# JeanElsner/practical-multi-view

Hardware: AMD Instinct MI355X
Metric: VO frames/sec on 1241x376 KITTI mono @400 tracks, bundle=5 (higher is better)
Workload: dtype u8/int32 front-end, f64 back-end

## Files before the change

### include/pmv_hip.h

```cpp
#ifndef PMV_HIP_H
#define PMV_HIP_H
#include <stdint.h>
#ifdef __cplusplus
extern "C" {
#endif

typedef struct pmv_ctx pmv_ctx;

enum pmv_status {
    PMV_OK = 0,
    PMV_ERR_NO_DEVICE = -1,
    PMV_ERR_INVALID = -2,
    PMV_ERR_CAPACITY = -3,
    PMV_ERR_HIP = -4,
    PMV_ERR_DEGENERATE = -5,
    PMV_ERR_OVERFLOW = -6
};

int pmv_ctx_create(pmv_ctx** out, int device, int max_w, int max_h, int n_slots, int max_tracks,
                   int max_ba_cams, int max_ba_points, int max_ba_obs);
void pmv_ctx_destroy(pmv_ctx* ctx);
const char* pmv_last_error(pmv_ctx* ctx);
const char* pmv_thread_error(void);
int pmv_sync(pmv_ctx* ctx);

int pmv_frame_upload(pmv_ctx* ctx, int slot, const uint8_t* gray, int w, int h, int stride);
int pmv_frame_upload_bgr(pmv_ctx* ctx, int slot, const uint8_t* bgr, int w, int h, int stride);
enum pmv_frame_format { PMV_FRAMES_GRAY = 0, PMV_FRAMES_BGR = 1 };
int pmv_set_frame_format(pmv_ctx* ctx, int format);
int pmv_frames_stage(pmv_ctx* ctx, int first_slot, int n, const uint8_t* gray, int w, int h);
int pmv_frames_build(pmv_ctx* ctx, int first_slot, int n);
int pmv_frames_stream_begin(pmv_ctx* ctx, int first_slot, int n, const uint8_t* gray, int w, int h);
int pmv_frames_stream_end(pmv_ctx* ctx);
int pmv_frame_get_level(pmv_ctx* ctx, int slot, int level, uint8_t* out, int* w, int* h);
int pmv_frame_num_levels(pmv_ctx* ctx, int slot);
#define PMV_PYR_PAD 64
int pmv_frame_get_level_padded(pmv_ctx* ctx, int slot, int level, uint8_t* out, int* pw, int* ph);

typedef struct pmv_clahe_params {
    double clip_limit;
    int tiles_x, tiles_y;
} pmv_clahe_params;
int pmv_frames_clahe(pmv_ctx* ctx, int first_slot, int n, const pmv_clahe_params* p);
int pmv_debug_clahe_launches(pmv_ctx* ctx, long long* out3);

int pmv_remap_map_create(pmv_ctx* ctx, int w, int h, const float* map_x, const float* map_y, int* out_id);
int pmv_remap_map_destroy(pmv_ctx* ctx, int id);
int pmv_frames_remap(pmv_ctx* ctx, int first_slot, int n, int map_id, int border_value);
int pmv_debug_remap_launches(pmv_ctx* ctx, long long* out3);
#define PMV_PREPROC_MAX_MAPS 8
typedef struct pmv_frame_preproc {
    int n_maps;
    int map_ids[PMV_PREPROC_MAX_MAPS];
    int border_value;
    int clahe;
    pmv_clahe_params clahe_params;
} pmv_frame_preproc;
int pmv_set_frame_preproc(pmv_ctx* ctx, const pmv_frame_preproc* p_or_null);
int pmv_get_frame_preproc(pmv_ctx* ctx, pmv_frame_preproc* out);
int pmv_debug_preproc_launches(pmv_ctx* ctx, long long* out4);
int pmv_debug_mem_live(long long* out2);
int pmv_undistort_map_build(const double* K9, const double* dist8, const double* R9_or_null, const double* newK9_or_null, int w, int h, float* map_x,
                            float* map_y);

#define PMV_GFTT_UNLIMITED_CAP 4096
int pmv_detect_gftt(pmv_ctx* ctx, int slot, const int* cells, int n_cells, int max_per_cell, double quality,
                    double min_dist, int* out_xy, int* out_count);
typedef struct pmv_gftt_params {
    double quality;
    double min_dist;
    int    block_size;
    int    use_harris;
    double k;
} pmv_gftt_params;
int pmv_detect_gftt_ex(pmv_ctx* ctx, int slot, const int* cells, int n_cells, int max_per_cell, const pmv_gftt_params* p, const uint8_t* mask,
                       int mask_stride, int* out_xy, int* out_count);
int pmv_debug_gftt_response_ex(pmv_ctx* ctx, int slot, const int* cell, const pmv_gftt_params* p, float* out);
int pmv_debug_gftt_general(pmv_ctx* ctx, int on);
int pmv_detect_shitomasi(pmv_ctx* ctx, int slot, const int* cells, int n_cells, int max_per_cell, double quality,
                         int* out_xy, double* out_score, int* out_count);
int pmv_debug_gftt_response(pmv_ctx* ctx, int slot, const int* cell, float* out);
int pmv_debug_shitomasi_response(pmv_ctx* ctx, int slot, const int* cell, double* out);

typedef struct pmv_subpix_params {
    int win_w, win_h;
    int zero_w, zero_h;
    int max_iter;
    double eps;
} pmv_subpix_params;
int pmv_corner_subpix(pmv_ctx* ctx, int slot, float* xy, int n, const pmv_subpix_params* p, uint8_t* out_iters, uint8_t* out_flags);
int pmv_debug_subpix_launches(pmv_ctx* ctx, long long* out3);

int pmv_detect_fast(pmv_ctx* ctx, int slot, const int* cells, int n_cells, int max_per_cell, int threshold, int nonmax, int* out_xy,
                    float* out_response, int* out_count);

int pmv_knn_match(pmv_ctx* ctx, int src_slot, int cmp_slot, const int* src_xy, int n, const int* cmp_xy, int m, int n_neighbours, int window,
                  int* out_best, float* out_err);
int pmv_lk_track(pmv_ctx* ctx, int prev_slot, int next_slot, const float* prev_xy, int n, float* out_xy,
                 uint8_t* out_status, float* out_err);
typedef struct pmv_lk_params {
    int win;
    int max_level;
    int max_iter;
    double eps;
    float min_eig;
} pmv_lk_params;
int pmv_set_lk_params(pmv_ctx* ctx, const pmv_lk_params* p);
int pmv_get_lk_params(pmv_ctx* ctx, pmv_lk_params* out);
enum { PMV_LK_USE_INITIAL_FLOW = 4, PMV_LK_GET_MIN_EIGENVALS = 8 };
int pmv_lk_track_ex(pmv_ctx* ctx, int prev_slot, int next_slot, const float* prev_xy, int n, float* next_xy , int flags,
                    uint8_t* out_status, float* out_err);
int pmv_lk_track_fb(pmv_ctx* ctx, int prev_slot, int next_slot, const float* prev_xy, int n, float* next_xy , int flags,
                    uint8_t* out_status, float* out_err, float* back_xy, uint8_t* back_status, float* back_err);
int pmv_debug_lk_general(pmv_ctx* ctx, int on);

int pmv_pnp_ransac(pmv_ctx* ctx, const float* obj_xyz, const float* img_xy, int m, const double* K, double* rvec,
                   double* tvec, int iterations, float reproj_err, double confidence, int* out_inliers,
                   int* out_n_inliers);

int pmv_debug_pnp_hypotheses(pmv_ctx* ctx, int n, double* models, int* counts);
int pmv_debug_ba_stamps(pmv_ctx* ctx, unsigned long long* out32);
int pmv_debug_lk_stamps(pmv_ctx* ctx, unsigned long long* out16);

typedef struct pmv_ba_summary {
    double initial_cost, final_cost;
    int iterations;
    int successful_steps;
    int termination;
} pmv_ba_summary;

int pmv_ba_residuals(pmv_ctx* ctx, const double* cams, int nc, const double* pts, int np, const double* obs_xy,
                     const int* cam_idx, const int* pt_idx, int n_obs, const double* K, double* out_r,
                     double* out_J);
int pmv_set_ba_mode(pmv_ctx* ctx, int mode);
int pmv_ba_solve(pmv_ctx* ctx, double* cams, int nc, double* pts, int np, const double* obs_xy, const int* cam_idx,
                 const int* pt_idx, int n_obs, const double* K, double huber_delta, int max_iterations,
                 pmv_ba_summary* summary);

int pmv_fivepoint_hypotheses(pmv_ctx* ctx, const double* q1, const double* q2, int n, const int* samples, int n_hyp, float thr, double* models,
                             int* n_models, int* counts);

int pmv_triangulate_candidates(pmv_ctx* ctx, const double* q1, const double* q2, int n, const double* P1x4,
                               const uint8_t* mask_in, double* out_Q, uint8_t* out_mask, int* out_good);
int pmv_triangulate_candidates_ahead(pmv_ctx* ctx, const double* q1, const double* q2, int n, const double* P1x4, const uint8_t* mask_in,
                                     double* out_Q, uint8_t* out_mask, int* out_good);

int pmv_find_essential_mat(pmv_ctx* ctx, const double* p1_xy, const double* p2_xy, int n, const double* K, double prob, double threshold,
                           double* E9, uint8_t* mask, int* out_found, int* out_samples_drawn);
int pmv_recover_pose(pmv_ctx* ctx, const double* E9, const double* p1_xy, const double* p2_xy, int n, const double* K, double* R9, double* t3,
                     uint8_t* mask, double* tri4n, int* out_good);
int pmv_debug_essential_iters_table(int n, double prob, double* out_denoms, double* out_num);

int pmv_find_fundamental_mat(pmv_ctx* ctx, const float* p1_xy, const float* p2_xy, int n, double threshold, double confidence, double* F9,
                             uint8_t* mask, int* out_found, int* out_samples_drawn);
int pmv_debug_fundamental_iters_table(int n, double confidence, double* out_denoms, double* out_num);
int pmv_debug_set_fundamental_r(int r);
int pmv_debug_fundamental_r(void);
int pmv_debug_whole_rounds(pmv_ctx* ctx, long long* out3);

int pmv_record_enable(pmv_ctx* ctx, int on);
int pmv_record_count(pmv_ctx* ctx);
long long pmv_record_size(pmv_ctx* ctx, int i);
int pmv_record_get(pmv_ctx* ctx, int i, void* out, long long capacity);

int pmv_prof_enable(pmv_ctx* ctx, int on);
int pmv_prof_select(pmv_ctx* ctx, unsigned mask);
int pmv_prof_kernel_count(void);
int pmv_lk_counters(pmv_ctx* ctx, unsigned long long* out3, int reset);
const char* pmv_prof_kernel_name(int id);
int pmv_prof_read(pmv_ctx* ctx, int id, int* launches, double* total_ms, double* max_ms);

typedef struct pmv_pipeline_params {
    int n_frames, w, h;
    int min_tracked_features, tracked_features_tol, init_frames, bundle_size, ba_iterations;
    int extractor;
    int threaded;
    int n_threads;
    int build_pyramids;
    int matcher;
    int device_fivepoint;
} pmv_pipeline_params;
typedef struct pmv_pipeline_result pmv_pipeline_result;

int pmv_pipeline_run(pmv_ctx* ctx, const pmv_pipeline_params* params, const double* K9, const double* gt_poses12,
                     pmv_pipeline_result** out);
int pmv_pipeline_run_streamed(pmv_ctx* ctx, const pmv_pipeline_params* params, const double* K9, const double* gt_poses12,
                              const uint8_t* host_frames, pmv_pipeline_result** out);
int pmv_pipeline_run_batch(pmv_ctx* ctx, int B, const pmv_pipeline_params* params, const double* K9, const double* const* gt_poses12,
                           const int* first_slot, pmv_pipeline_result** out);
int pmv_debug_batch_launches(pmv_ctx* ctx, long long* out4);
int pmv_pipeline_run_batch_streamed(pmv_ctx* ctx, int B, const pmv_pipeline_params* params, const double* K9, const double* const* gt_poses12,
                                    const uint8_t* const* host_frames, const int* first_slot, int ring, pmv_pipeline_result** out);
#define PMV_BATCH_INGEST_STATS 6
int pmv_batch_ingest_stats(pmv_ctx* ctx, double* out);
int pmv_batch_stats(pmv_ctx* ctx, long long* counts10, double* times15);

int pmv_batch_open(pmv_ctx* ctx, int n_seq, const int* sizes_wh, int n_sizes);
int pmv_batch_close(pmv_ctx* ctx);
int pmv_batch_frame_upload(pmv_ctx* ctx, int slot, const uint8_t* pixels, int w, int h, int stride, int format);
int pmv_batch_frame_upload_clahe(pmv_ctx* ctx, int slot, const uint8_t* pixels, int w, int h, int stride, int format, const pmv_clahe_params* p);
int pmv_batch_frame_upload_remap(pmv_ctx* ctx, int slot, const uint8_t* pixels, int w, int h, int stride, int format, int map_id, int border_value,
                                 const pmv_clahe_params* clahe_or_null);
int pmv_batch_lk_track(pmv_ctx* ctx, int prev_slot, int next_slot, const float* prev_xy, int n, float* out_xy, uint8_t* out_status, float* out_err);
int pmv_batch_lk_track_ex(pmv_ctx* ctx, int prev_slot, int next_slot, const float* prev_xy, int n, float* next_xy , int flags,
                          uint8_t* out_status, float* out_err);
int pmv_batch_lk_track_fb(pmv_ctx* ctx, int prev_slot, int next_slot, const float* prev_xy, int n, float* next_xy , int flags,
                          uint8_t* out_status, float* out_err, float* back_xy, uint8_t* back_status, float* back_err);
int pmv_batch_knn_match(pmv_ctx* ctx, int src_slot, int cmp_slot, const int* src_xy, int n, const int* cmp_xy, int m, int n_neighbours, int window,
                        int* out_best, float* out_err);
int pmv_batch_detect_gftt(pmv_ctx* ctx, int slot, const int* cells, int n_cells, int max_per_cell, double quality, double min_dist, int* out_xy,
                          int* out_count);
int pmv_batch_detect_gftt_ex(pmv_ctx* ctx, int slot, const int* cells, int n_cells, int max_per_cell, const pmv_gftt_params* p, const uint8_t* mask,
                             int mask_stride, int* out_xy, int* out_count);
int pmv_batch_corner_subpix(pmv_ctx* ctx, int slot, float* xy, int n, const pmv_subpix_params* p, uint8_t* out_iters, uint8_t* out_flags);
int pmv_batch_detect_shitomasi(pmv_ctx* ctx, int slot, const int* cells, int n_cells, int max_per_cell, double quality, int* out_xy, double* out_score,
                               int* out_count);
int pmv_batch_detect_fast(pmv_ctx* ctx, int slot, const int* cells, int n_cells, int max_per_cell, int threshold, int nonmax, int* out_xy,
                          float* out_response, int* out_count);
int pmv_batch_pnp_ransac(pmv_ctx* ctx, int seq, const float* obj_xyz, const float* img_xy, int m, const double* K, double* rvec, double* tvec,
                         int iterations, float reproj_err, double confidence, int* out_inliers, int* out_n_inliers);
int pmv_batch_ba_solve(pmv_ctx* ctx, int seq, double* cams, int nc, double* pts, int np, const double* obs_xy, const int* cam_idx, const int* pt_idx,
                       int n_obs, const double* K, double huber_delta, int max_iterations, pmv_ba_summary* summary);
int pmv_batch_triangulate_candidates(pmv_ctx* ctx, int seq, const double* q1, const double* q2, int n, const double* P1x4, const uint8_t* mask_in,
                                     double* out_Q, uint8_t* out_mask, int* out_good);
int pmv_batch_fivepoint_hypotheses(pmv_ctx* ctx, int seq, const double* q1, const double* q2, int n, const int* samples, int n_hyp, float thr,
                                   double* models, int* n_models, int* counts);
int pmv_batch_find_essential_mat(pmv_ctx* ctx, int seq, const double* p1_xy, const double* p2_xy, int n, const double* K, double prob, double threshold,
                                 double* E9, uint8_t* mask, int* out_found, int* out_samples_drawn);
int pmv_batch_recover_pose(pmv_ctx* ctx, int seq, const double* E9, const double* p1_xy, const double* p2_xy, int n, const double* K, double* R9, double* t3,
                           uint8_t* mask, double* tri4n, int* out_good);
int pmv_batch_find_fundamental_mat(pmv_ctx* ctx, int seq, const float* p1_xy, const float* p2_xy, int n, double threshold, double confidence,
                                   double* F9, uint8_t* mask, int* out_found, int* out_samples_drawn);
int pmv_batch_upload_stats(pmv_ctx* ctx, long long* out4);
int pmv_batch_upload_rounds(pmv_ctx* ctx, int* out8, int capacity);

void pmv_pipeline_free(pmv_pipeline_result* r);
void pmv_pipeline_release(pmv_pipeline_result* r);
void pmv_pipeline_drain(void);
int pmv_pipeline_num_poses(const pmv_pipeline_result* r);
void pmv_pipeline_get_poses(const pmv_pipeline_result* r, double* out12);
int pmv_pipeline_num_frames(const pmv_pipeline_result* r);
int pmv_pipeline_frame_feature_count(const pmv_pipeline_result* r, int k);
void pmv_pipeline_get_frame_features(const pmv_pipeline_result* r, int k, int* out3);
int pmv_pipeline_stats_count(void);
void pmv_pipeline_get_stats(const pmv_pipeline_result* r, double* out25);

#ifdef __cplusplus
}
#endif
#endif
```

### practical-multi-view_amd/__init__.py

```python
import ctypes as C
import os

import numpy as np

from . import build as _build

HERE = os.path.dirname(os.path.abspath(__file__))
ROOT = os.path.dirname(HERE)

_u8p = C.POINTER(C.c_uint8)
_i32p = C.POINTER(C.c_int)
_f32p = C.POINTER(C.c_float)
_f64p = C.POINTER(C.c_double)


class PmvError(RuntimeError):
    def __init__(self, code, msg):
        super().__init__(f"pmv error {code}: {msg}")
        self.code = code


class BaSummary(C.Structure):
    _fields_ = [("initial_cost", C.c_double), ("final_cost", C.c_double), ("iterations", C.c_int),
                ("successful_steps", C.c_int), ("termination", C.c_int)]


class LKParams(C.Structure):
    _fields_ = [("win", C.c_int), ("max_level", C.c_int), ("max_iter", C.c_int), ("eps", C.c_double), ("min_eig", C.c_float)]


class GfttParams(C.Structure):
    _fields_ = [("quality", C.c_double), ("min_dist", C.c_double), ("block_size", C.c_int), ("use_harris", C.c_int), ("k", C.c_double)]


class SubpixParams(C.Structure):
    _fields_ = [("win_w", C.c_int), ("win_h", C.c_int), ("zero_w", C.c_int), ("zero_h", C.c_int), ("max_iter", C.c_int), ("eps", C.c_double)]


class ClaheParams(C.Structure):
    _fields_ = [("clip_limit", C.c_double), ("tiles_x", C.c_int), ("tiles_y", C.c_int)]


def _clahe_params(who, clip_limit, tiles):
    if isinstance(clip_limit, (bool, np.bool_)) or not isinstance(clip_limit, (int, float, np.integer, np.floating)):
        raise ValueError(f"{who}: clip_limit must be a number, got {clip_limit!r}")
    try:
        tx, ty = tiles
    except (TypeError, ValueError):
        raise ValueError(f"{who}: tiles is a (tiles_x, tiles_y) pair, got {tiles!r}") from None
    for t in (tx, ty):
        if isinstance(t, (bool, np.bool_)) or not isinstance(t, (int, np.integer)):
            raise ValueError(f"{who}: tiles is a pair of integers, got {tiles!r}")
    return ClaheParams(float(clip_limit), int(tx), int(ty))


PREPROC_MAX_MAPS = 8


class FramePreproc(C.Structure):
    _fields_ = [("n_maps", C.c_int), ("map_ids", C.c_int * PREPROC_MAX_MAPS), ("border_value", C.c_int), ("clahe", C.c_int), ("clahe_params", ClaheParams)]


def _preproc_arg(who, remap, border_value, clahe):
    def is_int(v):
        return isinstance(v, (int, np.integer)) and not isinstance(v, (bool, np.bool_))
    if remap is None:
        ids = []
    elif is_int(remap):
        ids = [int(remap)]
    else:
        try:
            ids = list(remap)
        except TypeError:
            raise ValueError(f"{who}: remap is a map id or a sequence of map ids, got {remap!r}") from None
        if isinstance(remap, (str, bytes)) or not all(is_int(i) for i in ids):
            raise ValueError(f"{who}: remap is a map id or a sequence of integer map ids, got {remap!r}")
        ids = [int(i) for i in ids]
    if len(ids) > PREPROC_MAX_MAPS:
        raise ValueError(f"{who}: at most {PREPROC_MAX_MAPS} maps, got {len(ids)}")
    if not is_int(border_value) or not 0 <= int(border_value) <= 255:
        raise ValueError(f"{who}: border_value is an integer in 0..255, got {border_value!r}")
    p = FramePreproc()
    p.n_maps = len(ids)
    for k, i in enumerate(ids):
        p.map_ids[k] = i
    p.border_value = int(border_value)
    if clahe is not None:
        try:
            clip, tiles = clahe
        except (TypeError, ValueError):
            raise ValueError(f"{who}: clahe is None or (clip_limit, (tiles_x, tiles_y)), got {clahe!r}") from None
        cp = _clahe_params(who, clip, tiles)
        if not (cp.clip_limit >= 0.0 and np.isfinite(cp.clip_limit)):
            raise ValueError(f"{who}: clip_limit is a finite number >= 0, got {clip!r}")
        if not (1 <= cp.tiles_x <= 16 and 1 <= cp.tiles_y <= 16):
            raise ValueError(f"{who}: tiles are in 1..16 each, got {tiles!r}")
        p.clahe = 1
        p.clahe_params = cp
    if not ids and clahe is None and int(border_value) == 0:
        return None
    return p


def _remap_arg(who, remap):
    def is_int(v):
        return isinstance(v, (int, np.integer)) and not isinstance(v, (bool, np.bool_))
    if is_int(remap):
        return int(remap), 0
    try:
        map_id, border = remap
    except (TypeError, ValueError):
        raise ValueError(f"{who}: remap is a map id or (map_id, border_value), got {remap!r}") from None
    if not is_int(map_id) or not is_int(border):
        raise ValueError(f"{who}: remap is a map id or (map_id, border_value) of integers, got {remap!r}")
    return int(map_id), int(border)


def undistort_map(K, dist, size, R=None, new_K=None):
    def mat(m, name):
        a = np.ascontiguousarray(m, np.float64)
        if a.shape != (3, 3):
            raise ValueError(f"undistort_map: {name} is 3 x 3, got shape {a.shape}")
        return a
    Km = mat(K, "K")
    d = np.asarray(dist, np.float64).reshape(-1)
    if d.size > 8:
        raise ValueError(f"undistort_map: at most 8 distortion coefficients (k1, k2, p1, p2, k3, k4, k5, k6), got {d.size}")
    d8 = np.zeros(8, np.float64)
    d8[:d.size] = d
    try:
        w, h = size
    except (TypeError, ValueError):
        raise ValueError(f"undistort_map: size is (w, h), got {size!r}") from None
    w, h = int(w), int(h)
    if w < 1 or h < 1:
        raise ValueError(f"undistort_map: size {size!r}")
    Rm = None if R is None else mat(R, "R")
    Nm = None if new_K is None else mat(new_K, "new_K")
    mx, my = np.empty((h, w), np.float32), np.empty((h, w), np.float32)
    lib = load_library()
    _f32p = C.POINTER(C.c_float)
    lib.pmv_undistort_map_build.argtypes = [_f64p, _f64p, _f64p, _f64p, C.c_int, C.c_int, _f32p, _f32p]
    rc = lib.pmv_undistort_map_build(_p(Km, _f64p), _p(d8, _f64p), None if Rm is None else _p(Rm, _f64p), None if Nm is None else _p(Nm, _f64p), w, h,
                                     _p(mx, _f32p), _p(my, _f32p))
    if rc != 0:
        raise PmvError(rc, lib.pmv_last_error(None).decode())
    return mx, my


def mem_live():
    lib = load_library()
    out = (C.c_longlong * 2)()
    lib.pmv_debug_mem_live.argtypes = [C.POINTER(C.c_longlong)]
    rc = lib.pmv_debug_mem_live(out)
    if rc != 0:
        raise PmvError(rc, lib.pmv_last_error(None).decode())
    return int(out[0]), int(out[1])


LK_USE_INITIAL_FLOW = 4
LK_GET_MIN_EIGENVALS = 8

ABI_SYMBOLS = [
    "pmv_ctx_create", "pmv_ctx_destroy", "pmv_last_error", "pmv_thread_error", "pmv_sync",
    "pmv_frame_upload", "pmv_frame_upload_bgr", "pmv_set_frame_format", "pmv_frames_stage", "pmv_frames_build", "pmv_frames_stream_begin", "pmv_frames_stream_end", "pmv_frame_get_level", "pmv_frame_get_level_padded", "pmv_frame_num_levels",
    "pmv_detect_gftt", "pmv_detect_shitomasi", "pmv_detect_fast", "pmv_knn_match", "pmv_debug_gftt_response", "pmv_debug_shitomasi_response",
    "pmv_detect_gftt_ex", "pmv_debug_gftt_response_ex", "pmv_debug_gftt_general", "pmv_batch_detect_gftt_ex",
    "pmv_corner_subpix", "pmv_batch_corner_subpix", "pmv_debug_subpix_launches",
    "pmv_frames_clahe", "pmv_batch_frame_upload_clahe", "pmv_debug_clahe_launches",
    "pmv_remap_map_create", "pmv_remap_map_destroy", "pmv_frames_remap", "pmv_debug_remap_launches", "pmv_batch_frame_upload_remap", "pmv_undistort_map_build",
    "pmv_set_frame_preproc", "pmv_get_frame_preproc", "pmv_debug_preproc_launches",
    "pmv_debug_mem_live",
    "pmv_lk_track", "pmv_lk_track_ex", "pmv_lk_track_fb", "pmv_set_lk_params", "pmv_get_lk_params", "pmv_debug_lk_general", "pmv_set_ba_mode", "pmv_pnp_ransac", "pmv_debug_pnp_hypotheses", "pmv_debug_ba_stamps", "pmv_debug_lk_stamps", "pmv_ba_residuals", "pmv_ba_solve", "pmv_triangulate_candidates", "pmv_triangulate_candidates_ahead", "pmv_fivepoint_hypotheses",
    "pmv_find_essential_mat", "pmv_recover_pose", "pmv_debug_essential_iters_table",
    "pmv_find_fundamental_mat", "pmv_debug_fundamental_iters_table", "pmv_debug_set_fundamental_r", "pmv_debug_fundamental_r", "pmv_debug_whole_rounds",
    "pmv_record_enable", "pmv_record_count", "pmv_record_size", "pmv_record_get",
    "pmv_prof_enable", "pmv_prof_select", "pmv_prof_kernel_count", "pmv_lk_counters", "pmv_prof_kernel_name", "pmv_prof_read",
    "pmv_pipeline_run", "pmv_pipeline_run_streamed", "pmv_pipeline_run_batch", "pmv_pipeline_run_batch_streamed", "pmv_batch_ingest_stats", "pmv_batch_stats", "pmv_debug_batch_launches", "pmv_pipeline_free", "pmv_pipeline_release", "pmv_pipeline_drain", "pmv_pipeline_num_poses", "pmv_pipeline_get_poses", "pmv_pipeline_num_frames",
    "pmv_pipeline_frame_feature_count", "pmv_pipeline_get_frame_features", "pmv_pipeline_stats_count", "pmv_pipeline_get_stats",
    "pmv_batch_open", "pmv_batch_close", "pmv_batch_frame_upload", "pmv_batch_upload_stats", "pmv_batch_upload_rounds",
    "pmv_batch_lk_track", "pmv_batch_lk_track_ex", "pmv_batch_lk_track_fb", "pmv_batch_knn_match", "pmv_batch_detect_gftt", "pmv_batch_detect_shitomasi", "pmv_batch_detect_fast",
    "pmv_batch_pnp_ransac", "pmv_batch_ba_solve", "pmv_batch_triangulate_candidates", "pmv_batch_fivepoint_hypotheses",
    "pmv_batch_find_essential_mat", "pmv_batch_recover_pose", "pmv_batch_find_fundamental_mat",
]


GFTT_UNLIMITED_CAP = 4096


class PipelineParams(C.Structure):
    _fields_ = [("n_frames", C.c_int), ("w", C.c_int), ("h", C.c_int), ("min_tracked_features", C.c_int),
                ("tracked_features_tol", C.c_int), ("init_frames", C.c_int), ("bundle_size", C.c_int),
                ("ba_iterations", C.c_int), ("extractor", C.c_int), ("threaded", C.c_int), ("n_threads", C.c_int),
                ("build_pyramids", C.c_int), ("matcher", C.c_int), ("device_fivepoint", C.c_int)]


STAT_KEYS = ["lk_calls", "lk_points", "detect_calls", "pnp_calls", "pnp_points", "tri_calls", "ba_calls", "ba_obs",
             "ba_points", "heuristic_motion", "seconds", "init_offset", "n_landmarks", "scale", "t_lk", "t_detect", "t_pnp", "t_tri",
             "t_ba", "t_pnp_kernel", "t_ba_kernel", "t_tri_essential", "t_tri_pose", "tri_hypotheses", "tri_ahead"]


BATCH_INGEST_KEYS = ["rounds", "frames", "bytes", "memcpy_s", "ingest_wait_s", "seq_wait_s"]


FRAME_FORMATS = {"gray": 0, "bgr": 1}


def _host_frames(frames, fmt, who, h=None, w=None, n=None):
    if fmt != "bgr":
        f = np.ascontiguousarray(frames, np.uint8)
        if f.ndim != 3 or (h is not None and f.shape[1:] != (h, w)) or (n is not None and f.shape[0] != n):
            want = f"({'n' if n is None else n}, {'h' if h is None else h}, {'w' if w is None else w})"
            raise ValueError(f"{who}: the context's frame format is gray: frames must be {want} uint8, got {f.shape} (set_frame_format(\"bgr\") for colour frames)")
        return f
    f = np.asarray(frames)
    ok = f.dtype == np.uint8 and f.ndim == 4 and f.shape[3] == 3 and f.shape[0] >= 1
    if ok and h is not None:
        ok = f.shape[1:3] == (h, w)
    if ok and n is not None:
        ok = f.shape[0] == n
    if not ok:
        want = f"({'n' if n is None else n}, {'h' if h is None else h}, {'w' if w is None else w}, 3)"
        raise ValueError(f"{who}: the context's frame format is BGR: frames must be {want} uint8, got {f.shape} {f.dtype}")
    return np.ascontiguousarray(f)


def _batch_streamed_args(seqs, w, h, ring, first_slot, fmt="gray"):
    if len(seqs) < 1:
        raise ValueError("pipeline_run_batch_streamed: no sequences")
    if int(ring) != ring or ring < 1:
        raise ValueError(f"pipeline_run_batch_streamed: ring must be a positive integer, got {ring!r}")
    if (w is None) != (h is None):
        raise ValueError("pipeline_run_batch_streamed: w and h are given together, or both None (each sequence's own array shape)")
    ws = hs = [None] * len(seqs)
    if w is not None:
        ws = _per_sequence("pipeline_run_batch_streamed", "w", w, len(seqs))
        hs = _per_sequence("pipeline_run_batch_streamed", "h", h, len(seqs))
    frames, gts = [], []
    for b, seq in enumerate(seqs):
        if len(seq) != 2:
            raise ValueError(f"pipeline_run_batch_streamed: sequence {b} must be (frames, gt_poses)")
        f, gt = seq
        f = np.asarray(f)
        if fmt == "bgr":
            f = _host_frames(f, fmt, f"pipeline_run_batch_streamed: sequence {b}", hs[b], ws[b])
        elif f.dtype != np.uint8 or f.ndim != 3 or (ws[b] is not None and f.shape[1:] != (hs[b], ws[b])):
            want = f"(n, {hs[b]}, {ws[b]})" if ws[b] is not None else "(n, h, w)"
            raise ValueError(f"pipeline_run_batch_streamed: sequence {b}: frames must be {want} uint8, got {f.shape} {f.dtype}")
        f = np.ascontiguousarray(f)
        g = np.ascontiguousarray(gt, np.float64)
        if g.size != 12 * f.shape[0]:
            raise ValueError(f"pipeline_run_batch_streamed: sequence {b}: {f.shape[0]} frames but {g.size / 12:g} pose rows")
        frames.append(f)
        gts.append(g.reshape(f.shape[0], 12))
    B = len(frames)
    first = [b * int(ring) for b in range(B)] if first_slot is None else [int(v) for v in first_slot]
    if len(first) != B:
        raise ValueError(f"pipeline_run_batch_streamed: {len(first)} first slots for {B} sequences")
    return frames, gts, first


BATCH_UPLOAD_KEYS = ["rounds", "frames", "level0_launches", "pyrdown_launches"]


def _session_sizes(sizes):
    try:
        pairs = [tuple(p) for p in sizes]
    except TypeError:
        raise ValueError(f"batch_open: sizes must be a sequence of (w, h) integer pairs, got {sizes!r}") from None
    if not pairs:
        raise ValueError("batch_open: no sizes")
    for p in pairs:
        if len(p) != 2 or any(isinstance(v, (bool, np.bool_)) or not isinstance(v, (int, np.integer)) for v in p):
            raise ValueError(f"batch_open: sizes must be (w, h) integer pairs, got {p!r}")
    return np.asarray(pairs, np.int32).reshape(-1)


def _upload_source(frame, fmt):
    if not isinstance(fmt, str) or fmt not in FRAME_FORMATS:
        raise ValueError(f"batch_frame_upload: fmt must be one of {sorted(FRAME_FORMATS)}, got {fmt!r}")
    nd = 3 if fmt == "bgr" else 2
    if isinstance(frame, np.ndarray):
        if frame.dtype != np.uint8:
            raise ValueError(f"batch_frame_upload: frames are uint8, got {frame.dtype}")
        shape, strides, addr = tuple(frame.shape), tuple(frame.strides), frame.ctypes.data
    elif all(hasattr(frame, a) for a in ("data_ptr", "shape", "stride")):
        dt = str(getattr(frame, "dtype", "uint8"))
        if not dt.endswith("uint8"):
            raise ValueError(f"batch_frame_upload: frames are uint8, got {dt}")
        shape, strides, addr = tuple(int(v) for v in frame.shape), tuple(int(v) for v in frame.stride()), int(frame.data_ptr())
    else:
        raise ValueError(f"batch_frame_upload: a uint8 numpy array or an object with data_ptr(), shape and stride() is needed, got {type(frame).__name__}")
    if len(shape) != nd or (nd == 3 and shape[2] != 3):
        want = "(h, w, 3)" if nd == 3 else "(h, w)"
        raise ValueError(f"batch_frame_upload: a {fmt} frame is {want} uint8, got shape {shape}")
    h, w = shape[0], shape[1]
    if h < 1 or w < 1:
        raise ValueError(f"batch_frame_upload: empty frame {shape}")
    if (nd == 2 and strides[1] != 1) or (nd == 3 and (strides[2] != 1 or strides[1] != 3)):
        raise ValueError(f"batch_frame_upload: the pixels of a row must be contiguous (strides {strides} for shape {shape}); only the row stride is free")
    stride = strides[0] if h > 1 else max(strides[0], w * (nd == 3 and 3 or 1))
    if stride < w * (3 if nd == 3 else 1) or stride >= 2 ** 31:
        raise ValueError(f"batch_frame_upload: row stride {strides[0]} bytes for rows of {w * (3 if nd == 3 else 1)} bytes (overlapping or reversed rows)")
    return addr, w, h, stride, FRAME_FORMATS[fmt], frame


def _per_sequence(who, name, value, B):
    if np.ndim(value) == 0:
        return [int(value)] * B
    v = [int(x) for x in value]
    if len(v) != B:
        raise ValueError(f"{who}: {name} has {len(v)} entries for {B} sequences")
    return v


class PipelineResult:

    def __init__(self, lib, handle, want_features=True):
        n = lib.pmv_pipeline_num_poses(handle)
        self.poses = np.zeros((n, 12), np.float64)
        if n:
            lib.pmv_pipeline_get_poses(handle, _p(self.poses, _f64p))
        self.features = []
        if want_features:
            for k in range(lib.pmv_pipeline_num_frames(handle)):
                c = lib.pmv_pipeline_frame_feature_count(handle, k)
# ... 298 lines not shown
        return out

    def debug_gftt_general(self, on):
        self._ck(self.lib.pmv_debug_gftt_general(self.h, 1 if on else 0))

    def _corner_subpix(self, fn, ck, slot, xy, win, zero_zone, max_iter, eps, return_info):
        if not isinstance(xy, np.ndarray) or xy.dtype != np.float32 or xy.ndim != 2 or xy.shape[1] != 2:
            raise ValueError("corner_subpix: xy must be an (n, 2) float32 array")
        if len(win) != 2 or len(zero_zone) != 2:
            raise ValueError("corner_subpix: win and zero_zone are (w, h) pairs of half sizes")
        out = np.ascontiguousarray(xy).copy()
        n = out.shape[0]
        iters = np.zeros(n, np.uint8)
        flags = np.zeros(n, np.uint8)
        p = SubpixParams(int(win[0]), int(win[1]), int(zero_zone[0]), int(zero_zone[1]), int(max_iter), float(eps))
        fn.argtypes = [C.c_void_p, C.c_int, _f32p, C.c_int, C.POINTER(SubpixParams), _u8p, _u8p]
        ck(fn(self.h, int(slot), _p(out, _f32p), n, C.byref(p), _p(iters, _u8p) if return_info else None, _p(flags, _u8p) if return_info else None))
        return (out, iters, flags) if return_info else out

    def corner_subpix(self, slot, xy, win=(5, 5), zero_zone=(-1, -1), max_iter=30, eps=0.01, return_info=False):
        return self._corner_subpix(self.lib.pmv_corner_subpix, self._ck, slot, xy, win, zero_zone, max_iter, eps, return_info)

    def debug_subpix_launches(self):
        out = (C.c_longlong * 3)()
        self.lib.pmv_debug_subpix_launches.argtypes = [C.c_void_p, C.POINTER(C.c_longlong)]
        self._ck(self.lib.pmv_debug_subpix_launches(self.h, out))
        return [int(v) for v in out]

    def detect_shitomasi(self, slot, cells, max_per_cell, quality=0.4):
        cells = np.ascontiguousarray(cells, np.int32).reshape(-1, 4)
        n = cells.shape[0]
        xy = np.zeros((n, max(max_per_cell, 1), 2), np.int32)
        sc = np.zeros((n, max(max_per_cell, 1)), np.float64)
        cnt = np.zeros(n, np.int32)
        self._ck(self.lib.pmv_detect_shitomasi(self.h, slot, _p(cells, _i32p), n, max_per_cell, C.c_double(quality),
                                               _p(xy, _i32p), _p(sc, _f64p), _p(cnt, _i32p)))
        return [(xy[i, : cnt[i]].copy(), sc[i, : cnt[i]].copy()) for i in range(n)]

    def detect_fast(self, slot, cells, max_per_cell, threshold=10, nonmax=True):
        cells = np.ascontiguousarray(cells, np.int32).reshape(-1, 4)
        n = cells.shape[0]
        cap = max(max_per_cell, 1)
        xy = np.zeros((n, cap, 2), np.int32)
        rs = np.zeros((n, cap), np.float32)
        cnt = np.zeros(n, np.int32)
        self._ck(self.lib.pmv_detect_fast(self.h, slot, _p(cells, _i32p), n, max_per_cell, threshold, 1 if nonmax else 0, _p(xy, _i32p), _p(rs, _f32p),
                                          _p(cnt, _i32p)))
        return [(xy[i, : cnt[i]].copy(), rs[i, : cnt[i]].copy()) for i in range(n)]

    def knn_match(self, src_slot, cmp_slot, src_xy, cmp_xy, neighbours=7, window=15):
        s = np.ascontiguousarray(src_xy, np.int32).reshape(-1, 2)
        c = np.ascontiguousarray(cmp_xy, np.int32).reshape(-1, 2)
        best = np.zeros(max(len(s), 1), np.int32)
        err = np.zeros(max(len(s), 1), np.float32)
        self._ck(self.lib.pmv_knn_match(self.h, src_slot, cmp_slot, _p(s, _i32p), len(s), _p(c, _i32p), len(c), neighbours, window, _p(best, _i32p), _p(err, _f32p)))
        return best[: len(s)].copy(), err[: len(s)].copy()

    def gftt_response(self, slot, cell):
        cell = np.ascontiguousarray(cell, np.int32)
        out = np.zeros((cell[3], cell[2]), np.float32)
        self._ck(self.lib.pmv_debug_gftt_response(self.h, slot, _p(cell, _i32p), _p(out, _f32p)))
        return out

    def shitomasi_response(self, slot, cell):
        cell = np.ascontiguousarray(cell, np.int32)
        out = np.zeros((cell[3], cell[2]), np.float64)
        self._ck(self.lib.pmv_debug_shitomasi_response(self.h, slot, _p(cell, _i32p), _p(out, _f64p)))
        return out

    def lk_track(self, prev_slot, next_slot, prev_xy):
        p = np.ascontiguousarray(prev_xy, np.float32).reshape(-1, 2)
        n = p.shape[0]
        out = np.zeros((n, 2), np.float32)
        st = np.zeros(n, np.uint8)
        err = np.zeros(n, np.float32)
        self._ck(self.lib.pmv_lk_track(self.h, prev_slot, next_slot, _p(p, _f32p), n, _p(out, _f32p), _p(st, _u8p),
                                       _p(err, _f32p)))
        return out, st, err

    def _lk_ex(self, fn, ck, fb, prev_slot, next_slot, prev_xy, init_xy, min_eigenvals):
        p = np.ascontiguousarray(prev_xy, np.float32).reshape(-1, 2)
        n = p.shape[0]
        flags = (LK_USE_INITIAL_FLOW if init_xy is not None else 0) | (LK_GET_MIN_EIGENVALS if min_eigenvals else 0)
        nxt = np.zeros((n, 2), np.float32) if init_xy is None else np.array(init_xy, np.float32).reshape(-1, 2)
        if nxt.shape[0] != n:
            raise ValueError(f"init_xy has {nxt.shape[0]} points, prev_xy {n}")
        st = np.zeros(n, np.uint8)
        err = np.zeros(n, np.float32)
        args = [self.h, int(prev_slot), int(next_slot), _p(p, _f32p), n, _p(nxt, _f32p), flags, _p(st, _u8p), _p(err, _f32p)]
        if not fb:
            ck(fn(*args))
            return nxt, st, err
        bxy = np.zeros((n, 2), np.float32)
        bst = np.zeros(n, np.uint8)
        berr = np.zeros(n, np.float32)
        ck(fn(*args, _p(bxy, _f32p), _p(bst, _u8p), _p(berr, _f32p)))
        return nxt, st, err, bxy, bst, berr

    def lk_track_ex(self, prev_slot, next_slot, prev_xy, init_xy=None, min_eigenvals=False):
        return self._lk_ex(self.lib.pmv_lk_track_ex, self._ck, False, prev_slot, next_slot, prev_xy, init_xy, min_eigenvals)

    def lk_track_fb(self, prev_slot, next_slot, prev_xy, init_xy=None, min_eigenvals=False):
        return self._lk_ex(self.lib.pmv_lk_track_fb, self._ck, True, prev_slot, next_slot, prev_xy, init_xy, min_eigenvals)

    def set_lk_params(self, win=32, max_level=4, max_iter=30, eps=0.01, min_eig=1e-4):
        p = LKParams(int(win), int(max_level), int(max_iter), float(eps), float(min_eig))
        self.lib.pmv_set_lk_params.argtypes = [C.c_void_p, C.POINTER(LKParams)]
        self._ck(self.lib.pmv_set_lk_params(self.h, C.byref(p)))

    def lk_params(self):
        p = LKParams()
        self.lib.pmv_get_lk_params.argtypes = [C.c_void_p, C.POINTER(LKParams)]
        self._ck(self.lib.pmv_get_lk_params(self.h, C.byref(p)))
        return dict(win=p.win, max_level=p.max_level, max_iter=p.max_iter, eps=p.eps, min_eig=p.min_eig)

    def debug_lk_general(self, on):
        self._ck(self.lib.pmv_debug_lk_general(self.h, 1 if on else 0))

    def pnp_ransac(self, obj_xyz, img_xy, K, rvec, tvec, iterations=100, reproj_err=8.0, confidence=0.99):
        o = np.ascontiguousarray(obj_xyz, np.float32).reshape(-1, 3)
        i2 = np.ascontiguousarray(img_xy, np.float32).reshape(-1, 2)
        m = o.shape[0]
        Kd = np.ascontiguousarray(K, np.float64).reshape(9)
        rv = np.array(rvec, np.float64).reshape(3).copy()
        tv = np.array(tvec, np.float64).reshape(3).copy()
        inl = np.zeros(max(m, 1), np.int32)
        nin = C.c_int()
        self._ck(self.lib.pmv_pnp_ransac(self.h, _p(o, _f32p), _p(i2, _f32p), m, _p(Kd, _f64p), _p(rv, _f64p),
                                         _p(tv, _f64p), iterations, C.c_float(reproj_err), C.c_double(confidence),
                                         _p(inl, _i32p), C.byref(nin)))
        return rv, tv, inl[: nin.value].copy()

    def pnp_hypotheses(self, n=100):
        models = np.zeros((n, 6), np.float64)
        counts = np.zeros(n, np.int32)
        self._ck(self.lib.pmv_debug_pnp_hypotheses(self.h, n, _p(models, _f64p), _p(counts, _i32p)))
        return models, counts

    def ba_residuals(self, cams, pts, obs_xy, cam_idx, pt_idx, K):
        cams = np.ascontiguousarray(cams, np.float64).reshape(-1, 6)
        pts = np.ascontiguousarray(pts, np.float64).reshape(-1, 3)
        obs = np.ascontiguousarray(obs_xy, np.float64).reshape(-1, 2)
        ci = np.ascontiguousarray(cam_idx, np.int32)
        pi = np.ascontiguousarray(pt_idx, np.int32)
        Kd = np.ascontiguousarray(K, np.float64).reshape(9)
        n = obs.shape[0]
        r = np.zeros((n, 2), np.float64)
        J = np.zeros((n, 2, 9), np.float64)
        self._ck(self.lib.pmv_ba_residuals(self.h, _p(cams, _f64p), cams.shape[0], _p(pts, _f64p), pts.shape[0],
                                           _p(obs, _f64p), _p(ci, _i32p), _p(pi, _i32p), n, _p(Kd, _f64p),
                                           _p(r, _f64p), _p(J, _f64p)))
        return r, J

    def set_ba_mode(self, mode):
        self._ck(self.lib.pmv_set_ba_mode(self.h, int(mode)))

    def ba_solve(self, cams, pts, obs_xy, cam_idx, pt_idx, K, huber=1.0, max_iterations=5):
        cams = np.array(cams, np.float64).reshape(-1, 6).copy()
        pts = np.array(pts, np.float64).reshape(-1, 3).copy()
        obs = np.ascontiguousarray(obs_xy, np.float64).reshape(-1, 2)
        ci = np.ascontiguousarray(cam_idx, np.int32)
        pi = np.ascontiguousarray(pt_idx, np.int32)
        Kd = np.ascontiguousarray(K, np.float64).reshape(9)
        s = BaSummary()
        self._ck(self.lib.pmv_ba_solve(self.h, _p(cams, _f64p), cams.shape[0], _p(pts, _f64p), pts.shape[0],
                                       _p(obs, _f64p), _p(ci, _i32p), _p(pi, _i32p), obs.shape[0], _p(Kd, _f64p),
                                       C.c_double(huber), max_iterations, C.byref(s)))
        return cams, pts, s

    def fivepoint_hypotheses(self, q1, q2, samples, thr):
        q1 = np.ascontiguousarray(q1, np.float64).reshape(-1, 2)
        q2 = np.ascontiguousarray(q2, np.float64).reshape(-1, 2)
        s = np.ascontiguousarray(samples, np.int32).reshape(-1, 5)
        nh = s.shape[0]
        models = np.zeros((nh, 10, 9), np.float64)
        nm = np.zeros(nh, np.int32)
        counts = np.zeros((nh, 10), np.int32)
        self._ck(self.lib.pmv_fivepoint_hypotheses(self.h, _p(q1, _f64p), _p(q2, _f64p), q1.shape[0], _p(s, _i32p), nh, C.c_float(thr), _p(models, _f64p),
                                                   _p(nm, _i32p), _p(counts, _i32p)))
        return models, nm, counts

    def triangulate_candidates(self, q1, q2, P1x4, mask_in):
        q1 = np.ascontiguousarray(q1, np.float64).reshape(-1, 2)
        q2 = np.ascontiguousarray(q2, np.float64).reshape(-1, 2)
        n = q1.shape[0]
        P = np.ascontiguousarray(P1x4, np.float64).reshape(48)
        mi = np.ascontiguousarray(mask_in, np.uint8).reshape(n)
        Q = np.zeros((4, 4, n), np.float64)
        mask = np.zeros((4, n), np.uint8)
        good = np.zeros(4, np.int32)
        self._ck(self.lib.pmv_triangulate_candidates(self.h, _p(q1, _f64p), _p(q2, _f64p), n, _p(P, _f64p), _p(mi, _u8p),
                                                     _p(Q, _f64p), _p(mask, _u8p), _p(good, _i32p)))
        return Q, mask, good

    @staticmethod
    def _two_view_args(p1, p2, K):
        p1 = np.ascontiguousarray(p1, np.float64).reshape(-1, 2)
        p2 = np.ascontiguousarray(p2, np.float64).reshape(-1, 2)
        if p1.shape != p2.shape:
            raise ValueError(f"p1 {p1.shape} and p2 {p2.shape}: one (x, y) pair per correspondence in each")
        return p1, p2, np.ascontiguousarray(K, np.float64).reshape(9)

    def _find_essential(self, call, ck, head, p1, p2, K, prob, threshold):
        p1, p2, Kd = self._two_view_args(p1, p2, K)
        n = p1.shape[0]
        E = np.zeros(9, np.float64)
        mask = np.zeros(n, np.uint8)
        found, drawn = C.c_int(), C.c_int()
        ck(call(self.h, *head, _p(p1, _f64p), _p(p2, _f64p), n, _p(Kd, _f64p), C.c_double(prob), C.c_double(threshold), _p(E, _f64p), _p(mask, _u8p),
                C.byref(found), C.byref(drawn)))
        return bool(found.value), E.reshape(3, 3), mask, drawn.value

    def _recover_pose(self, call, ck, head, E, p1, p2, K, mask):
        p1, p2, Kd = self._two_view_args(p1, p2, K)
        n = p1.shape[0]
        Ed = np.ascontiguousarray(E, np.float64).reshape(9)
        m = np.array(mask, np.uint8).reshape(n).copy()
        R, t, tri = np.zeros(9, np.float64), np.zeros(3, np.float64), np.zeros((4, n), np.float64)
        good = C.c_int()
        ck(call(self.h, *head, _p(Ed, _f64p), _p(p1, _f64p), _p(p2, _f64p), n, _p(Kd, _f64p), _p(R, _f64p), _p(t, _f64p), _p(m, _u8p), _p(tri, _f64p),
                C.byref(good)))
        return R.reshape(3, 3), t, m, tri, good.value

    def find_essential_mat(self, p1, p2, K, prob=0.99, threshold=1.0):
        return self._find_essential(self.lib.pmv_find_essential_mat, self._ck, (), p1, p2, K, prob, threshold)

    def recover_pose(self, E, p1, p2, K, mask):
        return self._recover_pose(self.lib.pmv_recover_pose, self._ck, (), E, p1, p2, K, mask)

    def _find_fundamental(self, call, ck, head, p1, p2, threshold, confidence):
        p1 = np.ascontiguousarray(p1, np.float32).reshape(-1, 2)
        p2 = np.ascontiguousarray(p2, np.float32).reshape(-1, 2)
        if p1.shape != p2.shape:
            raise ValueError(f"p1 {p1.shape} and p2 {p2.shape}: one (x, y) pair per correspondence in each")
        n = p1.shape[0]
        F = np.zeros(9, np.float64)
        mask = np.zeros(n, np.uint8)
        found, drawn = C.c_int(), C.c_int()
        ck(call(self.h, *head, _p(p1, _f32p), _p(p2, _f32p), n, C.c_double(threshold), C.c_double(confidence), _p(F, _f64p), _p(mask, _u8p),
                C.byref(found), C.byref(drawn)))
        return bool(found.value), F.reshape(3, 3), mask, drawn.value

    def find_fundamental_mat(self, p1, p2, threshold=1.0, confidence=0.99):
        return self._find_fundamental(self.lib.pmv_find_fundamental_mat, self._ck, (), p1, p2, threshold, confidence)

    def record_enable(self, on=True):
        self._ck(self.lib.pmv_record_enable(self.h, 1 if on else 0))

    def records(self):
        self.lib.pmv_record_size.restype = C.c_longlong
        self.lib.pmv_record_size.argtypes = [C.c_void_p, C.c_int]
        self.lib.pmv_record_get.argtypes = [C.c_void_p, C.c_int, C.c_void_p, C.c_longlong]
        out = []
        for i in range(self.lib.pmv_record_count(self.h)):
            nb = self.lib.pmv_record_size(self.h, i)
            buf = np.zeros(nb, np.uint8)
            self._ck(self.lib.pmv_record_get(self.h, i, buf.ctypes.data_as(C.c_void_p), nb))
            out.append(parse_record(buf))
        return out

    def prof_enable(self, on=True):
        self._ck(self.lib.pmv_prof_enable(self.h, 1 if on else 0))

    def lk_counters(self, reset=False):
        out = (C.c_ulonglong * 3)()
        self._ck(self.lib.pmv_lk_counters(self.h, out, 1 if reset else 0))
        return int(out[0]), int(out[1]), int(out[2])

    def prof_select(self, names):
        self.lib.pmv_prof_kernel_name.restype = C.c_char_p
        mask = 0
        for i in range(self.lib.pmv_prof_kernel_count()):
            if self.lib.pmv_prof_kernel_name(i).decode() in names:
                mask |= 1 << i
        self._ck(self.lib.pmv_prof_select(self.h, C.c_uint(mask)))

    def prof_read(self):
        self.lib.pmv_prof_kernel_name.restype = C.c_char_p
        out = {}
        for i in range(self.lib.pmv_prof_kernel_count()):
            n, tot, mx = C.c_int(), C.c_double(), C.c_double()
            self._ck(self.lib.pmv_prof_read(self.h, i, C.byref(n), C.byref(tot), C.byref(mx)))
            if n.value:
                out[self.lib.pmv_prof_kernel_name(i).decode()] = (n.value, tot.value, mx.value)
        return out

    def pipeline_run(self, n_frames, w, h, K, gt_poses, min_tracked=400, tol=150, init_frames=5, bundle_size=5,
                     ba_iterations=5, extractor=0, threaded=0, build_pyramids=1, want_features=True, n_threads=1, async_free=False,
                     defer_free=False, host_frames=None, matcher=0, device_fivepoint=0):
        P = PipelineParams(n_frames, w, h, min_tracked, tol, init_frames, bundle_size, ba_iterations, extractor, threaded,
                           n_threads, build_pyramids, matcher, device_fivepoint)
        Kd = np.ascontiguousarray(K, np.float64).reshape(9)
        gt = np.ascontiguousarray(gt_poses, np.float64).reshape(n_frames, 12)
        out = C.c_void_p()
        if host_frames is not None:
            hf = _host_frames(host_frames, self.frame_format, "pipeline_run: host_frames", h, w, n_frames)
            self._ck(self.lib.pmv_pipeline_run_streamed(self.h, C.byref(P), _p(Kd, _f64p), _p(gt, _f64p), _p(hf, _u8p), C.byref(out)))
        else:
            self._ck(self.lib.pmv_pipeline_run(self.h, C.byref(P), _p(Kd, _f64p), _p(gt, _f64p), C.byref(out)))
        ok = False
        try:
            r = PipelineResult(self.lib, out, want_features)
            ok = True
        finally:
            if not (ok and defer_free):
                if async_free:
# ... 282 lines not shown
```

### practical-multi-view_amd/csrc/backend.h

```cpp
#pragma once
#include <hip/hip_runtime.h>
#include <stdint.h>
#include <stddef.h>
#include "../../include/pmv_hip.h"
#include "pmv_mem.h"
#include "backend_layout.h"

namespace pmv {


struct BackendBuffers {
    unsigned done_seq = 0;
    Buf<double> d_cams, d_pts, d_obs, d_K;
    Buf<int> d_cam_idx, d_pt_idx, d_pobs_start, d_pobs_list, d_cobs_start, d_cobs_list;
    Buf<double> d_x, d_cand, d_scale, d_diag, d_D2, d_step, d_res, d_J, d_Einv, d_gp, d_Yd, d_Wd, d_S, d_rhs, d_Gpart, d_summary;
    size_t ydwd_elems = 0, gpart_elems = 0;
    Buf<unsigned long long> d_stamps;
    Buf<void> d_bastate;
    Buf<double> d_bapart;
    Buf<char> d_tri_in, d_tri_out;
    Buf<char> d_fp_work;
    Buf<char> d_ess_in;
    Buf<char> d_fund_in;
    Buf<char> h_stage;
    Buf<char> d_ba_io;
    Buf<char> d_pnp_in;
    Buf<char> d_pnp_out;
    Buf<float> d_obj, d_img;
    Buf<int> d_samples, d_counts, d_inliers, d_info;
    Buf<double> d_models, d_rt, d_Kp;
    Buf<uint8_t> d_masks;
};

struct BAArgs {
    double* cams; double* pts; const double* obs; const int* cam_idx; const int* pt_idx; const double* K;
    const int* pobs_start; const int* pobs_list; const int* cobs_start; const int* cobs_list;
    const int4* erec;
    int nc, np, nobs, max_iterations;
    double huber;
    double *x, *cand, *scale, *diag, *D2, *step, *res, *J, *Einv, *gp, *Yd, *Wd, *S, *rhs, *Gpart, *summary;
    int ldw, krows, tiles_r, tiles_c, kslices, kper, gp_rows;
    unsigned long long* stamps;
    double* out;
    unsigned done_seq;
};

hipError_t launch_ba_residuals(hipStream_t s, const double* cams, const double* pts, const double* obs, const int* cam_idx,
                               const int* pt_idx, int nobs, const double* K, double* out_r, double* out_J);
hipError_t launch_ba_lm(hipStream_t s, const BAArgs& A);
constexpr int BA_MAX_ITERATIONS = 512;
hipError_t launch_ba_multi(hipStream_t s, const BAArgs& A, void* d_state, double* d_part);
hipError_t launch_pnp(hipStream_t s, const float* d_obj, const float* d_img, int m, const double* d_K, const int* d_samples,
                      int n_hyp, float thr, double confidence, double* d_models, uint8_t* d_masks, int* d_counts,
                      double* d_rt_out, int* d_inliers, int* d_info, char* host_out ,
                      unsigned long long* d_stamps , unsigned done_seq = 0 );

struct BAProb {
    BAArgs A;
    void* st2[2];
    int* chol_flags;
    double *part_cost, *part_gmax, *part4, *Ublk, *rhsblk, *candrot, *tmp3;
    int nbo, nbp, clear_blocks, tiles;
};
struct BABatchDims { int n_probs, max_eval_blocks, max_nc, max_nbp, max_tiles, max_m, max_iterations; };
void ba_fill_prob(BAProb& P, const BAArgs& A, void* d_state, double* d_part);
hipError_t launch_ba_multi_batch(hipStream_t s, const BAProb* d_probs, const BABatchDims& D);
hipError_t launch_ba_lm_batch(hipStream_t s, const BAArgs* d_args, int n_probs, int max_m);
struct PnPProblem {
    const float* obj; const float* img; const int* samples; const double* K;
    double* models; uint8_t* masks; int* counts; double* rt_out; int* inliers; int* info; char* host_out;
    int m, n_hyp; float thr; double confidence;
};
hipError_t launch_pnp_batch(hipStream_t s, const PnPProblem* d_probs, int n_probs, int max_hyp);
struct FivePointProblem {
    const int* samples; const double* q1; const double* q2;
    double* models_d; int* n_models_d;
    double* models_h; int* n_models_h; int* counts_h;
    int n, n_hyp; float thr;
};
hipError_t launch_fivepoint_batch(hipStream_t s, const FivePointProblem* d_probs, int n_probs, int max_hyp);
struct EssentialProblem {
    const double* q1; const double* q2;
    const double* iters;
    char* out;
    int n, max_iters; float thr;
    unsigned done_seq;
};
static_assert(sizeof(EssentialProblem) <= ESS_HDR, "the record is the header of the input block");
constexpr int ESS_MAX_WAVES = 16;
constexpr int ESS_DEFAULT_WAVES = 8;
int essential_round_width();
hipError_t launch_essential_ransac(hipStream_t s, const EssentialProblem* d_probs, int n_probs);
struct FundamentalProblem {
    const float* p1; const float* p2;
    const double* iters;
    char* out;
    int n, max_iters; float thr;
    unsigned done_seq;
};
static_assert(sizeof(FundamentalProblem) <= ESS_HDR, "the record is the header of the input block");
constexpr int FUND_MAX_R = 64;
constexpr int FUND_DEFAULT_R = 64;
int fundamental_round_width();
void fundamental_set_round_width(int r);
hipError_t launch_fundamental_ransac(hipStream_t s, const FundamentalProblem* d_probs, int n_probs);
struct DltProblem { const double* P1x4; const double* q1; const double* q2; const uint8_t* mask_in; double* Q; uint8_t* mask; int n; };
hipError_t launch_tri_dlt_batch(hipStream_t s, const DltProblem* d_probs, int n_probs, int max_n);
hipError_t launch_tri_dlt(hipStream_t s, const double* d_P1x4, const double* d_q1, const double* d_q2, const uint8_t* d_mask_in, int n,
                          double* d_Q, uint8_t* d_mask);

struct PnPProblem; struct DltProblem;
}
struct pmv_ctx;
namespace pmv {
int backend_alloc(pmv_ctx* c, BackendBuffers** out);
void backend_free(BackendBuffers* b);
int pnp_check(pmv_ctx* ctx, const float* obj_xyz, const float* img_xy, int m, const double* K, double* rvec, double* tvec, int iterations,
              double confidence, int* out_inliers, int* out_n_inliers);
int pnp_prepare(pmv_ctx* ctx, BackendBuffers* b, const float* obj_xyz, const float* img_xy, int m, const double* K, int iterations, float reproj_err,
                double confidence, PnPProblem* P, PnPLayout* L);
void pnp_finish(pmv_ctx* ctx, BackendBuffers* b, const float* obj_xyz, const float* img_xy, int m, const double* K, double* rvec, double* tvec,
                int iterations, float reproj_err, double confidence, const PnPLayout& L, int* out_inliers, int* out_n_inliers);
int ba_check(pmv_ctx* ctx, const double* cams, int nc, const double* pts, int np, const double* obs_xy, const int* cam_idx, const int* pt_idx,
             int n_obs, const double* K, double huber_delta, int max_iterations);
int ba_prepare(pmv_ctx* ctx, BackendBuffers* b, const double* cams, int nc, const double* pts, int np, const double* obs_xy, const int* cam_idx,
               const int* pt_idx, int n_obs, const double* K, double huber_delta, int max_iterations, bool multi, BAArgs* A, BaIoLayout* L);
void ba_finish(pmv_ctx* ctx, BackendBuffers* b, double* cams, int nc, double* pts, int np, const double* obs_xy, const int* cam_idx,
               const int* pt_idx, int n_obs, const double* K, double huber_delta, int max_iterations, const BaIoLayout& L, pmv_ba_summary* summary);
int fivepoint_prepare(pmv_ctx* ctx, BackendBuffers* b, const double* q1, const double* q2, int n, const int* samples, int n_hyp, float thr,
                      FivePointProblem* P, FivePointLayout* L);
void fivepoint_finish(BackendBuffers* b, int n_hyp, const FivePointLayout& L, double* models, int* n_models, int* counts);
int essential_check(pmv_ctx* ctx, const char* who, const double* p1_xy, const double* p2_xy, int n, const double* K, double prob, double threshold,
                    double* E9, uint8_t* mask, int* out_found, int* out_samples_drawn);
int essential_prepare(pmv_ctx* ctx, BackendBuffers* b, const double* p1_xy, const double* p2_xy, int n, const double* K, double prob, double threshold,
                      EssentialProblem* P, WholeLayout* L);
volatile unsigned* whole_done_word(BackendBuffers* b, const WholeLayout& L);
void whole_finish(BackendBuffers* b, int n, const WholeLayout& L, double* M9, uint8_t* mask, int* out_found, int* out_samples_drawn);
int fundamental_check(pmv_ctx* ctx, const char* who, const float* p1_xy, const float* p2_xy, int n, double threshold, double confidence, double* F9,
                      uint8_t* mask, int* out_found, int* out_samples_drawn);
int fundamental_prepare(pmv_ctx* ctx, BackendBuffers* b, const float* p1_xy, const float* p2_xy, int n, double threshold, double confidence,
                        FundamentalProblem* P, WholeLayout* L);
int recover_pose_check(pmv_ctx* ctx, const char* who, const double* E9, const double* p1_xy, const double* p2_xy, int n, const double* K, double* R9,
                       double* t3, uint8_t* mask, double* tri4n, int* out_good);
int dlt_prepare(pmv_ctx* ctx, BackendBuffers* b, const double* q1, const double* q2, int n, const double* P1x4, const uint8_t* mask_in, DltProblem* P,
                DltLayout* L);
void dlt_finish(pmv_ctx* ctx, BackendBuffers* b, const double* q1, const double* q2, int n, const double* P1x4, const uint8_t* mask_in,
                const DltLayout& L, double* out_Q, uint8_t* out_mask, int* out_good);
}
```

### practical-multi-view_amd/csrc/backend.hip

```cpp
#include "pmv_ctx.h"
#include "backend.h"
#include "pmv_wait.h"
#include "vo_pipeline.h"
#include <cmath>
#include <cstring>
#include <cstdio>
#include <cstdlib>
#include <vector>
#include <algorithm>

namespace pmv {

__global__ __launch_bounds__(256) void k_stage_block(const uint4* __restrict__ src, uint4* __restrict__ dst, unsigned n16) { BACKEND_PRIO();
    for (unsigned i = blockIdx.x * 256 + threadIdx.x; i < n16; i += gridDim.x * 256) dst[i] = src[i];
}
hipError_t stage_block(hipStream_t s, const void* mapped_src, void* dst, size_t bytes, unsigned max_blocks) {
    const unsigned n16 = (unsigned)((bytes + 15) >> 4);
    hipLaunchKernelGGL(k_stage_block, dim3(std::min(max_blocks, (n16 + 255u) / 256u)), dim3(256), 0, s, (const uint4*)mapped_src, (uint4*)dst, n16);
    return hipGetLastError();
}
static bool stage_by_kernel() { static const bool on = !(getenv("PMV_BA_STAGE") && !strcmp(getenv("PMV_BA_STAGE"), "dma")); return on; }

static int round_up(int a, int b) { return (a + b - 1) / b * b; }

int backend_alloc(pmv_ctx* c, BackendBuffers** out) {
    BackendBuffers* b = new BackendBuffers();
    *out = b;
    const size_t nc = (size_t)std::max(c->max_ba_cams, 1), np = (size_t)std::max(c->max_ba_points, 1), no = (size_t)std::max(c->max_ba_obs, 1);
    const size_t n = 6 * nc + 3 * np, m = 6 * nc;
    const size_t ldw = (size_t)round_up((int)m + 1, 16), krows = (size_t)round_up((int)(3 * np), 16);
    b->ydwd_elems = krows * ldw;
    b->gpart_elems = (size_t)8 * ldw * ldw;
    const size_t mt = (size_t)c->max_tracks;
    const BackendCaps caps = backend_caps(c->max_tracks, c->max_ba_cams, c->max_ba_points, c->max_ba_obs);
    const MemRow rows[] = {
        {&b->d_cams, nc * 6 * 8, MEM_DEVICE}, {&b->d_pts, np * 3 * 8, MEM_DEVICE}, {&b->d_obs, no * 2 * 8, MEM_DEVICE}, {&b->d_K, 9 * 8, MEM_DEVICE},
        {&b->d_cam_idx, no * 4, MEM_DEVICE}, {&b->d_pt_idx, no * 4, MEM_DEVICE},
        {&b->d_pobs_start, (np + 1) * 4, MEM_DEVICE}, {&b->d_pobs_list, no * 4, MEM_DEVICE},
        {&b->d_cobs_start, (nc + 1) * 4, MEM_DEVICE}, {&b->d_cobs_list, no * 4, MEM_DEVICE},
        {&b->d_x, 2 * n * 8, MEM_DEVICE}, {&b->d_cand, n * 8, MEM_DEVICE}, {&b->d_scale, n * 8, MEM_DEVICE}, {&b->d_diag, n * 8, MEM_DEVICE},
        {&b->d_D2, n * 8, MEM_DEVICE}, {&b->d_step, n * 8, MEM_DEVICE},
        {&b->d_res, 2 * no * 2 * 8, MEM_DEVICE}, {&b->d_J, 2 * no * 18 * 8, MEM_DEVICE},
        {&b->d_Einv, np * 9 * 8, MEM_DEVICE}, {&b->d_gp, np * 3 * 8, MEM_DEVICE},
        {&b->d_Yd, 2 * b->ydwd_elems * 8, MEM_DEVICE},
        {&b->d_Wd, b->ydwd_elems * 8, MEM_DEVICE},
        {&b->d_S, m * m * 8, MEM_DEVICE}, {&b->d_rhs, m * 8, MEM_DEVICE},
        {&b->d_Gpart, b->gpart_elems * 8, MEM_DEVICE},
        {&b->d_summary, 8 * 8, MEM_DEVICE},
        {&b->d_stamps, 32 * 8, MEM_DEVICE},
        {&b->d_bastate, 512 + 4 * BA_MAX_ITERATIONS, MEM_DEVICE},
        {&b->d_bapart, ((size_t)(no + 255) / 256 + 5 * ((size_t)(np + 63) / 64) + 64 * (size_t)nc + 3 * (size_t)no + 64) * 8, MEM_DEVICE},
        {&b->d_obj, mt * 12, MEM_DEVICE}, {&b->d_img, mt * 8, MEM_DEVICE},
        {&b->d_samples, MAX_HYP * 5 * 4, MEM_DEVICE}, {&b->d_counts, MAX_HYP * 4, MEM_DEVICE},
        {&b->d_inliers, mt * 4, MEM_DEVICE}, {&b->d_info, 16, MEM_DEVICE},
        {&b->d_models, MAX_HYP * 6 * 8, MEM_DEVICE}, {&b->d_rt, 6 * 8, MEM_DEVICE}, {&b->d_Kp, 9 * 8, MEM_DEVICE},
        {&b->d_masks, (size_t)MAX_HYP * mt, MEM_DEVICE},
        {&b->d_ba_io, caps.ba_io, MEM_DEVICE},
        {&b->d_pnp_in, caps.pnp_in, MEM_DEVICE}, {&b->d_pnp_out, caps.pnp_out, MEM_DEVICE},
        {&b->d_tri_in, caps.tri_in, MEM_DEVICE}, {&b->d_tri_out, caps.tri_out, MEM_DEVICE},
        {&b->d_fp_work, (size_t)FP_MAX_HYP * (90 * 8 + 4) + 64, MEM_DEVICE},
        {&b->d_ess_in, caps.ess_in, MEM_DEVICE},
        {&b->h_stage, caps.h_stage, MEM_MAPPED},
    };
    hipError_t e = mem_alloc_table(rows, sizeof(rows) / sizeof(rows[0]));
    if (e == hipSuccess) e = hipMemset(b->d_stamps, 0, 32 * 8);
    if (e != hipSuccess) { set_err(c, "backend_alloc: %s", hipGetErrorString(e)); return PMV_ERR_HIP; }
    return PMV_OK;
}
int backend_create(pmv_ctx* c) { return backend_alloc(c, &c->be); }

void backend_free(BackendBuffers* b) { delete b; }
void backend_destroy(pmv_ctx* c) {
    if (c->s_ahead) { (void)hipStreamSynchronize(c->s_ahead); (void)hipStreamDestroy(c->s_ahead); c->s_ahead = nullptr; }
    backend_free(c->be); c->be = nullptr;
    backend_free(c->be_ahead); c->be_ahead = nullptr;
}

struct CvRNG {
    uint64_t state;
    explicit CvRNG(uint64_t s) : state(s ? s : 0xffffffffULL) {}
    unsigned next() { state = (uint64_t)(unsigned)state * 4164903690U + (unsigned)(state >> 32); return (unsigned)state; }
    int uniform(int a, int b) { return a == b ? a : (int)(next() % (unsigned)(b - a) + a); }
};

}

using namespace pmv;

#define CKC(x) do { hipError_t e_ = (x); if (e_ != hipSuccess) { set_err(ctx, "%s: %s", #x, hipGetErrorString(e_)); return PMV_ERR_HIP; } } while (0)
#define REQ(cond, code, ...) do { if (!(cond)) { set_err(ctx, __VA_ARGS__); return code; } } while (0)

int pmv::pnp_check(pmv_ctx* ctx, const float* obj_xyz, const float* img_xy, int m, const double* K, double* rvec, double* tvec, int iterations,
                   double confidence, int* out_inliers, int* out_n_inliers) {
    REQ(ctx && obj_xyz && img_xy && K && rvec && tvec && out_inliers && out_n_inliers, PMV_ERR_INVALID, "pmv_pnp_ransac: null argument");
    *out_n_inliers = 0;
    REQ(m <= ctx->max_tracks, PMV_ERR_CAPACITY, "pmv_pnp_ransac: m=%d exceeds max_tracks=%d", m, ctx->max_tracks);
    REQ(m >= 6, PMV_ERR_DEGENERATE, "pmv_pnp_ransac: %d correspondences (need >= 6)", m);
    REQ(iterations >= 1 && iterations <= MAX_HYP, PMV_ERR_CAPACITY, "pmv_pnp_ransac: iterations=%d (1..%d)", iterations, MAX_HYP);
    REQ(confidence > 0 && confidence < 1, PMV_ERR_INVALID, "pmv_pnp_ransac: confidence must be in (0,1)");
    return PMV_OK;
}
int pmv::pnp_prepare(pmv_ctx* ctx, BackendBuffers* b, const float* obj_xyz, const float* img_xy, int m, const double* K, int iterations, float reproj_err,
                     double confidence, PnPProblem* P, PnPLayout* Lout) {
    const PnPLayout L = pnp_layout((size_t)m, (size_t)iterations);
    REQ(L.total <= b->h_stage.cap && L.in_bytes <= b->d_pnp_in.cap && L.total - L.out <= b->d_pnp_out.cap, PMV_ERR_CAPACITY,
        "pmv_pnp_ransac: m=%d with %d iterations does not fit the staging blocks", m, iterations);
    char* hs = (char*)b->h_stage;
    double* h_K = (double*)(hs + L.K);
    int* h_samples = (int*)(hs + L.samples);
    memcpy(h_K, K, 72);
    for (int k = -16; k <= 16; k++) h_K[10 + 16 + k] = std::exp(k * std::log(10.));
    memcpy(hs + L.obj, obj_xyz, (size_t)m * 12);
    memcpy(hs + L.img, img_xy, (size_t)m * 8);
    CvRNG rng((uint64_t)-1);
    for (int it = 0; it < iterations; it++) {
        int* idx = h_samples + it * 5;
        for (int i = 0; i < 5;) {
            int idx_i;
            for (;;) {
                idx_i = idx[i] = rng.uniform(0, m);
                int j = 0;
                for (; j < i; j++) if (idx_i == idx[j]) break;
                if (j == i) break;
            }
            i++;
        }
    }
    P->K = (const double*)(b->d_pnp_in + L.K);
    P->obj = (const float*)(b->d_pnp_in + L.obj);
    P->img = (const float*)(b->d_pnp_in + L.img);
    P->samples = (const int*)(b->d_pnp_in + L.samples);
    P->models = b->d_models; P->masks = b->d_masks; P->counts = b->d_counts;
    P->rt_out = (double*)b->d_pnp_out;
    P->info = (int*)(b->d_pnp_out + PNP_OUT_INFO);
    P->inliers = (int*)(b->d_pnp_out + PNP_OUT_INLIERS);
    P->host_out = b->h_stage.dm() + L.out;
    P->m = m; P->n_hyp = iterations;
    P->thr = (float)((double)reproj_err * (double)reproj_err);
    P->confidence = confidence;
    *Lout = L;
    return PMV_OK;
}
void pmv::pnp_finish(pmv_ctx* ctx, BackendBuffers* b, const float* obj_xyz, const float* img_xy, int m, const double* K, double* rvec, double* tvec,
                     int iterations, float reproj_err, double confidence, const PnPLayout& L, int* out_inliers, int* out_n_inliers) {
    const PnPResultHdr* R = (const PnPResultHdr*)((const char*)b->h_stage + L.out);
    const double* h_rt = R->rt;
    const int* h_inl = (const int*)((const char*)b->h_stage + L.inliers);
    const int n = R->info[0];
    if (ctx->log.on) {
        std::lock_guard<std::mutex> lk(ctx->log.mu);
        ctx->log.blobs.emplace_back();
        std::vector<char>& bl = ctx->log.blobs.back();
        const int hdr[4] = {0, m, iterations, n};
        const double opt[2] = {(double)reproj_err, confidence};
        pmv_call_log::put(bl, hdr, 16); pmv_call_log::put(bl, obj_xyz, (size_t)m * 12); pmv_call_log::put(bl, img_xy, (size_t)m * 8);
        pmv_call_log::put(bl, K, 72); pmv_call_log::put(bl, rvec, 24); pmv_call_log::put(bl, tvec, 24); pmv_call_log::put(bl, opt, 16);
        pmv_call_log::put(bl, h_rt, 48); pmv_call_log::put(bl, h_inl, (size_t)(n > 0 ? n : 0) * 4);
    }
    for (int i = 0; i < 3; i++) { rvec[i] = h_rt[i]; tvec[i] = h_rt[3 + i]; }
    *out_n_inliers = n;
    if (n > 0) memcpy(out_inliers, h_inl, (size_t)n * 4);
}

static int wait_done_word(pmv_ctx* ctx, hipStream_t s, volatile unsigned* done_word, unsigned done_seq, bool by_word) {
    if (by_word) CKC(spin_for_word(s, done_word, done_seq));
    else CKC(hipStreamSynchronize(s));
    return PMV_OK;
}

extern "C" {

static bool stamps_on() { static const bool on = getenv("PMV_BA_STAMPS") != nullptr; return on; }

int pmv_pnp_ransac(pmv_ctx* ctx, const float* obj_xyz, const float* img_xy, int m, const double* K, double* rvec, double* tvec,
                   int iterations, float reproj_err, double confidence, int* out_inliers, int* out_n_inliers) {
    int rc = pnp_check(ctx, obj_xyz, img_xy, m, K, rvec, tvec, iterations, confidence, out_inliers, out_n_inliers);
    if (rc) return rc;
    tl_prof = &ctx->prof;
    CKC(hipSetDevice(ctx->device));
    static const char* const dump = getenv("PMV_DUMP_PNP");
    if (dump) {
        if (FILE* f = fopen(dump, "ab")) {
            fwrite(&m, 4, 1, f); fwrite(obj_xyz, 12, m, f); fwrite(img_xy, 8, m, f); fwrite(K, 8, 9, f); fwrite(rvec, 8, 3, f); fwrite(tvec, 8, 3, f);
            fclose(f);
        }
    }
    BackendBuffers* b = ctx->be;
    hipStream_t s = ctx->s_back;
    PnPProblem P;
    PnPLayout L;
    if ((rc = pnp_prepare(ctx, b, obj_xyz, img_xy, m, K, iterations, reproj_err, confidence, &P, &L))) return rc;
    if (stage_by_kernel()) CKC(stage_block(s, b->h_stage.dm(), b->d_pnp_in, L.in_bytes, 8));
    else CKC(hipMemcpyAsync(b->d_pnp_in, b->h_stage, L.in_bytes, hipMemcpyHostToDevice, s));
    const bool flag_wait = back_wait_by_word();
    volatile unsigned* done_word = (volatile unsigned*)((char*)b->h_stage + L.done);
    if (++b->done_seq == 0) b->done_seq = 1;
    *done_word = 0;
    CKC(launch_pnp(s, P.obj, P.img, m, P.K, P.samples, iterations, P.thr, confidence, P.models, P.masks, P.counts,
                   P.rt_out, P.inliers, P.info, P.host_out, stamps_on() ? b->d_stamps : nullptr, flag_wait ? b->done_seq : 0u));
    if ((rc = wait_done_word(ctx, s, done_word, b->done_seq, flag_wait))) return rc;
    pnp_finish(ctx, b, obj_xyz, img_xy, m, K, rvec, tvec, iterations, reproj_err, confidence, L, out_inliers, out_n_inliers);
    return PMV_OK;
}

int pmv_record_enable(pmv_ctx* ctx, int on) {
    REQ(ctx, PMV_ERR_INVALID, "null ctx");
    if (on) ctx->log.blobs.clear();
    ctx->log.on = on != 0;
    return PMV_OK;
}
int pmv_record_count(pmv_ctx* ctx) { return ctx ? (int)ctx->log.blobs.size() : PMV_ERR_INVALID; }
long long pmv_record_size(pmv_ctx* ctx, int i) {
    if (!ctx || i < 0 || i >= (int)ctx->log.blobs.size()) return PMV_ERR_INVALID;
    return (long long)ctx->log.blobs[i].size();
}
int pmv_record_get(pmv_ctx* ctx, int i, void* out, long long capacity) {
    REQ(ctx && out && i >= 0 && i < (int)ctx->log.blobs.size(), PMV_ERR_INVALID, "pmv_record_get: bad argument");
    REQ(capacity >= (long long)ctx->log.blobs[i].size(), PMV_ERR_CAPACITY, "pmv_record_get: buffer too small");
    memcpy(out, ctx->log.blobs[i].data(), ctx->log.blobs[i].size());
    return PMV_OK;
}

int pmv_debug_ba_stamps(pmv_ctx* ctx, unsigned long long* out32) {
    REQ(ctx && out32, PMV_ERR_INVALID, "null argument");
    CKC(hipSetDevice(ctx->device));
    CKC(hipStreamSynchronize(ctx->s_back));
    CKC(hipMemcpy(out32, ctx->be->d_stamps, 256, hipMemcpyDeviceToHost));
    return PMV_OK;
}

int pmv_debug_pnp_hypotheses(pmv_ctx* ctx, int n, double* models, int* counts) {
    REQ(ctx && models && counts && n >= 1 && n <= MAX_HYP, PMV_ERR_INVALID, "pmv_debug_pnp_hypotheses: bad argument");
    CKC(hipSetDevice(ctx->device));
    CKC(hipStreamSynchronize(ctx->s_back));
    CKC(hipMemcpy(models, ctx->be->d_models, (size_t)n * 48, hipMemcpyDeviceToHost));
    CKC(hipMemcpy(counts, ctx->be->d_counts, (size_t)n * 4, hipMemcpyDeviceToHost));
    return PMV_OK;
}

int pmv_ba_residuals(pmv_ctx* ctx, const double* cams, int nc, const double* pts, int np, const double* obs_xy, const int* cam_idx,
                     const int* pt_idx, int n_obs, const double* K, double* out_r, double* out_J) {
    REQ(ctx && cams && pts && obs_xy && cam_idx && pt_idx && K && out_r && out_J, PMV_ERR_INVALID, "pmv_ba_residuals: null argument");
    REQ(nc >= 1 && nc <= ctx->max_ba_cams && np >= 1 && np <= ctx->max_ba_points && n_obs >= 0 && n_obs <= ctx->max_ba_obs, PMV_ERR_CAPACITY,
        "pmv_ba_residuals: nc=%d np=%d n_obs=%d exceed capacity %d/%d/%d", nc, np, n_obs, ctx->max_ba_cams, ctx->max_ba_points, ctx->max_ba_obs);
    for (int i = 0; i < n_obs; i++) REQ(cam_idx[i] >= 0 && cam_idx[i] < nc && pt_idx[i] >= 0 && pt_idx[i] < np, PMV_ERR_INVALID, "pmv_ba_residuals: index out of range at observation %d", i);
    if (n_obs == 0) return PMV_OK;
    tl_prof = &ctx->prof;
    CKC(hipSetDevice(ctx->device));
    BackendBuffers* b = ctx->be;
    hipStream_t s = ctx->s_back;
    CKC(hipMemcpyAsync(b->d_cams, cams, (size_t)nc * 48, hipMemcpyHostToDevice, s));
    CKC(hipMemcpyAsync(b->d_pts, pts, (size_t)np * 24, hipMemcpyHostToDevice, s));
    CKC(hipMemcpyAsync(b->d_obs, obs_xy, (size_t)n_obs * 16, hipMemcpyHostToDevice, s));
    CKC(hipMemcpyAsync(b->d_cam_idx, cam_idx, (size_t)n_obs * 4, hipMemcpyHostToDevice, s));
    CKC(hipMemcpyAsync(b->d_pt_idx, pt_idx, (size_t)n_obs * 4, hipMemcpyHostToDevice, s));
    CKC(hipMemcpyAsync(b->d_K, K, 72, hipMemcpyHostToDevice, s));
    CKC(launch_ba_residuals(s, b->d_cams, b->d_pts, b->d_obs, b->d_cam_idx, b->d_pt_idx, n_obs, b->d_K, b->d_res, b->d_J));
    CKC(hipMemcpyAsync(out_r, b->d_res, (size_t)n_obs * 16, hipMemcpyDeviceToHost, s));
    CKC(hipMemcpyAsync(out_J, b->d_J, (size_t)n_obs * 144, hipMemcpyDeviceToHost, s));
    CKC(hipStreamSynchronize(s));
    return PMV_OK;
}

}

int pmv::ba_check(pmv_ctx* ctx, const double* cams, int nc, const double* pts, int np, const double* obs_xy, const int* cam_idx, const int* pt_idx,
                  int n_obs, const double* K, double huber_delta, int max_iterations) {
    REQ(ctx && cams && pts && obs_xy && cam_idx && pt_idx && K, PMV_ERR_INVALID, "pmv_ba_solve: null argument");
    REQ(nc >= 1 && nc <= ctx->max_ba_cams && np >= 1 && np <= ctx->max_ba_points && n_obs >= 1 && n_obs <= ctx->max_ba_obs, PMV_ERR_CAPACITY,
        "pmv_ba_solve: nc=%d np=%d n_obs=%d exceed capacity %d/%d/%d", nc, np, n_obs, ctx->max_ba_cams, ctx->max_ba_points, ctx->max_ba_obs);
    REQ(max_iterations >= 0 && max_iterations <= BA_MAX_ITERATIONS && huber_delta > 0, PMV_ERR_INVALID, "pmv_ba_solve: bad options");
    for (int i = 0; i < n_obs; i++)
        REQ(cam_idx[i] >= 0 && cam_idx[i] < nc && pt_idx[i] >= 0 && pt_idx[i] < np, PMV_ERR_INVALID, "pmv_ba_solve: index out of range at observation %d", i);
    const int m = 6 * nc;
    REQ(((size_t)(m + 1) * m + (size_t)m) * 8 <= 150 * 1024, PMV_ERR_CAPACITY, "pmv_ba_solve: %d cameras exceed the LDS-resident reduced system (max 22)", nc);
    return PMV_OK;
}
int pmv::ba_prepare(pmv_ctx* ctx, BackendBuffers* b, const double* cams, int nc, const double* pts, int np, const double* obs_xy, const int* cam_idx,
                    const int* pt_idx, int n_obs, const double* K, double huber_delta, int max_iterations, bool multi, BAArgs* Aout, BaIoLayout* Lout) {
    const BaIoLayout L = ba_io_layout((size_t)nc, (size_t)np, (size_t)n_obs);
    REQ(L.total <= b->d_ba_io.cap && L.total <= b->h_stage.cap, PMV_ERR_CAPACITY, "pmv_ba_solve: io block too small");
    char* hs = (char*)b->h_stage;
    double* h_cams = (double*)(hs + L.cams); double* h_pts = (double*)(hs + L.pts); double* h_obs = (double*)(hs + L.obs); double* h_K = (double*)(hs + L.K);
    int* h_ci = (int*)(hs + L.cam_idx); int* h_pi = (int*)(hs + L.pt_idx);
    int* pstart = (int*)(hs + L.pstart); int* plist = (int*)(hs + L.plist); int* cstart = (int*)(hs + L.cstart); int* clist = (int*)(hs + L.clist);
    int* odup = (int*)(hs + L.erec);
    memcpy(h_cams, cams, (size_t)nc * 48); memcpy(h_pts, pts, (size_t)np * 24); memcpy(h_obs, obs_xy, (size_t)n_obs * 16);
    memcpy(h_K, K, 72); memcpy(h_ci, cam_idx, (size_t)n_obs * 4); memcpy(h_pi, pt_idx, (size_t)n_obs * 4);
    std::fill(pstart, pstart + np + 1, 0);
    std::fill(cstart, cstart + nc + 1, 0);
    for (int i = 0; i < n_obs; i++) { pstart[pt_idx[i] + 1]++; cstart[cam_idx[i] + 1]++; }
    for (int p = 0; p < np; p++) pstart[p + 1] += pstart[p];
    for (int c = 0; c < nc; c++) cstart[c + 1] += cstart[c];
    {
        std::vector<int> pf(pstart, pstart + np), cf(cstart, cstart + nc);
        for (int i = 0; i < n_obs; i++) { plist[pf[pt_idx[i]]++] = i; clist[cf[cam_idx[i]]++] = i; }
    }
    for (int p = 0; p < np; p++) {
        for (int e = pstart[p]; e < pstart[p + 1]; e++) {
            const int c = cam_idx[plist[e]];
            bool earlier = false, later = false;
            for (int e2 = pstart[p]; e2 < e; e2++) earlier = earlier || cam_idx[plist[e2]] == c;
            for (int e2 = e + 1; e2 < pstart[p + 1]; e2++) later = later || cam_idx[plist[e2]] == c;
            odup[4 * e] = plist[e]; odup[4 * e + 1] = c; odup[4 * e + 2] = p; odup[4 * e + 3] = earlier ? 2 : (later ? 1 : 0);
        }
    }
    const int m = 6 * nc;
    const int tiles_r = (m + 15) / 16, tiles_c = (m + 1 + 15) / 16;
    char* dio = b->d_ba_io;
    BAArgs A;
    A.cams = (double*)(dio + L.cams); A.pts = (double*)(dio + L.pts); A.obs = (const double*)(dio + L.obs); A.K = (const double*)(dio + L.K);
    A.cam_idx = (const int*)(dio + L.cam_idx); A.pt_idx = (const int*)(dio + L.pt_idx);
    A.pobs_start = (const int*)(dio + L.pstart); A.pobs_list = (const int*)(dio + L.plist); A.cobs_start = (const int*)(dio + L.cstart); A.cobs_list = (const int*)(dio + L.clist);
    A.erec = (const int4*)(dio + L.erec);
    A.nc = nc; A.np = np; A.nobs = n_obs; A.max_iterations = max_iterations; A.huber = huber_delta;
    A.x = b->d_x; A.cand = b->d_cand; A.scale = b->d_scale; A.diag = b->d_diag; A.D2 = b->d_D2; A.step = b->d_step; A.res = b->d_res; A.J = b->d_J;
    A.Einv = b->d_Einv; A.gp = b->d_gp; A.Yd = b->d_Yd; A.Wd = b->d_Wd; A.S = b->d_S; A.rhs = b->d_rhs; A.Gpart = b->d_Gpart; A.summary = (double*)(dio + L.summary);
    A.stamps = stamps_on() ? b->d_stamps : nullptr;
    A.out = nullptr;
    A.done_seq = 0;
    A.tiles_r = tiles_r; A.tiles_c = tiles_c;
    A.ldw = A.tiles_c * 16;
    A.krows = round_up(3 * np, 16);
    A.gp_rows = A.tiles_r * 16;
    int ks = 8 / (A.tiles_r * A.tiles_c);
    if (ks < 1) ks = 1;
    if (ks > 8) ks = 8;
    if (multi) ks = 8;
    A.kper = round_up((A.krows + ks - 1) / ks, 16);
    A.kslices = (A.krows + A.kper - 1) / A.kper;
    REQ((size_t)A.krows * A.ldw <= b->ydwd_elems && (size_t)A.kslices * A.gp_rows * A.ldw <= b->gpart_elems, PMV_ERR_CAPACITY, "pmv_ba_solve: workspace too small");
    if (multi) {
        A.Wd = A.Yd + (size_t)A.krows * A.ldw;
        A.out = (double*)b->h_stage.dm();
    }
    *Aout = A;
    *Lout = L;
    return PMV_OK;
}
void pmv::ba_finish(pmv_ctx* ctx, BackendBuffers* b, double* cams, int nc, double* pts, int np, const double* obs_xy, const int* cam_idx,
                    const int* pt_idx, int n_obs, const double* K, double huber_delta, int max_iterations, const BaIoLayout& L, pmv_ba_summary* summary) {
    const char* hs = (const char*)b->h_stage;
    const double* h_out = (const double*)(hs + L.summary);
    const double* h_cams = (const double*)(hs + L.cams);
    static const bool ba_trace = getenv("PMV_BA_TRACE") != nullptr;
    if (ba_trace) {
        fprintf(stderr, "[ba-trace] nc=%d np=%d nobs=%d cost %.15g -> %.15g it %d ok %d\n", nc, np, n_obs, h_out[0], h_out[1], (int)h_out[2], (int)h_out[3]);
        for (int c : {0, nc - 1}) {
            fprintf(stderr, "[ba-trace]   cam %d in ", c);
            for (int k = 0; k < 6; k++) fprintf(stderr, " %.15g", cams[6 * c + k]);
            fprintf(stderr, "\n[ba-trace]   cam %d out", c);
            for (int k = 0; k < 6; k++) fprintf(stderr, " %.15g", h_cams[6 * c + k]);
            fprintf(stderr, "\n");
        }
    }
    if (ctx->log.on) {
        std::lock_guard<std::mutex> lk(ctx->log.mu);
        ctx->log.blobs.emplace_back();
        std::vector<char>& bl = ctx->log.blobs.back();
        const int hdr[5] = {1, nc, np, n_obs, max_iterations};
        pmv_call_log::put(bl, hdr, 20); pmv_call_log::put(bl, cams, (size_t)nc * 48); pmv_call_log::put(bl, pts, (size_t)np * 24);
        pmv_call_log::put(bl, obs_xy, (size_t)n_obs * 16); pmv_call_log::put(bl, K, 72); pmv_call_log::put(bl, &huber_delta, 8);
        pmv_call_log::put(bl, cam_idx, (size_t)n_obs * 4); pmv_call_log::put(bl, pt_idx, (size_t)n_obs * 4);
        pmv_call_log::put(bl, h_cams, L.out_bytes - L.cams); pmv_call_log::put(bl, h_out, 40);
    }
    memcpy(cams, h_cams, (size_t)nc * 48);
    memcpy(pts, hs + L.pts, (size_t)np * 24);
    if (summary) {
        summary->initial_cost = h_out[0]; summary->final_cost = h_out[1]; summary->iterations = (int)h_out[2];
        summary->successful_steps = (int)h_out[3]; summary->termination = (int)h_out[4];
    }
}

extern "C" {

int pmv_set_ba_mode(pmv_ctx* ctx, int mode) {
    if (!ctx || (mode != 0 && mode != 1)) { set_err(ctx, "pmv_set_ba_mode: mode must be 0 (launch chain) or 1 (one workgroup per solve)"); return PMV_ERR_INVALID; }
    ctx->ba_mode = mode;
    return PMV_OK;
}

int pmv_ba_solve(pmv_ctx* ctx, double* cams, int nc, double* pts, int np, const double* obs_xy, const int* cam_idx, const int* pt_idx,
                 int n_obs, const double* K, double huber_delta, int max_iterations, pmv_ba_summary* summary) {
    int rc = ba_check(ctx, cams, nc, pts, np, obs_xy, cam_idx, pt_idx, n_obs, K, huber_delta, max_iterations);
    if (rc) return rc;
    if (max_iterations == 0) {
        if (summary) { summary->initial_cost = summary->final_cost = 0.0; summary->iterations = 0; summary->successful_steps = 0; summary->termination = 0; }
        return PMV_OK;
    }
    tl_prof = &ctx->prof;
    CKC(hipSetDevice(ctx->device));
    BackendBuffers* b = ctx->be;
    hipStream_t s = ctx->s_back;
    static const int mode = [] { const char* e = getenv("PMV_BA_MODE"); if (getenv("PMV_BA_SINGLE")) return 0;
                                 return (e && !strcmp(e, "single")) ? 0 : 1; }();
    const bool single = mode == 0 || ctx->ba_mode == 1;
    BAArgs A;
    BaIoLayout L;
    rc = ba_prepare(ctx, b, cams, nc, pts, np, obs_xy, cam_idx, pt_idx, n_obs, K, huber_delta, max_iterations, !single, &A, &L);
    if (rc) return rc;
    const size_t io_bytes = L.io_bytes;
    char* hs = (char*)b->h_stage;
    static const bool check = getenv("PMV_BA_CHECK") != nullptr;
    const bool flag_wait = back_wait_by_word() && !single && !check;
    volatile unsigned* done_word = (volatile unsigned*)(hs + L.done);
    if (flag_wait) {
        if (++b->done_seq == 0) b->done_seq = 1;
        *(double*)(hs + L.done) = 0.0;
        A.done_seq = b->done_seq;
    }
    if (stage_by_kernel() && !check) CKC(stage_block(s, b->h_stage.dm(), b->d_ba_io, io_bytes, 64));
    else CKC(hipMemcpyAsync(b->d_ba_io, hs, io_bytes, hipMemcpyHostToDevice, s));
    std::vector<char> saved;
    if (check) saved.assign(hs, hs + io_bytes);
    if (single) CKC(launch_ba_lm(s, A));
    else CKC(launch_ba_multi(s, A, b->d_bastate, b->d_bapart));
    const size_t out_bytes = L.out_bytes;
    if (single) CKC(hipMemcpyAsync(hs, b->d_ba_io, out_bytes, hipMemcpyDeviceToHost, s));
    if ((rc = wait_done_word(ctx, s, done_word, b->done_seq, flag_wait))) return rc;
    const double* h_out = (const double*)hs;
    if (!single && check) {
        std::vector<double> got(h_out, h_out + out_bytes / 8);
        CKC(hipMemcpyAsync(b->d_ba_io, saved.data(), io_bytes, hipMemcpyHostToDevice, s));
        A.Wd = b->d_Wd;
        CKC(launch_ba_lm(s, A));
        CKC(hipMemcpyAsync(hs, b->d_ba_io, out_bytes, hipMemcpyDeviceToHost, s));
        CKC(hipStreamSynchronize(s));
        double dmax = 0;
        for (size_t i = BA_SUM_SLOTS; i < out_bytes / 8; i++) dmax = std::max(dmax, fabs(got[i] - h_out[i]));
        fprintf(stderr, "[ba-check] nc=%d np=%d nobs=%d multi: cost %.12g -> %.12g it %d ok %d term %d | single: %.12g -> %.12g it %d ok %d term %d | max|dx| %.3e\n",
                nc, np, n_obs, got[0], got[1], (int)got[2], (int)got[3], (int)got[4], h_out[0], h_out[1], (int)h_out[2], (int)h_out[3],
                (int)h_out[4], dmax);
        {
            std::vector<double> base(h_out, h_out + out_bytes / 8);
            std::vector<char> pert(saved);
            double* pc = (double*)(pert.data() + L.cams);
            for (int i = 0; i < 6 * nc; i++) pc[i] += 1e-9 * ((i * 2654435761u >> 7) % 3 - 1.0);
            CKC(hipMemcpyAsync(b->d_ba_io, pert.data(), io_bytes, hipMemcpyHostToDevice, s));
            CKC(launch_ba_lm(s, A));
            CKC(hipMemcpyAsync(hs, b->d_ba_io, out_bytes, hipMemcpyDeviceToHost, s));
            CKC(hipStreamSynchronize(s));
            double d2 = 0;
            for (size_t i = BA_SUM_SLOTS; i < out_bytes / 8; i++) d2 = std::max(d2, fabs(base[i] - h_out[i]));
            fprintf(stderr, "[ba-check]    input perturbed by 1e-9 -> single-kernel output moves by %.3e\n", d2);
        }
        memcpy(hs, got.data(), out_bytes);
    }
    ba_finish(ctx, b, cams, nc, pts, np, obs_xy, cam_idx, pt_idx, n_obs, K, huber_delta, max_iterations, L, summary);
    return PMV_OK;
}

}

int pmv::fivepoint_prepare(pmv_ctx* ctx, BackendBuffers* b, const double* q1, const double* q2, int n, const int* samples, int n_hyp, float thr,
                           FivePointProblem* P, FivePointLayout* Lout) {
    REQ(q1 && q2 && samples && n >= 5 && n <= ctx->max_tracks && n_hyp >= 1 && n_hyp <= FP_MAX_HYP, PMV_ERR_INVALID,
        "five-point round: n=%d (5..max_tracks=%d), n_hyp=%d (1..%d)", n, ctx->max_tracks, n_hyp, FP_MAX_HYP);
    const FivePointLayout L = fivepoint_layout((size_t)n, (size_t)n_hyp);
    REQ(L.in_bytes <= b->d_tri_in.cap && L.total <= b->h_stage.cap, PMV_ERR_CAPACITY, "five-point round: input block too small");
    char* hs = (char*)b->h_stage;
    memcpy(hs + L.q1, q1, (size_t)n * 16); memcpy(hs + L.q2, q2, (size_t)n * 16); memcpy(hs + L.samples, samples, (size_t)5 * n_hyp * 4);
    P->q1 = (const double*)(b->d_tri_in + L.q1);
    P->q2 = (const double*)(b->d_tri_in + L.q2);
    P->samples = (const int*)(b->d_tri_in + L.samples);
    P->models_d = (double*)b->d_fp_work;
    P->n_models_d = (int*)(b->d_fp_work + (size_t)FP_MAX_HYP * 90 * 8);
    char* dh = b->h_stage.dm();
    P->models_h = (double*)(dh + L.models);
    P->n_models_h = (int*)(dh + L.n_models);
    P->counts_h = (int*)(dh + L.counts);
    P->n = n; P->n_hyp = n_hyp; P->thr = thr;
    memset(hs + L.n_models, 0, L.total - L.n_models);
    *Lout = L;
    return PMV_OK;
}
void pmv::fivepoint_finish(BackendBuffers* b, int n_hyp, const FivePointLayout& L, double* models, int* n_models, int* counts) {
    const char* hs = (const char*)b->h_stage;
    memcpy(models, hs + L.models, (size_t)n_hyp * 90 * 8);
    memcpy(n_models, hs + L.n_models, (size_t)n_hyp * 4);
    memcpy(counts, hs + L.counts, (size_t)n_hyp * 40);
}

int pmv::dlt_prepare(pmv_ctx* ctx, BackendBuffers* b, const double* q1, const double* q2, int n, const double* P1x4, const uint8_t* mask_in, DltProblem* P,
                     DltLayout* Lout) {
    const DltLayout L = dlt_layout((size_t)n);
    REQ(L.in_bytes <= b->d_tri_in.cap && L.total <= b->h_stage.cap, PMV_ERR_CAPACITY, "pmv_triangulate_candidates: n=%d does not fit the staging blocks", n);
    char* hs = (char*)b->h_stage;
    memcpy(hs + L.P, P1x4, 48 * 8); memcpy(hs + L.q1, q1, (size_t)n * 16); memcpy(hs + L.q2, q2, (size_t)n * 16); memcpy(hs + L.mask_in, mask_in, (size_t)n);
    P->P1x4 = (const double*)(b->d_tri_in + L.P);
    P->q1 = (const double*)(b->d_tri_in + L.q1);
    P->q2 = (const double*)(b->d_tri_in + L.q2);
    P->mask_in = (const uint8_t*)(b->d_tri_in + L.mask_in);
    P->Q = (double*)(b->h_stage.dm() + L.Q);
    P->mask = (uint8_t*)(b->h_stage.dm() + L.mask);
    P->n = n;
    *Lout = L;
    return PMV_OK;
}
void pmv::dlt_finish(pmv_ctx* ctx, BackendBuffers* b, const double* q1, const double* q2, int n, const double* P1x4, const uint8_t* mask_in,
                     const DltLayout& L, double* out_Q, uint8_t* out_mask, int* out_good) {
    const char* hs = (const char*)b->h_stage;
    memcpy(out_Q, hs + L.Q, (size_t)16 * n * 8);
    memcpy(out_mask, hs + L.mask, (size_t)4 * n);
    for (int c = 0; c < 4; c++) {
        int g = 0;
        for (int i = 0; i < n; i++) g += out_mask[(size_t)c * n + i];
        out_good[c] = g;
    }
    if (ctx->log.on) {
        std::lock_guard<std::mutex> lk(ctx->log.mu);
        ctx->log.blobs.emplace_back();
        std::vector<char>& bl = ctx->log.blobs.back();
        const int hdr[2] = {2, n};
        pmv_call_log::put(bl, hdr, 8); pmv_call_log::put(bl, q1, (size_t)n * 16); pmv_call_log::put(bl, q2, (size_t)n * 16); pmv_call_log::put(bl, P1x4, 384);
        pmv_call_log::put(bl, mask_in, (size_t)n); pmv_call_log::put(bl, out_Q, (size_t)n * 128); pmv_call_log::put(bl, out_mask, (size_t)n * 4);
        pmv_call_log::put(bl, out_good, 16);
    }
}

extern "C" {

int pmv_fivepoint_hypotheses(pmv_ctx* ctx, const double* q1, const double* q2, int n, const int* samples, int n_hyp, float thr, double* models,
                             int* n_models, int* counts) {
    REQ(ctx && models && n_models && counts, PMV_ERR_INVALID, "pmv_fivepoint_hypotheses: null argument");
    tl_prof = &ctx->prof;
    CKC(hipSetDevice(ctx->device));
    BackendBuffers* b = ctx->be;
    hipStream_t s = ctx->s_back;
// ... 226 lines not shown
```

### practical-multi-view_amd/csrc/backend_ba.hip

```cpp
#include "pmv_ctx.h"
#include <algorithm>
#include "backend.h"
#include "pmv_prof.h"
#include <float.h>

namespace pmv {

typedef double v4d __attribute__((ext_vector_type(4)));

constexpr int BA_T = 512;
constexpr int BA_NW = BA_T / 64;


__device__ inline void angle_axis_rotate(const double a[3], const double q[3], double p[3], double dpdw[9], double Rm[9], bool jac) {
    const double theta2 = a[0] * a[0] + a[1] * a[1] + a[2] * a[2];
    if (theta2 > DBL_EPSILON) {
        const double theta = sqrt(theta2);
        const double ct = cos(theta), st = sin(theta), ti = 1.0 / theta;
        const double w[3] = {a[0] * ti, a[1] * ti, a[2] * ti};
        const double wxq[3] = {w[1] * q[2] - w[2] * q[1], w[2] * q[0] - w[0] * q[2], w[0] * q[1] - w[1] * q[0]};
        const double wq = w[0] * q[0] + w[1] * q[1] + w[2] * q[2];
        const double tmp = wq * (1.0 - ct);
#pragma unroll
        for (int i = 0; i < 3; i++) p[i] = q[i] * ct + wxq[i] * st + w[i] * tmp;
// ... 1420 lines not shown
        __syncthreads();
        if (threadIdx.x == 0) __hip_atomic_store((unsigned*)(A.out + BA_SUM_DONE), A.done_seq, __ATOMIC_RELEASE, __HIP_MEMORY_SCOPE_SYSTEM);
    }
}

__global__ __launch_bounds__(BM_T) void k_bam_finish(BAArgs A, const BAGState* st_in, const double* part4, int nbp) { BACKEND_PRIO();
    bam_finish_role(A, st_in, part4, nbp);
}

hipError_t launch_ba_multi(hipStream_t s, const BAArgs& A, void* d_state, double* d_part) {
    BAGState* st2[2] = {(BAGState*)d_state, (BAGState*)((char*)d_state + 256)};
    int* chol_flags = (int*)((char*)d_state + 512);
    static_assert(sizeof(BAGState) <= 256, "BAGState");
    const int nbo = (A.nobs + BM_T - 1) / BM_T, nbp = (A.np + BM_PB - 1) / BM_PB, m = 6 * A.nc;
    double* part_cost = d_part;
    double* part_gmax = part_cost + nbo;
    double* part4 = part_gmax + nbp;
    double* Ublk = part4 + 4 * nbp;
    double* rhsblk = Ublk + 36 * A.nc;
    double* candrot = rhsblk + 6 * A.nc;
    double* tmp3 = candrot + 16 * A.nc;
    const size_t shm = ((size_t)(m + 1) * m + (size_t)m) * sizeof(double);
    if (A.max_iterations > BA_MAX_ITERATIONS) return hipErrorInvalidValue;
    ProfScope ps(K_BA_LM, s);
    const int tiles = A.tiles_r * A.tiles_c;
    const int clear_blocks = (int)std::min<size_t>(64, ((size_t)A.krows * A.ldw + 4 * BM_T - 1) / (4 * BM_T));
    { ProfScope p_(K_BAM_EVAL0, s);
    hipLaunchKernelGGL(k_bam_eval0, dim3(nbo + clear_blocks), dim3(BM_T), 0, s, A, st2[1], chol_flags, part_cost, nbo); }
    for (int it = 0; it < A.max_iterations; it++) {
        BAGState* sin = st2[it & 1];
        BAGState* sc = st2[(it + 1) & 1];
        int* cf = chol_flags + it;
        if (it == 0) {
            ProfScope p_(K_BAM_CAMPOINT, s);
            hipLaunchKernelGGL(k_bam_campoint, dim3(A.nc), dim3(BM_T), 0, s, A, sc, sc, 0, part4, nbp, cf, A.nc, Ublk, rhsblk, part_gmax);
            hipLaunchKernelGGL(k_bam_campoint, dim3(nbp), dim3(BM_T), 0, s, A, sc, sc, 0, part4, nbp, cf, 0, Ublk, rhsblk, part_gmax);
        } else {
            ProfScope p_(K_BAM_CAMPOINT, s);
            hipLaunchKernelGGL(k_bam_campoint, dim3(A.nc + nbp), dim3(BM_T), 0, s, A, sin, sc, 1, part4, nbp, cf, A.nc, Ublk, rhsblk, part_gmax);
        }
        { ProfScope p_(K_BAM_GEMM, s);
        hipLaunchKernelGGL(k_bam_gemm, dim3(tiles * BG_H), dim3(64 * BG_W), 0, s, A, sc); }
        { ProfScope p_(K_BAM_SOLVE, s);
        hipLaunchKernelGGL(k_bam_solve, dim3(1), dim3(BM_T), shm, s, A, sc, cf, part_cost, nbo, part_gmax, nbp, Ublk, rhsblk, candrot); }
        { ProfScope p_(K_BAM_BACKSUB, s);
        hipLaunchKernelGGL(k_bam_backsub, dim3(nbp), dim3(BM_T), 0, s, A, sc, candrot, tmp3, part4); }
    }
    { ProfScope p_(K_BAM_FINISH, s);
    hipLaunchKernelGGL(k_bam_finish, dim3(1), dim3(BM_T), 0, s, A, st2[A.max_iterations & 1], part4, nbp); }
    return hipGetLastError();
}

void ba_fill_prob(BAProb& P, const BAArgs& A, void* d_state, double* d_part) {
    P.A = A;
    P.st2[0] = d_state; P.st2[1] = (char*)d_state + 256;
    P.chol_flags = (int*)((char*)d_state + 512);
    P.nbo = (A.nobs + BM_T - 1) / BM_T; P.nbp = (A.np + BM_PB - 1) / BM_PB;
    P.part_cost = d_part; P.part_gmax = P.part_cost + P.nbo; P.part4 = P.part_gmax + P.nbp; P.Ublk = P.part4 + 4 * P.nbp;
    P.rhsblk = P.Ublk + 36 * A.nc; P.candrot = P.rhsblk + 6 * A.nc; P.tmp3 = P.candrot + 16 * A.nc;
    P.clear_blocks = (int)std::min<size_t>(64, ((size_t)A.krows * A.ldw + 4 * BM_T - 1) / (4 * BM_T));
    P.tiles = A.tiles_r * A.tiles_c;
}
__global__ __launch_bounds__(BM_T) void k_bamB_eval0(const BAProb* __restrict__ probs) { BACKEND_PRIO();
    const BAProb& P = probs[blockIdx.y];
    const BAArgs A = P.A;
    const int bx = blockIdx.x;
    if (bx < P.nbo) { bam_eval0_role(A, (BAGState*)P.st2[1], P.chol_flags, P.part_cost, bx, P.nbo); return; }
    const int zb = bx - P.nbo, nzb = P.clear_blocks;
    if (zb >= nzb) return;
    const size_t n2 = (size_t)A.krows * A.ldw;
    double2* z = (double2*)A.Yd;
    for (size_t i = (size_t)zb * BM_T + threadIdx.x; i < n2; i += (size_t)nzb * BM_T) z[i] = double2{0.0, 0.0};
}
__global__ __launch_bounds__(BM_T) void k_bamB_campoint(const BAProb* __restrict__ probs, int it, int part) { BACKEND_PRIO();
    __shared__ double swork[BM_WORK];
    const BAProb& P = probs[blockIdx.y];
    const BAArgs A = P.A;
    BAGState* sin = (BAGState*)P.st2[it & 1];
    BAGState* sc = (BAGState*)P.st2[(it + 1) & 1];
    int* cf = P.chol_flags + it;
    const int bx = blockIdx.x;
    if (part == 0) { if (bx >= A.nc) return; bam_campoint_role(A, sc, sc, false, P.part4, P.nbp, cf, A.nc, P.Ublk, P.rhsblk, P.part_gmax, bx, swork); }
    else if (part == 1) { if (bx >= P.nbp) return; bam_campoint_role(A, sc, sc, false, P.part4, P.nbp, cf, 0, P.Ublk, P.rhsblk, P.part_gmax, bx, swork); }
    else { if (bx >= A.nc + P.nbp) return; bam_campoint_role(A, sin, sc, true, P.part4, P.nbp, cf, A.nc, P.Ublk, P.rhsblk, P.part_gmax, bx, swork); }
}
__global__ __launch_bounds__(64 * BG_W) void k_bamB_gemm(const BAProb* __restrict__ probs, int it) { BACKEND_PRIO();
    __shared__ double swork[BG_W * 4 * 64];
    const BAProb& P = probs[blockIdx.y];
    if ((int)blockIdx.x >= P.tiles * BG_H) return;
    const BAArgs A = P.A;
    bam_gemm_role(A, (const BAGState*)P.st2[(it + 1) & 1], blockIdx.x, swork);
}
__global__ __launch_bounds__(BM_T) void k_bamB_solve(const BAProb* __restrict__ probs, int it) { BACKEND_PRIO();
    const BAProb& P = probs[blockIdx.x];
    const BAArgs A = P.A;
    bam_solve_role(A, (BAGState*)P.st2[(it + 1) & 1], P.chol_flags + it, P.part_cost, P.nbo, P.part_gmax, P.nbp, P.Ublk, P.rhsblk, P.candrot);
}
__global__ __launch_bounds__(BM_T) void k_bamB_backsub(const BAProb* __restrict__ probs, int it) { BACKEND_PRIO();
    const BAProb& P = probs[blockIdx.y];
    if ((int)blockIdx.x >= P.nbp) return;
    const BAArgs A = P.A;
    bam_backsub_role(A, (const BAGState*)P.st2[(it + 1) & 1], P.candrot, P.tmp3, P.part4, blockIdx.x);
}
__global__ __launch_bounds__(BM_T) void k_bamB_finish(const BAProb* __restrict__ probs, int max_it) { BACKEND_PRIO();
    const BAProb& P = probs[blockIdx.x];
    const BAArgs A = P.A;
    bam_finish_role(A, (const BAGState*)P.st2[max_it & 1], P.part4, P.nbp);
}
hipError_t launch_ba_multi_batch(hipStream_t s, const BAProb* d_probs, const BABatchDims& D) {
    if (D.n_probs <= 0) return hipSuccess;
    if (!d_probs || D.max_iterations < 1 || D.max_iterations > BA_MAX_ITERATIONS) return hipErrorInvalidValue;
    const size_t shm = ((size_t)(D.max_m + 1) * D.max_m + (size_t)D.max_m) * sizeof(double);
    if (shm > 150 * 1024) return hipErrorInvalidValue;
    const unsigned np = (unsigned)D.n_probs;
    ProfScope ps(K_BA_LM, s);
    hipLaunchKernelGGL(k_bamB_eval0, dim3(D.max_eval_blocks, np), dim3(BM_T), 0, s, d_probs);
    for (int it = 0; it < D.max_iterations; it++) {
        if (it == 0) {
            hipLaunchKernelGGL(k_bamB_campoint, dim3(D.max_nc, np), dim3(BM_T), 0, s, d_probs, it, 0);
            hipLaunchKernelGGL(k_bamB_campoint, dim3(D.max_nbp, np), dim3(BM_T), 0, s, d_probs, it, 1);
        } else
            hipLaunchKernelGGL(k_bamB_campoint, dim3(D.max_nc + D.max_nbp, np), dim3(BM_T), 0, s, d_probs, it, 2);
        hipLaunchKernelGGL(k_bamB_gemm, dim3(D.max_tiles * BG_H, np), dim3(64 * BG_W), 0, s, d_probs, it);
        hipLaunchKernelGGL(k_bamB_solve, dim3(np), dim3(BM_T), shm, s, d_probs, it);
        hipLaunchKernelGGL(k_bamB_backsub, dim3(D.max_nbp, np), dim3(BM_T), 0, s, d_probs, it);
    }
    hipLaunchKernelGGL(k_bamB_finish, dim3(np), dim3(BM_T), 0, s, d_probs, D.max_iterations);
    return hipGetLastError();
}

hipError_t launch_ba_residuals(hipStream_t s, const double* cams, const double* pts, const double* obs, const int* cam_idx,
                               const int* pt_idx, int nobs, const double* K, double* out_r, double* out_J) {
    if (nobs <= 0) return hipSuccess;
    ProfScope ps(K_BA_RESID, s);
    hipLaunchKernelGGL(k_ba_residuals, dim3((nobs + 255) / 256), dim3(256), 0, s, cams, pts, obs, cam_idx, pt_idx, nobs, K, out_r, out_J);
    return hipGetLastError();
}
hipError_t launch_ba_lm_batch(hipStream_t s, const BAArgs* d_args, int n_probs, int max_m) {
    if (!d_args || n_probs < 1 || max_m < 6) return hipErrorInvalidValue;
    const size_t shm = ((size_t)(max_m + 1) * max_m + (size_t)max_m) * sizeof(double);
    ProfScope ps(K_BA_LM, s);
    hipLaunchKernelGGL(k_ba_lm_batch, dim3(n_probs), dim3(BA_T), shm, s, d_args);
    return hipGetLastError();
}
hipError_t launch_ba_lm(hipStream_t s, const BAArgs& A) {
    const int m = 6 * A.nc;
    const size_t shm = ((size_t)(m + 1) * m + (size_t)m) * sizeof(double);
    ProfScope ps(K_BA_LM, s);
    hipLaunchKernelGGL(k_ba_lm, dim3(1), dim3(BA_T), shm, s, A);
    return hipGetLastError();
}

hipError_t backend_prepare_device() {
    hipError_t e = hipFuncSetAttribute((const void*)k_bam_solve, hipFuncAttributeMaxDynamicSharedMemorySize, 150 * 1024);
    if (e != hipSuccess) return e;
    e = hipFuncSetAttribute((const void*)k_bamB_solve, hipFuncAttributeMaxDynamicSharedMemorySize, 150 * 1024);
    if (e != hipSuccess) return e;
    e = hipFuncSetAttribute((const void*)k_ba_lm_batch, hipFuncAttributeMaxDynamicSharedMemorySize, 150 * 1024);
    if (e != hipSuccess) return e;
    return hipFuncSetAttribute((const void*)k_ba_lm, hipFuncAttributeMaxDynamicSharedMemorySize, 150 * 1024);
}

}
```

### practical-multi-view_amd/csrc/backend_pnp.hip

```cpp
#include "pmv_ctx.h"
#include "backend.h"
#include "pmv_prof.h"
#include "pmv_dense.h"
#include <float.h>

namespace pmv {

#define WAVE_SYNC_PNP() asm volatile("s_waitcnt lgkmcnt(0)" ::: "memory")

struct EpnpShared {
    double A[144], V[144];
    double M[10 * 12];
    double pws[15], us[10], alphas[20], cws[12];
    double v4[48];
    double L[60], rho[6];
    double case_err[3], case_R[27], case_t[9];
};

__device__ inline void epnp_qr_solve(double* A, double* b, double* X) {
    constexpr int nr = 6, nc = 4;
    double A1[4], A2[4];
#pragma unroll
    for (int k = 0; k < nc; k++) {
        double eta = fabs(A[k * nc + k]);
#pragma unroll
        for (int i = k + 1; i < nr; i++) {
            const double elt = fabs(A[(i - 1) * nc + k]);
            if (eta < elt) eta = elt;
        }
        if (eta == 0) { X[0] = X[1] = X[2] = X[3] = 0.0; return; }
        double sum2 = 0.0;
        const double inv_eta = 1. / eta;
#pragma unroll
        for (int i = k; i < nr; i++) { A[i * nc + k] *= inv_eta; sum2 += A[i * nc + k] * A[i * nc + k]; }
        double sigma = sqrt(sum2);
        if (A[k * nc + k] < 0) sigma = -sigma;
        A[k * nc + k] += sigma;
        A1[k] = sigma * A[k * nc + k];
        A2[k] = -eta * sigma;
#pragma unroll
        for (int j = k + 1; j < nc; j++) {
            double sum = 0;
#pragma unroll
            for (int i = k; i < nr; i++) sum += A[i * nc + k] * A[i * nc + j];
            const double tau = sum / A1[k];
#pragma unroll
            for (int i = k; i < nr; i++) A[i * nc + j] -= tau * A[i * nc + k];
        }
    }
#pragma unroll
    for (int j = 0; j < nc; j++) {
        double tau = 0;
#pragma unroll
        for (int i = j; i < nr; i++) tau += A[i * nc + j] * b[i];
        tau /= A1[j];
#pragma unroll
        for (int i = j; i < nr; i++) b[i] -= tau * A[i * nc + j];
    }
    X[nc - 1] = b[nc - 1] / A2[nc - 1];
#pragma unroll
    for (int i = nc - 2; i >= 0; i--) {
        double sum = 0;
#pragma unroll
        for (int j = i + 1; j < nc; j++) sum += A[i * nc + j] * X[j];
        X[i] = (b[i] - sum) / A2[i];
    }
}

__device__ inline void epnp_gauss_newton(const double* L, const double* rho, double* betas) {
    for (int k = 0; k < 5; k++) {
        double A[24], b[6], x[4];
#pragma unroll
        for (int i = 0; i < 6; i++) {
            const double* rowL = L + i * 10;
            double* rowA = A + i * 4;
            rowA[0] = 2 * rowL[0] * betas[0] + rowL[1] * betas[1] + rowL[3] * betas[2] + rowL[6] * betas[3];
            rowA[1] = rowL[1] * betas[0] + 2 * rowL[2] * betas[1] + rowL[4] * betas[2] + rowL[7] * betas[3];
            rowA[2] = rowL[3] * betas[0] + rowL[4] * betas[1] + 2 * rowL[5] * betas[2] + rowL[8] * betas[3];
            rowA[3] = rowL[6] * betas[0] + rowL[7] * betas[1] + rowL[8] * betas[2] + 2 * rowL[9] * betas[3];
            b[i] = rho[i] - (rowL[0] * betas[0] * betas[0] + rowL[1] * betas[0] * betas[1] + rowL[2] * betas[1] * betas[1] +
                             rowL[3] * betas[0] * betas[2] + rowL[4] * betas[1] * betas[2] + rowL[5] * betas[2] * betas[2] +
                             rowL[6] * betas[0] * betas[3] + rowL[7] * betas[1] * betas[3] + rowL[8] * betas[2] * betas[3] +
                             rowL[9] * betas[3] * betas[3]);
        }
        epnp_qr_solve(A, b, x);
        for (int i = 0; i < 4; i++) betas[i] += x[i];
    }
}

__device__ double epnp_R_and_t(const EpnpShared& sh, const double* betas, double fu, double fv, double uc, double vc,
                               double R[9], double t[3]) {
    const int n = 5;
    double ccs[12], pcs[15];
    for (int i = 0; i < 12; i++) ccs[i] = 0.0;
    for (int i = 0; i < 4; i++) {
        const double* v = sh.v4 + 12 * i;
        for (int j = 0; j < 4; j++)
            for (int k = 0; k < 3; k++) ccs[j * 3 + k] += betas[i] * v[3 * j + k];
    }
    for (int i = 0; i < n; i++) {
        const double* a = &sh.alphas[4 * i];
        for (int j = 0; j < 3; j++) pcs[3 * i + j] = a[0] * ccs[j] + a[1] * ccs[3 + j] + a[2] * ccs[6 + j] + a[3] * ccs[9 + j];
    }
    if (pcs[2] < 0.0) {
        for (int i = 0; i < 12; i++) ccs[i] = -ccs[i];
        for (int i = 0; i < 15; i++) pcs[i] = -pcs[i];
    }
    double pc0[3] = {0, 0, 0}, pw0[3] = {0, 0, 0};
    for (int i = 0; i < n; i++)
        for (int j = 0; j < 3; j++) { pc0[j] += pcs[3 * i + j]; pw0[j] += sh.pws[3 * i + j]; }
    for (int j = 0; j < 3; j++) { pc0[j] /= n; pw0[j] /= n; }
    double abt[9] = {0, 0, 0, 0, 0, 0, 0, 0, 0};
    for (int i = 0; i < n; i++) {
        const double* pc = &pcs[3 * i];
        const double* pw = &sh.pws[3 * i];
        for (int j = 0; j < 3; j++) {
            abt[3 * j] += (pc[j] - pc0[j]) * (pw[0] - pw0[0]);
            abt[3 * j + 1] += (pc[j] - pc0[j]) * (pw[1] - pw0[1]);
            abt[3 * j + 2] += (pc[j] - pc0[j]) * (pw[2] - pw0[2]);
        }
    }
    double U[9], s[3], V[9];
    d_svd3(abt, U, s, V);
    for (int i = 0; i < 3; i++)
        for (int j = 0; j < 3; j++) R[i * 3 + j] = U[i * 3] * V[j * 3] + U[i * 3 + 1] * V[j * 3 + 1] + U[i * 3 + 2] * V[j * 3 + 2];
    const double det = R[0] * R[4] * R[8] + R[1] * R[5] * R[6] + R[2] * R[3] * R[7] - R[2] * R[4] * R[6] - R[1] * R[3] * R[8] - R[0] * R[5] * R[7];
    if (det < 0) { R[6] = -R[6]; R[7] = -R[7]; R[8] = -R[8]; }
    t[0] = pc0[0] - d_dot3(R, pw0);
    t[1] = pc0[1] - d_dot3(R + 3, pw0);
    t[2] = pc0[2] - d_dot3(R + 6, pw0);
    double sum2 = 0.0;
    for (int i = 0; i < n; i++) {
        const double* pw = &sh.pws[3 * i];
        const double Xc = d_dot3(R, pw) + t[0], Yc = d_dot3(R + 3, pw) + t[1], inv_Zc = 1.0 / (d_dot3(R + 6, pw) + t[2]);
        const double ue = uc + fu * Xc * inv_Zc, ve = vc + fv * Yc * inv_Zc;
        const double u = sh.us[2 * i], v = sh.us[2 * i + 1];
        sum2 += sqrt((u - ue) * (u - ue) + (v - ve) * (v - ve));
    }
    return sum2 / n;
}

__device__ __forceinline__ bool d_jacobi_rotation(double apq, double app, double aqq, double tol_abs, double& c_out, double& s_out) {
    const double theta = (aqq - app) / (2.0 * apq);
    const double t = (theta >= 0 ? 1.0 : -1.0) / (fabs(theta) + sqrt(theta * theta + 1.0));
    const double c = 1.0 / sqrt(t * t + 1.0);
    const double s = t * c;
    const bool rot = !(fabs(apq) <= tol_abs);
    c_out = rot ? c : 1.0;
    s_out = rot ? s : 0.0;
    return rot;
}

template <bool LDS_L>
__device__ __forceinline__ void pnp_hyp_body(const float* __restrict__ obj, const float* __restrict__ img,
                                             const int* __restrict__ samples, const double* __restrict__ K,
                                             double* __restrict__ models, int m, float thr, uint8_t* __restrict__ masks,
                                             int* __restrict__ counts, unsigned long long* stamps, const int h) {
    __shared__ EpnpShared sh;
    __shared__ double sR[9], sT[3];
    const int lane = threadIdx.x;
    unsigned long long t_prev = __builtin_readcyclecounter();
#define HSTAMP(k) do { if (stamps && h == 0 && lane == 0) { const unsigned long long t_ = __builtin_readcyclecounter(); stamps[k] += t_ - t_prev; t_prev = t_; } } while (0)
    const double fu = K[0], fv = K[4], uc = K[2], vc = K[5];
    const int n = 5;
    if (lane < n) {
        const double ifx = 1. / fu, ify = 1. / fv;
        const int i = lane;
        const int s = samples[h * 5 + i];
        sh.pws[3 * i] = obj[3 * s]; sh.pws[3 * i + 1] = obj[3 * s + 1]; sh.pws[3 * i + 2] = obj[3 * s + 2];
        const float xn = (float)(((double)img[2 * s] - uc) * ifx);
        const float yn = (float)(((double)img[2 * s + 1] - vc) * ify);
        sh.us[2 * i] = xn * fu + uc;
        sh.us[2 * i + 1] = yn * fv + vc;
    }
    WAVE_SYNC_PNP();
    if (lane == 0) {
        double* cws = sh.cws;
        cws[0] = cws[1] = cws[2] = 0;
        for (int i = 0; i < n; i++)
            for (int j = 0; j < 3; j++) cws[j] += sh.pws[3 * i + j];
        for (int j = 0; j < 3; j++) cws[j] /= n;
        double C[9], w[3], V[9];
        for (int a = 0; a < 3; a++)
            for (int b = 0; b < 3; b++) {
                double acc = 0;
                for (int i = 0; i < n; i++) acc += (sh.pws[3 * i + a] - cws[a]) * (sh.pws[3 * i + b] - cws[b]);
                C[a * 3 + b] = acc;
            }
        d_jacobi_eig<3>(C, w, V);
        for (int i = 1; i < 4; i++) {
            const int src = 3 - i;
            const double k = sqrt((w[src] > 0 ? w[src] : 0.0) / n);
            for (int j = 0; j < 3; j++) cws[3 * i + j] = cws[j] + k * V[j * 3 + src];
        }
        double cc[9], U[9], s3[3], V3[9], ci[9];
        for (int i = 0; i < 3; i++)
            for (int j = 1; j < 4; j++) cc[3 * i + j - 1] = cws[3 * j + i] - cws[i];
        d_svd3(cc, U, s3, V3);
        const double thr = 2 * DBL_EPSILON * (s3[0] + s3[1] + s3[2]);
        for (int i = 0; i < 3; i++)
            for (int j = 0; j < 3; j++) {
                double acc = 0;
                for (int k = 0; k < 3; k++)
                    if (s3[k] > thr) acc += V3[i * 3 + k] * U[j * 3 + k] / s3[k];
                ci[i * 3 + j] = acc;
            }
        for (int i = 0; i < n; i++) {
            const double* pi = &sh.pws[3 * i];
            double* a = &sh.alphas[4 * i];
            for (int j = 0; j < 3; j++)
                a[1 + j] = ci[3 * j] * (pi[0] - cws[0]) + ci[3 * j + 1] * (pi[1] - cws[1]) + ci[3 * j + 2] * (pi[2] - cws[2]);
            a[0] = 1.0f - a[1] - a[2] - a[3];
        }
        for (int i = 0; i < n; i++) {
            const double* as = &sh.alphas[4 * i];
            double* M1 = &sh.M[(2 * i) * 12];
            double* M2 = M1 + 12;
            const double u = sh.us[2 * i], v = sh.us[2 * i + 1];
            for (int k = 0; k < 4; k++) {
                M1[3 * k] = as[k] * fu; M1[3 * k + 1] = 0.0; M1[3 * k + 2] = as[k] * (uc - u);
                M2[3 * k] = 0.0; M2[3 * k + 1] = as[k] * fv; M2[3 * k + 2] = as[k] * (vc - v);
            }
        }
    }
    __syncthreads();
    HSTAMP(22);
    for (int idx = lane; idx < 144; idx += 64) {
        const int a = idx / 12, b = idx - a * 12;
        const int lo = a < b ? a : b, hi = a < b ? b : a;
        double acc = 0;
        for (int r = 0; r < 2 * n; r++) acc += sh.M[r * 12 + lo] * sh.M[r * 12 + hi];
        sh.A[idx] = acc;
        sh.V[idx] = (a == b) ? 1.0 : 0.0;
    }
    __syncthreads();
    double tol_abs = 0;
    for (int i = 0; i < 12; i++) tol_abs += fabs(sh.A[i * 13]);
    tol_abs *= 1e-17;
    const int jg = lane / 6, jg2 = lane - jg * 6;
    unsigned sched[6] = {0u, 0u, 0u, 0u, 0u, 0u};
#pragma unroll
    for (int r = 0; r < 11; r++) {
        int a = 11, b = r, a2 = 11, b2 = r;
        if (jg != 0) { a = (r + jg) % 11; b = (r - jg + 11) % 11; }
        if (jg2 != 0) { a2 = (r + jg2) % 11; b2 = (r - jg2 + 11) % 11; }
        const int p = a < b ? a : b, q = a < b ? b : a, p2 = a2 < b2 ? a2 : b2, q2 = a2 < b2 ? b2 : a2;
        sched[r >> 1] |= (unsigned)((p & 15) | ((q & 15) << 4) | (p2 << 8) | (q2 << 12)) << ((r & 1) * 16);
    }
    const unsigned long long t_jac0 = __builtin_readcyclecounter();
    int n_rounds = 0;
    for (int sweep = 0; sweep < 30; sweep++) {
        int rotated = 0;
#pragma unroll
        for (int r = 0; r < 11; r++) {
            const unsigned w = sched[r >> 1] >> ((r & 1) * 16);
            const int p = w & 15, q = (w >> 4) & 15, p2 = (w >> 8) & 15, q2 = (w >> 12) & 15;
            bool rot2 = false;
            double c2 = 1.0, sn2 = 0.0;
            double app = 0, apq = 0, aqp = 0, aqq = 0, v0p = 0, v0q = 0, v1p = 0, v1q = 0;
            if (lane < 36) {
                const double hpq = sh.A[p2 * 12 + q2], hpp = sh.A[p2 * 12 + p2], hqq = sh.A[q2 * 12 + q2];
                app = sh.A[p * 12 + p2]; apq = sh.A[p * 12 + q2]; aqp = sh.A[q * 12 + p2]; aqq = sh.A[q * 12 + q2];
                v0p = sh.V[jg * 12 + p2]; v0q = sh.V[jg * 12 + q2]; v1p = sh.V[(jg + 6) * 12 + p2]; v1q = sh.V[(jg + 6) * 12 + q2];
                rot2 = d_jacobi_rotation(hpq, hpp, hqq, tol_abs, c2, sn2);
            }
            const int nrot = __popcll(__ballot(rot2 && lane < 6));
            rotated += nrot;
            n_rounds++;
            if (nrot == 0) continue;
            const double c = __shfl(c2, jg), sn = __shfl(sn2, jg);
            if (lane < 36) {
                const double bpp = c2 * app - sn2 * apq, bpq = sn2 * app + c2 * apq;
                const double bqp = c2 * aqp - sn2 * aqq, bqq = sn2 * aqp + c2 * aqq;
                sh.A[p * 12 + p2] = c * bpp - sn * bqp;
                sh.A[q * 12 + p2] = sn * bpp + c * bqp;
                sh.A[p * 12 + q2] = c * bpq - sn * bqq;
                sh.A[q * 12 + q2] = sn * bpq + c * bqq;
                sh.V[jg * 12 + p2] = c2 * v0p - sn2 * v0q;
                sh.V[jg * 12 + q2] = sn2 * v0p + c2 * v0q;
                sh.V[(jg + 6) * 12 + p2] = c2 * v1p - sn2 * v1q;
                sh.V[(jg + 6) * 12 + q2] = sn2 * v1p + c2 * v1q;
            }
            WAVE_SYNC_PNP();
        }
        if (!rotated) break;
    }
    if (stamps && h == 0 && lane == 0) { stamps[19] += __builtin_readcyclecounter() - t_jac0; stamps[20] += n_rounds; }
    HSTAMP(23);
    if (lane == 0) {
        double w[12];
        int ord[12];
        for (int i = 0; i < 12; i++) { w[i] = sh.A[i * 12 + i]; ord[i] = i; }
        for (int i = 0; i < 11; i++) {
            int m = i;
            for (int j = i + 1; j < 12; j++) if (w[j] < w[m]) m = j;
            if (m != i) { double t = w[i]; w[i] = w[m]; w[m] = t; int o = ord[i]; ord[i] = ord[m]; ord[m] = o; }
        }
        for (int i = 0; i < 4; i++)
            for (int k = 0; k < 12; k++) sh.v4[i * 12 + k] = sh.V[k * 12 + ord[i]];
        const double* cws = sh.cws;
        double* rho = sh.rho;
        rho[0] = d_dist2(cws, cws + 3); rho[1] = d_dist2(cws, cws + 6); rho[2] = d_dist2(cws, cws + 9);
        rho[3] = d_dist2(cws + 3, cws + 6); rho[4] = d_dist2(cws + 3, cws + 9); rho[5] = d_dist2(cws + 6, cws + 9);
    }
    WAVE_SYNC_PNP();
    if (lane < 60) {
        const int i = lane / 10, k = lane - i * 10;
        const int pa = (i < 3) ? 0 : ((i < 5) ? 1 : 2), pb = (i < 3) ? i + 1 : ((i < 5) ? i - 1 : 3);
        const int u = (k == 0 || k == 1 || k == 3 || k == 6) ? 0 : ((k == 2 || k == 4 || k == 7) ? 1 : ((k == 5 || k == 8) ? 2 : 3));
        const int w = (k == 0) ? 0 : ((k == 1 || k == 2) ? 1 : ((k == 3 || k == 4 || k == 5) ? 2 : 3));
        const double* vu = sh.v4 + 12 * u;
        const double* vw = sh.v4 + 12 * w;
        const double du[3] = {vu[3 * pa] - vu[3 * pb], vu[3 * pa + 1] - vu[3 * pb + 1], vu[3 * pa + 2] - vu[3 * pb + 2]};
        const double dw[3] = {vw[3 * pa] - vw[3 * pb], vw[3 * pa + 1] - vw[3 * pb + 1], vw[3 * pa + 2] - vw[3 * pb + 2]};
        const double d = d_dot3(du, dw);
        sh.L[i * 10 + k] = (u == w) ? d : 2.0f * d;
    }
    __syncthreads();
    HSTAMP(24);
    if (lane < 3) {
        const int N = lane + 1;
        double Lr[LDS_L ? 1 : 60], rhor[LDS_L ? 1 : 6], betas[4];
        if (!LDS_L) {
            for (int i = 0; i < 60; i++) Lr[i] = sh.L[i];
            for (int i = 0; i < 6; i++) rhor[i] = sh.rho[i];
        }
        const double* L = LDS_L ? sh.L : Lr;
        const double* rho = LDS_L ? sh.rho : rhor;
        double l5[30], b5[5];
        {
            const int c0 = 0, c1 = 1, c2 = (N == 1) ? 3 : 2, c3 = (N == 1) ? 6 : ((N == 3) ? 3 : -1), c4 = (N == 3) ? 4 : -1;
#pragma unroll
            for (int i = 0; i < 6; i++) {
                l5[i * 5 + 0] = sh.L[i * 10 + c0];
                l5[i * 5 + 1] = sh.L[i * 10 + c1];
                l5[i * 5 + 2] = sh.L[i * 10 + c2];
                l5[i * 5 + 3] = (c3 >= 0) ? sh.L[i * 10 + (c3 >= 0 ? c3 : 0)] : 0.0;
                l5[i * 5 + 4] = (c4 >= 0) ? sh.L[i * 10 + (c4 >= 0 ? c4 : 0)] : 0.0;
            }
        }
        d_pinv_solve<6, 5>(l5, rho, b5);
        if (N == 1) {
            if (b5[0] < 0) { betas[0] = sqrt(-b5[0]); betas[1] = -b5[1] / betas[0]; betas[2] = -b5[2] / betas[0]; betas[3] = -b5[3] / betas[0]; }
            else { betas[0] = sqrt(b5[0]); betas[1] = b5[1] / betas[0]; betas[2] = b5[2] / betas[0]; betas[3] = b5[3] / betas[0]; }
        } else if (N == 2) {
            if (b5[0] < 0) { betas[0] = sqrt(-b5[0]); betas[1] = (b5[2] < 0) ? sqrt(-b5[2]) : 0.0; }
            else { betas[0] = sqrt(b5[0]); betas[1] = (b5[2] > 0) ? sqrt(b5[2]) : 0.0; }
            if (b5[1] < 0) betas[0] = -betas[0];
            betas[2] = 0.0; betas[3] = 0.0;
        } else {
            if (b5[0] < 0) { betas[0] = sqrt(-b5[0]); betas[1] = (b5[2] < 0) ? sqrt(-b5[2]) : 0.0; }
            else { betas[0] = sqrt(b5[0]); betas[1] = (b5[2] > 0) ? sqrt(b5[2]) : 0.0; }
            if (b5[1] < 0) betas[0] = -betas[0];
            betas[2] = b5[3] / betas[0];
            betas[3] = 0.0;
        }
        HSTAMP(25);
        epnp_gauss_newton(L, rho, betas);
        HSTAMP(26);
        double R[9], t[3];
        sh.case_err[lane] = epnp_R_and_t(sh, betas, fu, fv, uc, vc, R, t);
        for (int i = 0; i < 9; i++) sh.case_R[lane * 9 + i] = R[i];
        for (int i = 0; i < 3; i++) sh.case_t[lane * 3 + i] = t[i];
    }
    __syncthreads();
    HSTAMP(27);
    if (lane == 0) {
        int N = 0;
        if (sh.case_err[1] < sh.case_err[0]) N = 1;
        if (sh.case_err[2] < sh.case_err[N]) N = 2;
        double rv[3];
        d_rodrigues_m2v(sh.case_R + 9 * N, rv);
        for (int i = 0; i < 3; i++) { models[h * 6 + i] = rv[i]; models[h * 6 + 3 + i] = sh.case_t[N * 3 + i]; sT[i] = sh.case_t[N * 3 + i]; }
        d_rodrigues_v2m(rv, sR);
    }
    __syncthreads();
    HSTAMP(28);
    {
        const double t0 = sT[0], t1 = sT[1], t2 = sT[2];
        int good = 0;
        for (int i = lane; i < m; i += 64) {
            const double X = obj[3 * i], Y = obj[3 * i + 1], Z = obj[3 * i + 2];
            double x = sR[0] * X + sR[1] * Y + sR[2] * Z + t0;
            double y = sR[3] * X + sR[4] * Y + sR[5] * Z + t1;
            double z = sR[6] * X + sR[7] * Y + sR[8] * Z + t2;
            z = z ? 1. / z : 1;
            x *= z; y *= z;
            const float px = (float)(x * fu + uc), py = (float)(y * fv + vc);
            const float dx = img[2 * i] - px, dy = img[2 * i + 1] - py;
            const float e = dx * dx + dy * dy;
            const int f = e <= thr;
            masks[(size_t)h * m + i] = (uint8_t)f;
            good += f;
        }
#pragma unroll
        for (int o = 32; o > 0; o >>= 1) good += __shfl_xor(good, o, 64);
        if (lane == 0) counts[h] = good;
    }
    HSTAMP(29);
#undef HSTAMP
}

__device__ inline int d_ransac_update_num_iters(double p, double ep, int modelPoints, int maxIters) {
    p = fmax(p, 0.); p = fmin(p, 1.);
    ep = fmax(ep, 0.); ep = fmin(ep, 1.);
    double num = fmax(1. - p, DBL_MIN);
    double denom = 1. - pow(1. - ep, (double)modelPoints);
    if (denom < DBL_MIN) return 0;
    num = log(num);
    denom = log(denom);
    return denom >= 0 || -num >= maxIters * (-denom) ? maxIters : (int)rint(num / denom);
}

__device__ inline void d_angle_axis_rotate_jac(const double a[3], const double q[3], double p[3], double dpdw[9]) {
    const double theta2 = a[0] * a[0] + a[1] * a[1] + a[2] * a[2];
    if (theta2 > DBL_EPSILON) {
        const double theta = sqrt(theta2);
        const double ct = cos(theta), st = sin(theta), ti = 1.0 / theta;
        const double w[3] = {a[0] * ti, a[1] * ti, a[2] * ti};
        const double wxq[3] = {w[1] * q[2] - w[2] * q[1], w[2] * q[0] - w[0] * q[2], w[0] * q[1] - w[1] * q[0]};
        const double wq = w[0] * q[0] + w[1] * q[1] + w[2] * q[2];
        const double tmp = wq * (1.0 - ct);
        for (int i = 0; i < 3; i++) p[i] = q[i] * ct + wxq[i] * st + w[i] * tmp;
        if (!dpdw) return;
        for (int k = 0; k < 3; k++) {
            double dwk[3];
            for (int i = 0; i < 3; i++) dwk[i] = ((i == k ? 1.0 : 0.0) - w[i] * w[k]) * ti;
            const double dwxq[3] = {dwk[1] * q[2] - dwk[2] * q[1], dwk[2] * q[0] - dwk[0] * q[2], dwk[0] * q[1] - dwk[1] * q[0]};
            const double dwq = dwk[0] * q[0] + dwk[1] * q[1] + dwk[2] * q[2];
            const double dct = -st * w[k], dst = ct * w[k];
            const double dtmp = dwq * (1.0 - ct) + wq * (st * w[k]);
            for (int i = 0; i < 3; i++) dpdw[i * 3 + k] = q[i] * dct + dwxq[i] * st + wxq[i] * dst + dwk[i] * tmp + w[i] * dtmp;
        }
    } else {
        const double wxq[3] = {a[1] * q[2] - a[2] * q[1], a[2] * q[0] - a[0] * q[2], a[0] * q[1] - a[1] * q[0]};
        for (int i = 0; i < 3; i++) p[i] = q[i] + wxq[i];
        if (!dpdw) return;
        dpdw[0] = 0;     dpdw[1] = q[2];  dpdw[2] = -q[1];
        dpdw[3] = -q[2]; dpdw[4] = 0;     dpdw[5] = q[0];
        dpdw[6] = q[1];  dpdw[7] = -q[0]; dpdw[8] = 0;
    }
}

constexpr int RF_T = 256;
struct RefitShared {
    double tile[28 * (256 + 8)];
    double part[28 * 8];
    double red[4 * 28];
    double JtJ[36], JtErr[6], param[6], prev[6];
    double err2, prevErr2;
    int best, last, n_in, state, lambdaLg10, iters, done;
    int wsum[4];
};

constexpr int RF_ROW = RF_T + 8;
__device__ inline void block_sum28(const double* acc, RefitShared& sh) {
    const int tid = threadIdx.x;
#pragma unroll
    for (int k = 0; k < 28; k++) sh.tile[k * RF_ROW + tid] = acc[k];
    __syncthreads();
    if (tid < 28 * 8) {
        const int k = tid >> 3, part = tid & 7;
        const double* src = &sh.tile[k * RF_ROW + part];
        double s0 = 0, s1 = 0, s2 = 0, s3 = 0;
#pragma unroll
        for (int j = 0; j < 32; j += 4) { s0 += src[8 * j]; s1 += src[8 * (j + 1)]; s2 += src[8 * (j + 2)]; s3 += src[8 * (j + 3)]; }
        sh.part[k * 8 + part] = (s0 + s1) + (s2 + s3);
    }
    __syncthreads();
    if (tid < 28) {
        double sacc = sh.part[tid * 8];
#pragma unroll
        for (int q = 1; q < 8; q++) sacc += sh.part[tid * 8 + q];
        sh.red[tid] = sacc;
    }
    __syncthreads();
}

__device__ __forceinline__ void pnp_select_refit_body(const float* __restrict__ obj, const float* __restrict__ img, int m,
                                                      const double* __restrict__ K, const double* __restrict__ models,
                                                      const uint8_t* __restrict__ masks, const int* __restrict__ counts,
                                                      int n_hyp, double confidence, double* __restrict__ rt_out,
                                                      int* __restrict__ inliers, int* __restrict__ info, char* __restrict__ host_out,
                                                      unsigned long long* stamps, const unsigned done_seq) {
    __shared__ RefitShared sh;
    const unsigned long long t_start = __builtin_readcyclecounter();
    unsigned long long t_lm0 = 0;
    int n_pass = 0;
    const int tid = threadIdx.x, lane = tid & 63, wid = tid >> 6;
    if (tid == 0) {
        int maxGood = 0, niters = n_hyp > 1 ? n_hyp : 1, best = -1, last = -1;
        for (int iter = 0; iter < niters && iter < n_hyp; iter++) {
            last = iter;
            const int good = counts[iter];
            if (good > (maxGood > 4 ? maxGood : 4)) {
                best = iter;
                maxGood = good;
                niters = d_ransac_update_num_iters(confidence, (double)(m - good) / m, 5, niters);
            }
        }
        sh.best = best; sh.last = last; sh.n_in = 0;
        info[1] = last + 1;
    }
    __syncthreads();
    if (sh.best < 0) {
        if (tid == 0) {
            info[0] = 0;
            const int l = sh.last < 0 ? 0 : sh.last;
            for (int i = 0; i < 6; i++) rt_out[i] = models[l * 6 + i];
            if (host_out) {
                for (int i = 0; i < 6; i++) ((double*)host_out)[i] = models[l * 6 + i];
                ((int*)(host_out + PNP_OUT_INFO))[0] = 0; ((int*)(host_out + PNP_OUT_INFO))[1] = sh.last + 1;
                if (done_seq) { __threadfence_system(); __hip_atomic_store((unsigned*)(host_out + PNP_OUT_DONE), done_seq, __ATOMIC_RELEASE, __HIP_MEMORY_SCOPE_SYSTEM); }
            }
        }
        return;
    }
    const uint8_t* mk = masks + (size_t)sh.best * m;
    int base = 0;
    for (int c0 = 0; c0 < m; c0 += RF_T) {
        const int i = c0 + tid;
        const int f = (i < m) ? mk[i] : 0;
        const unsigned long long bal = __ballot(f);
        const int before = __popcll(bal & ((1ull << lane) - 1ull));
        if (lane == 0) sh.wsum[wid] = __popcll(bal);
        __syncthreads();
        int off = base;
        for (int w = 0; w < wid; w++) off += sh.wsum[w];
        if (f) inliers[off + before] = i;
        const int tot = sh.wsum[0] + sh.wsum[1] + sh.wsum[2] + sh.wsum[3];
        __syncthreads();
        base += tot;
    }
    const int n = base;
    if (tid == 0) { sh.n_in = n; info[0] = n; }
    if (tid < 6) { sh.param[tid] = models[sh.last * 6 + tid]; }
    if (tid == 0) { sh.lambdaLg10 = -3; sh.iters = 0; sh.done = 0; sh.state = 0; }
    __syncthreads();
    const double fx = K[0], fy = K[4], cx = K[2], cy = K[5];
    constexpr int RF_KEEP = 2;
    double keepX[RF_KEEP][3], keepU[RF_KEEP][2];
#pragma unroll
    for (int q = 0; q < RF_KEEP; q++) {
        const int e = tid + q * RF_T;
        const int i = e < n ? inliers[e] : 0;
        keepX[q][0] = (double)obj[3 * i]; keepX[q][1] = (double)obj[3 * i + 1]; keepX[q][2] = (double)obj[3 * i + 2];
        keepU[q][0] = (double)img[2 * i]; keepU[q][1] = (double)img[2 * i + 1];
    }
    t_lm0 = __builtin_readcyclecounter();
    for (;;) {
        n_pass++;
        unsigned long long t_p = __builtin_readcyclecounter();
#define RSTAMP(k) do { if (stamps && tid == 0) { const unsigned long long t_ = __builtin_readcyclecounter(); stamps[k] += t_ - t_p; t_p = t_; } } while (0)
        double acc[28];
#pragma unroll
        for (int k = 0; k < 28; k++) acc[k] = 0;
        const double p0 = sh.param[0], p1 = sh.param[1], p2 = sh.param[2], p3 = sh.param[3], p4 = sh.param[4], p5 = sh.param[5];
        const double pa[3] = {p0, p1, p2};
        for (int e = tid, q = 0; e < n; e += RF_T, q++) {
            double X[3], U[2];
            if (q == 0) { X[0] = keepX[0][0]; X[1] = keepX[0][1]; X[2] = keepX[0][2]; U[0] = keepU[0][0]; U[1] = keepU[0][1]; }
            else if (q == 1) { X[0] = keepX[1][0]; X[1] = keepX[1][1]; X[2] = keepX[1][2]; U[0] = keepU[1][0]; U[1] = keepU[1][1]; }
            else {
                const int i = inliers[e];
                X[0] = (double)obj[3 * i]; X[1] = (double)obj[3 * i + 1]; X[2] = (double)obj[3 * i + 2];
                U[0] = (double)img[2 * i]; U[1] = (double)img[2 * i + 1];
            }
            double Xc[3], dpdw[9];
            d_angle_axis_rotate_jac(pa, X, Xc, dpdw);
            Xc[0] += p3; Xc[1] += p4; Xc[2] += p5;
            const double z = Xc[2] ? 1. / Xc[2] : 1;
            const double x = Xc[0] * z, y = Xc[1] * z;
            const double ex = x * fx + cx - U[0], ey = y * fy + cy - U[1];
            acc[27] += ex * ex + ey * ey;
            {
                double Ju[6], Jv[6];
                const double du[3] = {fx * z, 0, -fx * x * z}, dv[3] = {0, fy * z, -fy * y * z};
#pragma unroll
                for (int k = 0; k < 3; k++) {
                    Ju[k] = du[0] * dpdw[k] + du[1] * dpdw[3 + k] + du[2] * dpdw[6 + k];
                    Jv[k] = dv[0] * dpdw[k] + dv[1] * dpdw[3 + k] + dv[2] * dpdw[6 + k];
                    Ju[3 + k] = du[k];
                    Jv[3 + k] = dv[k];
                }
                int k = 0;
#pragma unroll
                for (int a = 0; a < 6; a++) {
#pragma unroll
                    for (int b = a; b < 6; b++) acc[k++] += Ju[a] * Ju[b] + Jv[a] * Jv[b];
                }
#pragma unroll
                for (int a = 0; a < 6; a++) acc[21 + a] += Ju[a] * ex + Jv[a] * ey;
            }
        }
        RSTAMP(10);
        block_sum28(acc, sh);
        RSTAMP(11);
        if (tid == 0) {
            const double err2 = sh.red[27];
            bool do_step = false, take_j = false;
            if (sh.state == 0) {
                if (sh.iters == 0) sh.prevErr2 = err2;
                take_j = do_step = true;
                sh.state = 1;
            } else {
                bool retry = false;
                if (err2 > sh.prevErr2) {
                    if (++sh.lambdaLg10 <= 16) { do_step = true; retry = true; }
                }
                if (!retry) {
                    sh.lambdaLg10 = sh.lambdaLg10 - 1 > -16 ? sh.lambdaLg10 - 1 : -16;
                    double dn = 0, pn = 0;
                    for (int i = 0; i < 6; i++) { dn += (sh.param[i] - sh.prev[i]) * (sh.param[i] - sh.prev[i]); pn += sh.prev[i] * sh.prev[i]; }
                    if (++sh.iters >= 20 || sqrt(dn) / sqrt(pn) < (double)FLT_EPSILON) sh.done = 1;
                    else { sh.prevErr2 = err2; take_j = do_step = true; }
                }
            }
            if (take_j) {
                int k = 0;
                for (int a = 0; a < 6; a++)
                    for (int b = a; b < 6; b++) { sh.JtJ[a * 6 + b] = sh.JtJ[b * 6 + a] = sh.red[k]; k++; }
                for (int a = 0; a < 6; a++) { sh.JtErr[a] = sh.red[21 + a]; sh.prev[a] = sh.param[a]; }
            }
            if (do_step) {
                const double lambda = K[10 + 16 + sh.lambdaLg10];
                double a[6][7];
#pragma unroll
                for (int i = 0; i < 6; i++) {
#pragma unroll
                    for (int k = 0; k < 6; k++) a[i][k] = sh.JtJ[i * 6 + k];
                    a[i][i] *= 1. + lambda;
                    a[i][6] = sh.JtErr[i];
                }
                bool ok = true;
#pragma unroll
                for (int c = 0; c < 6; c++) {
                    if (!ok) continue;
                    int piv = c;
                    double best = fabs(a[c][c]);
#pragma unroll
                    for (int q = c + 1; q < 6; q++) { const double v = fabs(a[q][c]); if (v > best) { best = v; piv = q; } }
                    if (best == 0.0) { ok = false; continue; }
#pragma unroll
                    for (int q = c + 1; q < 6; q++) {
                        if (piv == q) {
#pragma unroll
                            for (int k = 0; k < 7; k++) { const double t = a[c][k]; a[c][k] = a[q][k]; a[q][k] = t; }
                        }
                    }
#pragma unroll
                    for (int r = c + 1; r < 6; r++) {
                        const double f = a[r][c] / a[c][c];
                        if (f != 0.0) {
#pragma unroll
                            for (int k = c; k < 7; k++) a[r][k] -= f * a[c][k];
                        }
                    }
                }
                double bb[6] = {0, 0, 0, 0, 0, 0};
                if (ok) {
#pragma unroll
                    for (int q = 5; q >= 0; q--) {
                        double v = a[q][6];
#pragma unroll
                        for (int k = q + 1; k < 6; k++) v -= a[q][k] * bb[k];
                        bb[q] = v / a[q][q];
                    }
                }
#pragma unroll
                for (int i = 0; i < 6; i++) sh.param[i] = sh.prev[i] - bb[i];
            }
        }
        __syncthreads();
        RSTAMP(12);
        if (sh.done) break;
    }
#undef RSTAMP
    if (stamps && tid == 0) {
        const unsigned long long t_end = __builtin_readcyclecounter();
        stamps[30] += t_lm0 - t_start; stamps[31] += t_end - t_lm0; stamps[21] += n_pass;
    }
    if (tid < 6) rt_out[tid] = sh.param[tid];
    if (host_out) {
        if (tid < 6) ((double*)host_out)[tid] = sh.param[tid];
        if (tid == 0) { ((int*)(host_out + PNP_OUT_INFO))[0] = n; ((int*)(host_out + PNP_OUT_INFO))[1] = sh.last + 1; }
        int* hin = (int*)(host_out + PNP_OUT_INLIERS);
        for (int e = tid; e < n; e += RF_T) hin[e] = inliers[e];
        if (done_seq) {
            __threadfence_system();
            __syncthreads();
            if (tid == 0) __hip_atomic_store((unsigned*)(host_out + PNP_OUT_DONE), done_seq, __ATOMIC_RELEASE, __HIP_MEMORY_SCOPE_SYSTEM);
        }
    }
}

__global__ __launch_bounds__(64) void k_pnp_hyp(const float* __restrict__ obj, const float* __restrict__ img,
                                                const int* __restrict__ samples, const double* __restrict__ K,
                                                double* __restrict__ models, int m, float thr, uint8_t* __restrict__ masks,
                                                int* __restrict__ counts, unsigned long long* stamps) { BACKEND_PRIO();
    pnp_hyp_body<false>(obj, img, samples, K, models, m, thr, masks, counts, stamps, blockIdx.x);
}
__global__ __launch_bounds__(RF_T) void k_pnp_select_refit(const float* __restrict__ obj, const float* __restrict__ img, int m,
                                                           const double* __restrict__ K, const double* __restrict__ models,
                                                           const uint8_t* __restrict__ masks, const int* __restrict__ counts,
                                                           int n_hyp, double confidence, double* __restrict__ rt_out,
                                                           int* __restrict__ inliers, int* __restrict__ info, char* __restrict__ host_out,
                                                           unsigned long long* stamps, unsigned done_seq) { BACKEND_PRIO();
    pnp_select_refit_body(obj, img, m, K, models, masks, counts, n_hyp, confidence, rt_out, inliers, info, host_out, stamps, done_seq);
}
__global__ __launch_bounds__(64) __attribute__((amdgpu_waves_per_eu(2, 2))) void k_pnp_hyp_batch(const PnPProblem* __restrict__ probs, int h0, int replay) { BACKEND_PRIO();
    const PnPProblem p = probs[blockIdx.y];
    const int h = h0 + (int)blockIdx.x;
    if (h >= p.n_hyp) return;
    if (replay) {
        int maxGood = 0, niters = p.n_hyp > 1 ? p.n_hyp : 1;
        for (int iter = 0; iter < niters && iter < h0; iter++) {
            const int good = p.counts[iter];
            if (good > (maxGood > 4 ? maxGood : 4)) {
                maxGood = good;
                niters = d_ransac_update_num_iters(p.confidence, (double)(p.m - good) / p.m, 5, niters);
            }
        }
        if (niters <= h0) return;
    }
    pnp_hyp_body<true>(p.obj, p.img, p.samples, p.K, p.models, p.m, p.thr, p.masks, p.counts, nullptr, h);
}
__global__ __launch_bounds__(RF_T) void k_pnp_select_refit_batch(const PnPProblem* __restrict__ probs) { BACKEND_PRIO();
    const PnPProblem p = probs[blockIdx.x];
    pnp_select_refit_body(p.obj, p.img, p.m, p.K, p.models, p.masks, p.counts, p.n_hyp, p.confidence, p.rt_out, p.inliers, p.info, p.host_out, nullptr, 0u);
}

hipError_t launch_pnp_batch(hipStream_t s, const PnPProblem* d_probs, int n_probs, int max_hyp) {
    if (n_probs <= 0) return hipSuccess;
    if (!d_probs || max_hyp < 1) return hipErrorInvalidValue;
    static const int stage1 = getenv("PMV_PNP_STAGE1") ? atoi(getenv("PMV_PNP_STAGE1")) : 16;
    const int h0 = stage1 > 0 && stage1 < max_hyp ? stage1 : max_hyp;
    { ProfScope ps(K_PNP_HYP, s);
    hipLaunchKernelGGL(k_pnp_hyp_batch, dim3(h0, n_probs), dim3(64), 0, s, d_probs, 0, 0); }
    if (h0 < max_hyp) {
        ProfScope ps(K_PNP_HYP, s);
        hipLaunchKernelGGL(k_pnp_hyp_batch, dim3(max_hyp - h0, n_probs), dim3(64), 0, s, d_probs, h0, 1);
    }
    ProfScope ps3(K_PNP_REFIT, s);
    hipLaunchKernelGGL(k_pnp_select_refit_batch, dim3(n_probs), dim3(RF_T), 0, s, d_probs);
    return hipGetLastError();
}

hipError_t launch_pnp(hipStream_t s, const float* d_obj, const float* d_img, int m, const double* d_K, const int* d_samples,
                      int n_hyp, float thr, double confidence, double* d_models, uint8_t* d_masks, int* d_counts,
                      double* d_rt_out, int* d_inliers, int* d_info, char* host_out, unsigned long long* d_stamps, unsigned done_seq) {
    { ProfScope ps(K_PNP_HYP, s);
    hipLaunchKernelGGL(k_pnp_hyp, dim3(n_hyp), dim3(64), 0, s, d_obj, d_img, d_samples, d_K, d_models, m, thr, d_masks, d_counts, d_stamps); }
    ProfScope ps3(K_PNP_REFIT, s);
    hipLaunchKernelGGL(k_pnp_select_refit, dim3(1), dim3(RF_T), 0, s, d_obj, d_img, m, d_K, d_models, d_masks, d_counts, n_hyp,
                       confidence, d_rt_out, d_inliers, d_info, host_out, d_stamps, done_seq);
    return hipGetLastError();
}

}
```

### practical-multi-view_amd/csrc/pmv_ctx.h

```cpp
#pragma once
#include <atomic>
#include "pmv_device.h"
#include "pmv_mem.h"
#include "pmv_block.h"
#include "pmv_prof.h"
#include "../../include/pmv_hip.h"
#include <algorithm>
#include <utility>
#include <vector>
#include <mutex>

namespace pmv {
struct BatchEngine;
struct BatchSession;
struct BatchIngest;
enum SlotState : uint8_t { SLOT_EMPTY = 0, SLOT_STAGED, SLOT_BUILT };
constexpr int MAX_CELLS = 64;
constexpr int MAX_PER_CELL = 4096;
struct BackendBuffers;
}

struct pmv_call_log {
    bool on = false;
    std::mutex mu;
    std::vector<std::vector<char>> blobs;
    static void put(std::vector<char>& b, const void* p, size_t n) { const char* c = (const char*)p; b.insert(b.end(), c, c + n); }
};

struct pmv_ctx {
    int device = 0;
    int max_w = 0, max_h = 0, n_slots = 0, max_tracks = 0, max_ba_cams = 0, max_ba_points = 0, max_ba_obs = 0;
    hipStream_t s_front = nullptr, s_back = nullptr;
    pmv::PyrLayout cap;
    std::vector<pmv::PyrLayout> slot_layout;
    std::vector<uint8_t> slot_state;
    pmv::Buf<uint8_t> d_slots;
    static constexpr int MAX_GEOM = 256;
    std::vector<pmv::PyrLayout> geom;
    pmv::Buf<pmv::PyrLayout> d_geom;
    int geom_index(int w, int h) const { for (size_t i = 0; i < geom.size(); i++) if (geom[i].w[0] == w && geom[i].h[0] == h) return (int)i; return -1; }
    std::atomic<long long> batch_launches[4];
    std::atomic<long long> whole_rounds[3];
    static constexpr int TIGHT_FRAMES = 64;
    pmv::Buf<uint8_t> d_tight;
    pmv::Buf<float> d_prev_xy, d_out_xy, d_err;
    pmv::Buf<uint8_t> d_status;
    pmv::Buf<float> h_prev_xy, h_out_xy, h_err;
    pmv::Buf<uint8_t> h_status;
    pmv::Buf<int> h_knn, d_knn;
    pmv::Buf<unsigned long long> d_lk_stamps;
    pmv::Buf<uint16_t> h_work;
    pmv::Buf<uint8_t> h_lkx{pmv::MEM_MAPPED};
    std::atomic<unsigned long long> lk_work[3];
    void add_lk_work(const uint16_t* w, size_t n) { unsigned long long it = 0, lv = 0; for (size_t i = 0; i < n; i++) { it += w[i] & 0xffu; lv += w[i] >> 8; } lk_work[0] += it; lk_work[1] += lv; lk_work[2] += n; }
    pmv::Buf<int> d_cells;
    pmv::Buf<int> h_cells;
    pmv::Buf<double> d_eig;
    pmv::Buf<void> d_cellmax;
    pmv::Buf<unsigned> d_spill;
    pmv::Buf<int> d_det_xy, d_det_count, d_flags;
    pmv::Buf<double> d_det_score;
    pmv::Buf<int> h_det_xy, h_det_count;
    pmv::Buf<double> h_det_score;
    pmv::Buf<uint8_t> h_gmask{pmv::MEM_PINNED}, d_gmask;
    int gftt_general = 0;
    pmv::Buf<uint8_t> h_subpix{pmv::MEM_MAPPED};
    pmv::Buf<float> d_subpix_tab, h_subpix_tab{pmv::MEM_PINNED};
    int subpix_tab_key[4] = {0, 0, 0, 0};
    std::atomic<long long> subpix_launches[3];
    static constexpr int CLAHE_CHUNK = 64;
    pmv::Buf<uint8_t> h_clahe{pmv::MEM_PINNED}, d_clahe, d_clahe_lut;
    std::atomic<long long> clahe_launches[3];
    static constexpr int MAX_REMAP_MAPS = 16;
    struct RemapMap { int w = 0, h = 0; const uint8_t* d = nullptr; };
    RemapMap remap_maps[MAX_REMAP_MAPS];
    pmv::Buf<uint8_t> remap_mem[MAX_REMAP_MAPS];
    std::mutex remap_mu;
    static constexpr int REMAP_CHUNK = 64;
    pmv::Buf<uint8_t> h_remap{pmv::MEM_PINNED}, d_remap, d_remap_scratch;
    std::atomic<long long> remap_launches[3];
    pmv::BackendBuffers* be = nullptr;
    pmv::BackendBuffers* be_ahead = nullptr;
    hipStream_t s_ahead = nullptr;
    std::mutex ahead_mu;
    int ba_mode = 0;
    int frame_format = PMV_FRAMES_GRAY;
    pmv_frame_preproc preproc = {};
    std::atomic<long long> preproc_launches[4];
    pmv_lk_params lk = {pmv::LK_WIN, 4, 30, 0.01, 1e-4f};
    int lk_general = 0;
    std::atomic<int> batch_open{0};
    pmv::BatchEngine* engine = nullptr;
    std::mutex owner_mu;
    pmv::BatchSession* session = nullptr;
    std::atomic<int> session_state{0}, session_calls{0};
    pmv::BatchIngest* ingest = nullptr;
    pmv::BatchIngest* bingest = nullptr;
    double bingest_stats[PMV_BATCH_INGEST_STATS] = {};
    pmv::Profiler prof;
    pmv_call_log log;
    std::mutex err_mu;
    char err[512] = "";
};

namespace pmv {
void set_err(pmv_ctx* c, const char* fmt, ...);
const char* thread_error();
PyrLayout make_layout(int w, int h, int win, int max_level);
LKParams lk_launch_params(const pmv_ctx* ctx);
int backend_create(pmv_ctx* c);
void backend_destroy(pmv_ctx* c);
PyrLayout layout_for(pmv_ctx* ctx, int w, int h);
int geom_table_set(pmv_ctx* ctx, const int* w, const int* h, int B);
int slot_ready(pmv_ctx* ctx, int slot, BatchIngest* feed = nullptr, int seq = 0, hipStream_t s = nullptr, int* round = nullptr);
void batch_ingest_destroy(BatchIngest*& g);
void batch_engine_destroy(pmv_ctx* ctx);
void batch_session_destroy(pmv_ctx* ctx);
int lkx_check(pmv_ctx* ctx, const char* who, int flags, const float* next_xy, int n, bool fb, const float* back_xy, const uint8_t* back_status, const float* back_err);
int lk_check(pmv_ctx* ctx, bool bracket, int prev_slot, int next_slot, const float* prev_xy, int n, const float* out_xy, const uint8_t* out_status, const float* out_err);
int knn_check(pmv_ctx* ctx, bool bracket, int src_slot, int cmp_slot, const int* src_xy, int n, const int* cmp_xy, int m, int n_neighbours, int window, const int* out_best,
              const float* out_err);
int detect_check(pmv_ctx* ctx, bool bracket, int slot, const int* cells, int n_cells, int max_per_cell);
int gftt_ex_check(pmv_ctx* ctx, const char* who, const pmv_gftt_params* p, const int* out_xy, const int* out_count);
int gftt_mask_check(pmv_ctx* ctx, const char* who, int slot, const uint8_t* mask, int mask_stride);
size_t gftt_pack_mask(uint8_t* dst, size_t pos, int* cell_recs, const int* cells, int n_cells, const uint8_t* mask, int mask_stride);
int subpix_check(pmv_ctx* ctx, const char* who, bool bracket, int slot, const float* xy, int n, const pmv_subpix_params* p);
inline void subpix_zero_zone(const pmv_subpix_params* p, int* zw, int* zh) {
    const bool on = p->zero_w >= 0 && p->zero_h >= 0 && 2 * p->zero_w + 1 < 2 * p->win_w + 1 && 2 * p->zero_h + 1 < 2 * p->win_h + 1;
    *zw = on ? p->zero_w : -1; *zh = on ? p->zero_h : -1;
}
int clahe_check(pmv_ctx* ctx, const char* who, const pmv_clahe_params* p);
int remap_check(pmv_ctx* ctx, const char* who, int map_id, int border_value, pmv_ctx::RemapMap* map);
int fast_check(pmv_ctx* ctx, bool bracket, int slot, const int* cells, int n_cells, int max_per_cell, const int* out_xy, const float* out_response);
inline void lk_xcd_order(const float* prev_xy, int n, int* order) {
    static thread_local std::vector<std::pair<float, int>> byx;
    const int nb = (n + 7) / 8 * 8;
    byx.resize(n);
    for (int i = 0; i < n; i++) byx[i] = {prev_xy[2 * i], i};
    std::sort(byx.begin(), byx.end());
    for (int b = 0; b < nb; b++) order[b] = -1;
    for (int i = 0; i < n; i++) {
        const int s8 = (int)((long)i * 8 / n), first = (int)(((long)s8 * n + 7) / 8);
        order[(i - first) * 8 + s8] = byx[i].second;
    }
}
inline Carve carve_of(const Growable& g) { return Carve(g.p, g.dev, g.cap); }
struct SubpixBlock { Carved<SubpixRec> rec; Carved<float> xy; Carved<uint8_t> iters, flags; };
inline SubpixBlock subpix_block(Carve& c, size_t cap) { return {c.take<SubpixRec>(cap), c.take<float>(2 * cap), c.take<uint8_t>(cap), c.take<uint8_t>(cap)}; }
struct LkBackBlock { Carved<float> xy, err; Carved<uint8_t> status; };
inline LkBackBlock lk_back_block(Carve& c, size_t cap) { return {c.take<float>(2 * cap), c.take<float>(cap), c.take<uint8_t>(cap)}; }
hipError_t frontend_prepare_device();
hipError_t backend_prepare_device();
}
```

Before: 3618.

## Fuse PnP RANSAC hypothesis and refit kernels into one launch with flag handoff

Adds a fused PnP kernel where the first n_hyp workgroups compute EPnP hypotheses from inputs staged into LDS and publish inlier counts through per-hypothesis tagged flags. The final workgroup spins on those flags, runs the adaptive RANSAC selection as counts arrive, then does the LM refit from the LDS copy. This removes a second kernel launch and the inter-kernel gap, and lets the refit overlap with hypothesis evaluation. It relies on the refit block co-residing with the hypothesis blocks, adds a spin-wait with a timeout error path, and is the default via a new pnp_mode setting.

```diff
diff --git a/include/pmv_hip.h b/include/pmv_hip.h
--- a/include/pmv_hip.h
+++ b/include/pmv_hip.h
@@ -133,6 +133,7 @@
                      const int* cam_idx, const int* pt_idx, int n_obs, const double* K, double* out_r,
                      double* out_J);
 int pmv_set_ba_mode(pmv_ctx* ctx, int mode);
+int pmv_set_pnp_mode(pmv_ctx* ctx, int mode);
 int pmv_ba_solve(pmv_ctx* ctx, double* cams, int nc, double* pts, int np, const double* obs_xy, const int* cam_idx,
                  const int* pt_idx, int n_obs, const double* K, double huber_delta, int max_iterations,
                  pmv_ba_summary* summary);
diff --git a/practical-multi-view_amd/__init__.py b/practical-multi-view_amd/__init__.py
--- a/practical-multi-view_amd/__init__.py
+++ b/practical-multi-view_amd/__init__.py
@@ -171,7 +171,7 @@
     "pmv_remap_map_create", "pmv_remap_map_destroy", "pmv_frames_remap", "pmv_debug_remap_launches", "pmv_batch_frame_upload_remap", "pmv_undistort_map_build",
     "pmv_set_frame_preproc", "pmv_get_frame_preproc", "pmv_debug_preproc_launches",
     "pmv_debug_mem_live",
-    "pmv_lk_track", "pmv_lk_track_ex", "pmv_lk_track_fb", "pmv_set_lk_params", "pmv_get_lk_params", "pmv_debug_lk_general", "pmv_set_ba_mode", "pmv_pnp_ransac", "pmv_debug_pnp_hypotheses", "pmv_debug_ba_stamps", "pmv_debug_lk_stamps", "pmv_ba_residuals", "pmv_ba_solve", "pmv_triangulate_candidates", "pmv_triangulate_candidates_ahead", "pmv_fivepoint_hypotheses",
+    "pmv_lk_track", "pmv_lk_track_ex", "pmv_lk_track_fb", "pmv_set_lk_params", "pmv_get_lk_params", "pmv_debug_lk_general", "pmv_set_ba_mode", "pmv_set_pnp_mode", "pmv_pnp_ransac", "pmv_debug_pnp_hypotheses", "pmv_debug_ba_stamps", "pmv_debug_lk_stamps", "pmv_ba_residuals", "pmv_ba_solve", "pmv_triangulate_candidates", "pmv_triangulate_candidates_ahead", "pmv_fivepoint_hypotheses",
     "pmv_find_essential_mat", "pmv_recover_pose", "pmv_debug_essential_iters_table",
     "pmv_find_fundamental_mat", "pmv_debug_fundamental_iters_table", "pmv_debug_set_fundamental_r", "pmv_debug_fundamental_r", "pmv_debug_whole_rounds",
     "pmv_record_enable", "pmv_record_count", "pmv_record_size", "pmv_record_get",
@@ -776,6 +776,9 @@
                                            _p(r, _f64p), _p(J, _f64p)))
         return r, J
 
+    def set_pnp_mode(self, mode):
+        self._ck(self.lib.pmv_set_pnp_mode(self.h, int(mode)))
+
     def set_ba_mode(self, mode):
         self._ck(self.lib.pmv_set_ba_mode(self.h, int(mode)))
 
diff --git a/practical-multi-view_amd/csrc/backend.h b/practical-multi-view_amd/csrc/backend.h
--- a/practical-multi-view_amd/csrc/backend.h
+++ b/practical-multi-view_amd/csrc/backend.h
@@ -30,6 +30,7 @@
     Buf<int> d_samples, d_counts, d_inliers, d_info;
     Buf<double> d_models, d_rt, d_Kp;
     Buf<uint8_t> d_masks;
+    Buf<unsigned long long> d_pnp_flags;
 };
 
 struct BAArgs {
@@ -54,6 +55,13 @@
                       int n_hyp, float thr, double confidence, double* d_models, uint8_t* d_masks, int* d_counts,
                       double* d_rt_out, int* d_inliers, int* d_info, char* host_out ,
                       unsigned long long* d_stamps , unsigned done_seq = 0 );
+
+bool pnp_fused_fits(const float* d_obj, const float* d_img, int m, const double* d_K);
+hipError_t launch_pnp_fused(hipStream_t s, const float* d_obj, const float* d_img, int m, const double* d_K, const int* d_samples,
+                            int n_hyp, float thr, double confidence, double* d_models, uint8_t* d_masks, int* d_counts,
+                            double* d_rt_out, int* d_inliers, int* d_info, char* host_out, unsigned long long* d_stamps, unsigned done_seq,
+                            unsigned long long* d_flags, unsigned tag);
+hipError_t pnp_prepare_device();
 
 struct BAProb {
     BAArgs A;
diff --git a/practical-multi-view_amd/csrc/backend.hip b/practical-multi-view_amd/csrc/backend.hip
--- a/practical-multi-view_amd/csrc/backend.hip
+++ b/practical-multi-view_amd/csrc/backend.hip
@@ -54,7 +54,7 @@
         {&b->d_samples, MAX_HYP * 5 * 4, MEM_DEVICE}, {&b->d_counts, MAX_HYP * 4, MEM_DEVICE},
         {&b->d_inliers, mt * 4, MEM_DEVICE}, {&b->d_info, 16, MEM_DEVICE},
         {&b->d_models, MAX_HYP * 6 * 8, MEM_DEVICE}, {&b->d_rt, 6 * 8, MEM_DEVICE}, {&b->d_Kp, 9 * 8, MEM_DEVICE},
-        {&b->d_masks, (size_t)MAX_HYP * mt, MEM_DEVICE},
+        {&b->d_masks, (size_t)MAX_HYP * mt, MEM_DEVICE}, {&b->d_pnp_flags, MAX_HYP * 8, MEM_DEVICE},
         {&b->d_ba_io, caps.ba_io, MEM_DEVICE},
         {&b->d_pnp_in, caps.pnp_in, MEM_DEVICE}, {&b->d_pnp_out, caps.pnp_out, MEM_DEVICE},
         {&b->d_tri_in, caps.tri_in, MEM_DEVICE}, {&b->d_tri_out, caps.tri_out, MEM_DEVICE},
@@ -64,6 +64,7 @@
     };
     hipError_t e = mem_alloc_table(rows, sizeof(rows) / sizeof(rows[0]));
     if (e == hipSuccess) e = hipMemset(b->d_stamps, 0, 32 * 8);
+    if (e == hipSuccess) e = hipMemset(b->d_pnp_flags, 0, MAX_HYP * 8);
     if (e != hipSuccess) { set_err(c, "backend_alloc: %s", hipGetErrorString(e)); return PMV_ERR_HIP; }
     return PMV_OK;
 }
@@ -196,9 +197,14 @@
     volatile unsigned* done_word = (volatile unsigned*)((char*)b->h_stage + L.done);
     if (++b->done_seq == 0) b->done_seq = 1;
     *done_word = 0;
-    CKC(launch_pnp(s, P.obj, P.img, m, P.K, P.samples, iterations, P.thr, confidence, P.models, P.masks, P.counts,
-                   P.rt_out, P.inliers, P.info, P.host_out, stamps_on() ? b->d_stamps : nullptr, flag_wait ? b->done_seq : 0u));
+    if (ctx->pnp_mode == 0 && pnp_fused_fits(P.obj, P.img, m, P.K))
+        CKC(launch_pnp_fused(s, P.obj, P.img, m, P.K, P.samples, iterations, P.thr, confidence, P.models, P.masks, P.counts, P.rt_out, P.inliers,
+                             P.info, P.host_out, stamps_on() ? b->d_stamps : nullptr, flag_wait ? b->done_seq : 0u, b->d_pnp_flags, b->done_seq));
+    else
+        CKC(launch_pnp(s, P.obj, P.img, m, P.K, P.samples, iterations, P.thr, confidence, P.models, P.masks, P.counts,
+                       P.rt_out, P.inliers, P.info, P.host_out, stamps_on() ? b->d_stamps : nullptr, flag_wait ? b->done_seq : 0u));
     if ((rc = wait_done_word(ctx, s, done_word, b->done_seq, flag_wait))) return rc;
+    REQ(((const PnPResultHdr*)((const char*)b->h_stage + L.out))->info[0] >= 0, PMV_ERR_HIP, "pmv_pnp_ransac: a hypothesis of the launch never reported");
     pnp_finish(ctx, b, obj_xyz, img_xy, m, K, rvec, tvec, iterations, reproj_err, confidence, L, out_inliers, out_n_inliers);
     return PMV_OK;
 }
@@ -374,6 +380,11 @@
 
 extern "C" {
 
+int pmv_set_pnp_mode(pmv_ctx* ctx, int mode) {
+    if (!ctx || (mode != 0 && mode != 1)) { set_err(ctx, "pmv_set_pnp_mode: mode must be 0 (one launch) or 1 (hypotheses and refit as two launches)"); return PMV_ERR_INVALID; }
+    ctx->pnp_mode = mode;
+    return PMV_OK;
+}
 int pmv_set_ba_mode(pmv_ctx* ctx, int mode) {
     if (!ctx || (mode != 0 && mode != 1)) { set_err(ctx, "pmv_set_ba_mode: mode must be 0 (launch chain) or 1 (one workgroup per solve)"); return PMV_ERR_INVALID; }
     ctx->ba_mode = mode;
diff --git a/practical-multi-view_amd/csrc/backend_ba.hip b/practical-multi-view_amd/csrc/backend_ba.hip
--- a/practical-multi-view_amd/csrc/backend_ba.hip
+++ b/practical-multi-view_amd/csrc/backend_ba.hip
@@ -1596,7 +1596,9 @@
 }
 
 hipError_t backend_prepare_device() {
-    hipError_t e = hipFuncSetAttribute((const void*)k_bam_solve, hipFuncAttributeMaxDynamicSharedMemorySize, 150 * 1024);
+    hipError_t e = pnp_prepare_device();
+    if (e != hipSuccess) return e;
+    e = hipFuncSetAttribute((const void*)k_bam_solve, hipFuncAttributeMaxDynamicSharedMemorySize, 150 * 1024);
     if (e != hipSuccess) return e;
     e = hipFuncSetAttribute((const void*)k_bamB_solve, hipFuncAttributeMaxDynamicSharedMemorySize, 150 * 1024);
     if (e != hipSuccess) return e;
diff --git a/practical-multi-view_amd/csrc/backend_pnp.hip b/practical-multi-view_amd/csrc/backend_pnp.hip
--- a/practical-multi-view_amd/csrc/backend_pnp.hip
+++ b/practical-multi-view_amd/csrc/backend_pnp.hip
@@ -7,6 +7,28 @@
 namespace pmv {
 
 #define WAVE_SYNC_PNP() asm volatile("s_waitcnt lgkmcnt(0)" ::: "memory")
+
+constexpr int PNP_FUSED_MAX_M = 2048;
+__host__ __device__ inline int pnp_in_granules(int m) { return (int)((PNP_HDR + (size_t)m * 20 + 15) / 16); }
+inline size_t pnp_fused_lds(int m) { return (size_t)pnp_in_granules(m) * 16 + (size_t)m * 4; }
+template <int T>
+__device__ __forceinline__ void pnp_stage_in(float4* dst, const float4* __restrict__ src, int n_gran, int tid) {
+    for (int gb = tid; gb < n_gran; gb += 8 * T) {
+#define PNP_LD(u) const int g##u = gb + u * T; float4 v##u = make_float4(0.f, 0.f, 0.f, 0.f); if (g##u < n_gran) v##u = src[g##u];
+#define PNP_ST(u) if (g##u < n_gran) dst[g##u] = v##u;
+        PNP_LD(0) PNP_LD(1) PNP_LD(2) PNP_LD(3) PNP_LD(4) PNP_LD(5) PNP_LD(6) PNP_LD(7)
+        PNP_ST(0) PNP_ST(1) PNP_ST(2) PNP_ST(3) PNP_ST(4) PNP_ST(5) PNP_ST(6) PNP_ST(7)
+#undef PNP_LD
+#undef PNP_ST
+    }
+}
+__device__ __forceinline__ void pnp_publish(unsigned long long* flag, unsigned tag, int count, int lane) {
+    asm volatile("s_waitcnt vmcnt(0)" ::: "memory");
+    __builtin_amdgcn_fence(__ATOMIC_RELEASE, "agent");
+    asm volatile("s_waitcnt vmcnt(0)" ::: "memory");
+    if (lane == 0) __hip_atomic_store(flag, ((unsigned long long)tag << 32) | (unsigned)count, __ATOMIC_RELAXED, __HIP_MEMORY_SCOPE_AGENT);
+}
+constexpr unsigned long long PNP_WAIT_TICKS = 5000000ull;
 
 struct EpnpShared {
     double A[144], V[144];
@@ -151,25 +173,37 @@
     return rot;
 }
 
-template <bool LDS_L>
+template <bool LDS_L, bool FUSED = false>
 __device__ __forceinline__ void pnp_hyp_body(const float* __restrict__ obj, const float* __restrict__ img,
                                              const int* __restrict__ samples, const double* __restrict__ K,
                                              double* __restrict__ models, int m, float thr, uint8_t* __restrict__ masks,
-                                             int* __restrict__ counts, unsigned long long* stamps, const int h) {
+                                             int* __restrict__ counts, unsigned long long* stamps, const int h,
+                                             float4* lds_blk = nullptr, unsigned long long* flags = nullptr, unsigned tag = 0) {
     __shared__ EpnpShared sh;
     __shared__ double sR[9], sT[3];
     const int lane = threadIdx.x;
+#define HYP_BLOCK_SYNC() do { if constexpr (FUSED) WAVE_SYNC_PNP(); else __syncthreads(); } while (0)
     unsigned long long t_prev = __builtin_readcyclecounter();
 #define HSTAMP(k) do { if (stamps && h == 0 && lane == 0) { const unsigned long long t_ = __builtin_readcyclecounter(); stamps[k] += t_ - t_prev; t_prev = t_; } } while (0)
     const double fu = K[0], fv = K[4], uc = K[2], vc = K[5];
     const int n = 5;
+    const float* pobj = obj;
+    const float* pimg = img;
+    int s_fused = 0;
+    if constexpr (FUSED) {
+        if (lane < n) s_fused = samples[h * 5 + lane];
+        pnp_stage_in<64>(lds_blk, (const float4*)K, pnp_in_granules(m), lane);
+        pobj = (const float*)((const char*)lds_blk + PNP_HDR);
+        pimg = pobj + 3 * m;
+        WAVE_SYNC_PNP();
+    }
     if (lane < n) {
         const double ifx = 1. / fu, ify = 1. / fv;
         const int i = lane;
-        const int s = samples[h * 5 + i];
-        sh.pws[3 * i] = obj[3 * s]; sh.pws[3 * i + 1] = obj[3 * s + 1]; sh.pws[3 * i + 2] = obj[3 * s + 2];
-        const float xn = (float)(((double)img[2 * s] - uc) * ifx);
-        const float yn = (float)(((double)img[2 * s + 1] - vc) * ify);
+        const int s = FUSED ? s_fused : samples[h * 5 + i];
+        sh.pws[3 * i] = pobj[3 * s]; sh.pws[3 * i + 1] = pobj[3 * s + 1]; sh.pws[3 * i + 2] = pobj[3 * s + 2];
+        const float xn = (float)(((double)pimg[2 * s] - uc) * ifx);
+        const float yn = (float)(((double)pimg[2 * s + 1] - vc) * ify);
         sh.us[2 * i] = xn * fu + uc;
         sh.us[2 * i + 1] = yn * fv + vc;
     }
@@ -223,7 +257,7 @@
             }
         }
     }
-    __syncthreads();
+    HYP_BLOCK_SYNC();
     HSTAMP(22);
     for (int idx = lane; idx < 144; idx += 64) {
         const int a = idx / 12, b = idx - a * 12;
@@ -233,7 +267,7 @@
         sh.A[idx] = acc;
         sh.V[idx] = (a == b) ? 1.0 : 0.0;
     }
-    __syncthreads();
+    HYP_BLOCK_SYNC();
     double tol_abs = 0;
     for (int i = 0; i < 12; i++) tol_abs += fabs(sh.A[i * 13]);
     tol_abs *= 1e-17;
@@ -316,7 +350,7 @@
         const double d = d_dot3(du, dw);
         sh.L[i * 10 + k] = (u == w) ? d : 2.0f * d;
     }
-    __syncthreads();
+    HYP_BLOCK_SYNC();
     HSTAMP(24);
     if (lane < 3) {
         const int N = lane + 1;
@@ -363,7 +397,7 @@
         for (int i = 0; i < 9; i++) sh.case_R[lane * 9 + i] = R[i];
         for (int i = 0; i < 3; i++) sh.case_t[lane * 3 + i] = t[i];
     }
-    __syncthreads();
+    HYP_BLOCK_SYNC();
     HSTAMP(27);
     if (lane == 0) {
         int N = 0;
@@ -374,20 +408,20 @@
         for (int i = 0; i < 3; i++) { models[h * 6 + i] = rv[i]; models[h * 6 + 3 + i] = sh.case_t[N * 3 + i]; sT[i] = sh.case_t[N * 3 + i]; }
         d_rodrigues_v2m(rv, sR);
     }
-    __syncthreads();
+    HYP_BLOCK_SYNC();
     HSTAMP(28);
     {
         const double t0 = sT[0], t1 = sT[1], t2 = sT[2];
         int good = 0;
         for (int i = lane; i < m; i += 64) {
-            const double X = obj[3 * i], Y = obj[3 * i + 1], Z = obj[3 * i + 2];
+            const double X = pobj[3 * i], Y = pobj[3 * i + 1], Z = pobj[3 * i + 2];
             double x = sR[0] * X + sR[1] * Y + sR[2] * Z + t0;
             double y = sR[3] * X + sR[4] * Y + sR[5] * Z + t1;
             double z = sR[6] * X + sR[7] * Y + sR[8] * Z + t2;
             z = z ? 1. / z : 1;
             x *= z; y *= z;
             const float px = (float)(x * fu + uc), py = (float)(y * fv + vc);
-            const float dx = img[2 * i] - px, dy = img[2 * i + 1] - py;
+            const float dx = pimg[2 * i] - px, dy = pimg[2 * i + 1] - py;
             const float e = dx * dx + dy * dy;
             const int f = e <= thr;
             masks[(size_t)h * m + i] = (uint8_t)f;
@@ -396,9 +430,11 @@
 #pragma unroll
         for (int o = 32; o > 0; o >>= 1) good += __shfl_xor(good, o, 64);
         if (lane == 0) counts[h] = good;
+        if constexpr (FUSED) pnp_publish(flags + h, tag, good, lane);
     }
     HSTAMP(29);
 #undef HSTAMP
+#undef HYP_BLOCK_SYNC
 }
 
 __device__ inline int d_ransac_update_num_iters(double p, double ep, int modelPoints, int maxIters) {
@@ -477,18 +513,59 @@
     __syncthreads();
 }
 
+template <bool FUSED = false>
 __device__ __forceinline__ void pnp_select_refit_body(const float* __restrict__ obj, const float* __restrict__ img, int m,
                                                       const double* __restrict__ K, const double* __restrict__ models,
                                                       const uint8_t* __restrict__ masks, const int* __restrict__ counts,
                                                       int n_hyp, double confidence, double* __restrict__ rt_out,
                                                       int* __restrict__ inliers, int* __restrict__ info, char* __restrict__ host_out,
-                                                      unsigned long long* stamps, const unsigned done_seq) {
+                                                      unsigned long long* stamps, const unsigned done_seq,
+                                                      float4* lds_blk = nullptr, const unsigned long long* flags = nullptr, unsigned tag = 0) {
     __shared__ RefitShared sh;
     const unsigned long long t_start = __builtin_readcyclecounter();
     unsigned long long t_lm0 = 0;
     int n_pass = 0;
     const int tid = threadIdx.x, lane = tid & 63, wid = tid >> 6;
-    if (tid == 0) {
+    const double* Kt = K;
+    const float* pobj = obj;
+    const float* pimg = img;
+    const int* inl = inliers;
+    int* inl_lds = nullptr;
+    if constexpr (FUSED) {
+        pnp_stage_in<RF_T>(lds_blk, (const float4*)K, pnp_in_granules(m), tid);
+        Kt = (const double*)lds_blk;
+        pobj = (const float*)((const char*)lds_blk + PNP_HDR);
+        pimg = pobj + 3 * m;
+        inl = inl_lds = (int*)(lds_blk + pnp_in_granules(m));
+        if (wid == 0) {
+            int maxGood = 0, niters = n_hyp > 1 ? n_hyp : 1, best = -1, last = -1, iter = 0;
+            const unsigned long long t_wait0 = wall_clock64();
+            while (iter < niters && iter < n_hyp) {
+                const int gi = iter + lane;
+                unsigned long long g = 0;
+                if (gi < n_hyp) g = __hip_atomic_load(flags + gi, __ATOMIC_RELAXED, __HIP_MEMORY_SCOPE_AGENT);
+                const unsigned long long bal = __ballot(gi < n_hyp && (unsigned)(g >> 32) == tag);
+                const int ready = bal == ~0ull ? 64 : __ffsll((unsigned long long)~bal) - 1;
+                if (ready == 0) {
+                    if (wall_clock64() - t_wait0 > PNP_WAIT_TICKS) { best = -2; break; }
+                    __builtin_amdgcn_s_sleep(2);
+                    continue;
+                }
+                for (int k = 0; k < ready && iter < niters; k++, iter++) {
+                    last = iter;
+                    const int good = __shfl((int)(unsigned)g, k);
+                    if (good > (maxGood > 4 ? maxGood : 4)) {
+                        best = iter;
+                        maxGood = good;
+                        niters = d_ransac_update_num_iters(confidence, (double)(m - good) / m, 5, niters);
+                    }
+                }
+            }
+            if (lane == 0) { sh.best = best; sh.last = last; sh.n_in = 0; info[1] = last + 1; }
+            __builtin_amdgcn_fence(__ATOMIC_ACQUIRE, "agent");
+            asm volatile("s_waitcnt vmcnt(0)" ::: "memory");
+        }
+    } else if (tid == 0) {
         int maxGood = 0, niters = n_hyp > 1 ? n_hyp : 1, best = -1, last = -1;
         for (int iter = 0; iter < niters && iter < n_hyp; iter++) {
             last = iter;
@@ -503,6 +580,22 @@
         info[1] = last + 1;
     }
     __syncthreads();
+    if (FUSED && sh.best < 0) {
+        const int n0 = sh.best == -2 ? -1 : 0, l = sh.last < 0 ? 0 : sh.last;
+        double v = 0;
+        if (tid < 6 && n0 == 0) v = models[l * 6 + tid];
+        if (tid < 6) { rt_out[tid] = v; if (host_out) ((double*)host_out)[tid] = v; }
+        if (tid == 0) {
+            info[0] = n0;
+            if (host_out) { ((int*)(host_out + PNP_OUT_INFO))[0] = n0; ((int*)(host_out + PNP_OUT_INFO))[1] = sh.last + 1; }
+        }
+        if (host_out && done_seq) {
+            __threadfence_system();
+            __syncthreads();
+            if (tid == 0) __hip_atomic_store((unsigned*)(host_out + PNP_OUT_DONE), done_seq, __ATOMIC_RELEASE, __HIP_MEMORY_SCOPE_SYSTEM);
+        }
+        return;
+    }
     if (sh.best < 0) {
         if (tid == 0) {
             info[0] = 0;
@@ -527,7 +620,7 @@
         __syncthreads();
         int off = base;
         for (int w = 0; w < wid; w++) off += sh.wsum[w];
-        if (f) inliers[off + before] = i;
+        if (f) { inliers[off + before] = i; if constexpr (FUSED) inl_lds[off + before] = i; }
         const int tot = sh.wsum[0] + sh.wsum[1] + sh.wsum[2] + sh.wsum[3];
         __syncthreads();
         base += tot;
@@ -537,15 +630,15 @@
     if (tid < 6) { sh.param[tid] = models[sh.last * 6 + tid]; }
     if (tid == 0) { sh.lambdaLg10 = -3; sh.iters = 0; sh.done = 0; sh.state = 0; }
     __syncthreads();
-    const double fx = K[0], fy = K[4], cx = K[2], cy = K[5];
+    const double fx = Kt[0], fy = Kt[4], cx = Kt[2], cy = Kt[5];
     constexpr int RF_KEEP = 2;
     double keepX[RF_KEEP][3], keepU[RF_KEEP][2];
 #pragma unroll
     for (int q = 0; q < RF_KEEP; q++) {
         const int e = tid + q * RF_T;
-        const int i = e < n ? inliers[e] : 0;
-        keepX[q][0] = (double)obj[3 * i]; keepX[q][1] = (double)obj[3 * i + 1]; keepX[q][2] = (double)obj[3 * i + 2];
-        keepU[q][0] = (double)img[2 * i]; keepU[q][1] = (double)img[2 * i + 1];
+        const int i = e < n ? inl[e] : 0;
+        keepX[q][0] = (double)pobj[3 * i]; keepX[q][1] = (double)pobj[3 * i + 1]; keepX[q][2] = (double)pobj[3 * i + 2];
+        keepU[q][0] = (double)pimg[2 * i]; keepU[q][1] = (double)pimg[2 * i + 1];
     }
     t_lm0 = __builtin_readcyclecounter();
     for (;;) {
@@ -562,9 +655,9 @@
             if (q == 0) { X[0] = keepX[0][0]; X[1] = keepX[0][1]; X[2] = keepX[0][2]; U[0] = keepU[0][0]; U[1] = keepU[0][1]; }
             else if (q == 1) { X[0] = keepX[1][0]; X[1] = keepX[1][1]; X[2] = keepX[1][2]; U[0] = keepU[1][0]; U[1] = keepU[1][1]; }
             else {
-                const int i = inliers[e];
-                X[0] = (double)obj[3 * i]; X[1] = (double)obj[3 * i + 1]; X[2] = (double)obj[3 * i + 2];
-                U[0] = (double)img[2 * i]; U[1] = (double)img[2 * i + 1];
+                const int i = inl[e];
+                X[0] = (double)pobj[3 * i]; X[1] = (double)pobj[3 * i + 1]; X[2] = (double)pobj[3 * i + 2];
+                U[0] = (double)pimg[2 * i]; U[1] = (double)pimg[2 * i + 1];
             }
             double Xc[3], dpdw[9];
             d_angle_axis_rotate_jac(pa, X, Xc, dpdw);
@@ -623,7 +716,7 @@
                 for (int a = 0; a < 6; a++) { sh.JtErr[a] = sh.red[21 + a]; sh.prev[a] = sh.param[a]; }
             }
             if (do_step) {
-                const double lambda = K[10 + 16 + sh.lambdaLg10];
+                const double lambda = Kt[10 + 16 + sh.lambdaLg10];
                 double a[6][7];
 #pragma unroll
                 for (int i = 0; i < 6; i++) {
@@ -685,7 +778,7 @@
         if (tid < 6) ((double*)host_out)[tid] = sh.param[tid];
         if (tid == 0) { ((int*)(host_out + PNP_OUT_INFO))[0] = n; ((int*)(host_out + PNP_OUT_INFO))[1] = sh.last + 1; }
         int* hin = (int*)(host_out + PNP_OUT_INLIERS);
-        for (int e = tid; e < n; e += RF_T) hin[e] = inliers[e];
+        for (int e = tid; e < n; e += RF_T) hin[e] = inl[e];
         if (done_seq) {
             __threadfence_system();
             __syncthreads();
@@ -730,6 +823,20 @@
     pnp_select_refit_body(p.obj, p.img, p.m, p.K, p.models, p.masks, p.counts, p.n_hyp, p.confidence, p.rt_out, p.inliers, p.info, p.host_out, nullptr, 0u);
 }
 
+__global__ __launch_bounds__(RF_T) void k_pnp_fused(const float* obj, const float* img, const int* samples, const double* K, double* models,
+                                                    int m, float thr, uint8_t* masks, int* counts, int n_hyp, double confidence, double* rt_out,
+                                                    int* inliers, int* info, char* host_out, unsigned long long* stamps, unsigned done_seq,
+                                                    unsigned long long* flags, unsigned tag) { BACKEND_PRIO();
+    extern __shared__ __attribute__((aligned(16))) float4 pnp_lds[];
+    if ((int)blockIdx.x < n_hyp) {
+        if (threadIdx.x >= 64) return;
+        pnp_hyp_body<false, true>(obj, img, samples, K, models, m, thr, masks, counts, stamps, blockIdx.x, pnp_lds, flags, tag);
+    } else {
+        pnp_select_refit_body<true>(obj, img, m, K, models, masks, counts, n_hyp, confidence, rt_out, inliers, info, host_out, stamps, done_seq,
+                                    pnp_lds, flags, tag);
+    }
+}
+
 hipError_t launch_pnp_batch(hipStream_t s, const PnPProblem* d_probs, int n_probs, int max_hyp) {
     if (n_probs <= 0) return hipSuccess;
     if (!d_probs || max_hyp < 1) return hipErrorInvalidValue;
@@ -757,4 +864,21 @@
     return hipGetLastError();
 }
 
-}
+bool pnp_fused_fits(const float* d_obj, const float* d_img, int m, const double* d_K) {
+    return m <= PNP_FUSED_MAX_M && (const char*)d_obj == (const char*)d_K + PNP_HDR && d_img == d_obj + 3 * (size_t)m;
+}
+hipError_t launch_pnp_fused(hipStream_t s, const float* d_obj, const float* d_img, int m, const double* d_K, const int* d_samples,
+                            int n_hyp, float thr, double confidence, double* d_models, uint8_t* d_masks, int* d_counts,
+                            double* d_rt_out, int* d_inliers, int* d_info, char* host_out, unsigned long long* d_stamps, unsigned done_seq,
+                            unsigned long long* d_flags, unsigned tag) {
+    if (!pnp_fused_fits(d_obj, d_img, m, d_K) || !d_flags || !tag) return hipErrorInvalidValue;
+    ProfScope ps(K_PNP_HYP, s);
+    hipLaunchKernelGGL(k_pnp_fused, dim3(n_hyp + 1), dim3(RF_T), pnp_fused_lds(m), s, d_obj, d_img, d_samples, d_K, d_models, m, thr, d_masks,
+                       d_counts, n_hyp, confidence, d_rt_out, d_inliers, d_info, host_out, d_stamps, done_seq, d_flags, tag);
+    return hipGetLastError();
+}
+hipError_t pnp_prepare_device() {
+    return hipFuncSetAttribute((const void*)k_pnp_fused, hipFuncAttributeMaxDynamicSharedMemorySize, (int)pnp_fused_lds(PNP_FUSED_MAX_M));
+}
+
+}
diff --git a/practical-multi-view_amd/csrc/pmv_ctx.h b/practical-multi-view_amd/csrc/pmv_ctx.h
--- a/practical-multi-view_amd/csrc/pmv_ctx.h
+++ b/practical-multi-view_amd/csrc/pmv_ctx.h
@@ -84,6 +84,7 @@
     hipStream_t s_ahead = nullptr;
     std::mutex ahead_mu;
     int ba_mode = 0;
+    int pnp_mode = 0;
     int frame_format = PMV_FRAMES_GRAY;
     pmv_frame_preproc preproc = {};
     std::atomic<long long> preproc_launches[4];
```

Result: faster. 3737, median of 5 (+3.3%).
